# google/speedy

Measured on AMD Instinct MI355X. Metric: Msamples/s processed (16 kHz mono, 3.5x nonlinear), higher is better.
Workload: dtype int16 samples; f64 DFT, f32 features, int32 AMDF/OLA

## Files before the change

### include/speedy_hip.h

```cpp
#ifndef SPEEDY_HIP_H_
#define SPEEDY_HIP_H_
#include <stddef.h>
#include <stdint.h>
#ifdef __cplusplus
extern "C" {
#endif

#ifndef SPX_FEATURE_COUNT
#define SPX_FEATURE_COUNT 15
#endif

typedef struct spx_plan* spx_plan_t;

typedef struct {
  int64_t in_off;
  int64_t n_in;
  int64_t out_off;
  int64_t out_cap;
  int32_t channels;
  float speed;
  float nonlinear;
  float feedback;
} spx_stream_job;

// ... 16 lines not shown
int spx_plan_future(spx_plan_t plan);
int spx_plan_max_required(spx_plan_t plan);
int64_t spx_plan_frames(spx_plan_t plan, int64_t n_in);
int64_t spx_plan_out_capacity(spx_plan_t plan, int64_t n_in, float speed);
int64_t spx_plan_out_capacity_for(spx_plan_t plan, int64_t n_in, float speed, float nonlinear);

size_t spx_batch_workspace_bytes(spx_plan_t plan, const spx_stream_job* jobs, int n_streams);

int spx_batch_run(spx_plan_t plan, const spx_stream_job* jobs, int n_streams, const int16_t* in,
                  int16_t* out, int64_t* n_out, void* workspace, size_t workspace_bytes,
                  const spx_taps* taps, void* hip_stream);

int spx_batch_run_rate(spx_plan_t plan, const spx_stream_job* jobs, const float* rates, int n_streams, const int16_t* in,
                       int16_t* out, int64_t* n_out, void* workspace, size_t workspace_bytes,
                       const spx_taps* taps, void* hip_stream);
size_t spx_batch_workspace_bytes_rate(spx_plan_t plan, const spx_stream_job* jobs, const float* rates, int n_streams);
int64_t spx_plan_out_capacity_rate(spx_plan_t plan, int64_t n_in, float speed, float nonlinear, float rate);

size_t spx_batch_workspace_bytes_float(spx_plan_t plan, const spx_stream_job* jobs, const float* rates, int n_streams);
int spx_batch_run_float(spx_plan_t plan, const spx_stream_job* jobs, const float* rates, int n_streams, const float* in,
                        float* out, int64_t* n_out, void* workspace, size_t workspace_bytes,
                        const spx_taps* taps, void* hip_stream);
int spx_float_to_short(const float* in, int16_t* out, size_t n, int nonlinear_scale, void* hip_stream);
int spx_short_to_float(const int16_t* in, float* out, size_t n, void* hip_stream);

int spx_batch_run_ahead(spx_plan_t plan, const spx_stream_job* jobs, int n_streams, const int16_t* in,
                        int16_t* out, int64_t* n_out, void* workspace, size_t workspace_bytes,
                        const spx_taps* taps, void* hip_stream);

int spx_batch_run_overlapped(spx_plan_t plan, const spx_stream_job* jobs, int n_streams, const int16_t* in,
                             int16_t* out, int64_t* n_out, void* workspace, size_t workspace_bytes,
                             const spx_taps* taps, void* hip_stream);

int spx_batch_run_ahead_when(spx_plan_t plan, const spx_stream_job* jobs, int n_streams, const int16_t* in,
                             int16_t* out, int64_t* n_out, void* workspace, size_t workspace_bytes,
                             const spx_taps* taps, void* hip_stream, void* in_ready_event);

typedef struct spx_pipeline* spx_pipeline_t;
#define SPX_PIPELINE_DEVICE_OUT 1u
spx_pipeline_t spx_pipeline_create(spx_plan_t plan, const spx_stream_job* jobs, int n_streams, int depth, unsigned flags);
spx_pipeline_t spx_pipeline_create_mixed(const spx_plan_t* plans, int n_plans, const spx_stream_job* jobs, const int* plan_index,
                                         int n_streams, int depth, unsigned flags);
void spx_pipeline_destroy(spx_pipeline_t p);
int spx_pipeline_depth(spx_pipeline_t p);
size_t spx_pipeline_input_values(spx_pipeline_t p);
int16_t* spx_pipeline_host_input(spx_pipeline_t p);
int64_t spx_pipeline_submit(spx_pipeline_t p, const int16_t* in, int in_is_device);
int64_t spx_pipeline_submit_jobs(spx_pipeline_t p, const spx_stream_job* jobs, const int16_t* in, int in_is_device);
int spx_pipeline_jobs_fit(spx_pipeline_t p, const spx_stream_job* jobs);
int spx_pipeline_input_consumed(spx_pipeline_t p, int64_t ticket);
int spx_pipeline_wait(spx_pipeline_t p, int64_t ticket, const int16_t** out, const int64_t** offsets, const int64_t** counts);
void* spx_host_alloc(size_t bytes);
void spx_host_free(void* p);

int spx_batch_analyze(spx_plan_t plan, const spx_stream_job* jobs, int n_streams, const int16_t* in,
                      void* workspace, size_t workspace_bytes, const spx_taps* taps, void* hip_stream);
int spx_batch_walk(spx_plan_t plan, const spx_stream_job* jobs, int n_streams, const int16_t* in,
                   int16_t* out, int64_t* n_out, void* workspace, size_t workspace_bytes,
                   const spx_taps* taps, void* hip_stream);

size_t spx_batch_workspace_bytes_mixed(const spx_plan_t* plans, int n_plans, const spx_stream_job* jobs,
                                       const int* plan_index, int n_streams);
int spx_batch_run_mixed(const spx_plan_t* plans, int n_plans, const spx_stream_job* jobs, const int* plan_index,
                        int n_streams, const int16_t* in, int16_t* out, int64_t* n_out, void* workspace,
                        size_t workspace_bytes, void* hip_stream);

int spx_batch_run_mixed_taps(const spx_plan_t* plans, int n_plans, const spx_stream_job* jobs, const int* plan_index,
                             int n_streams, const int16_t* in, int16_t* out, int64_t* n_out, void* workspace,
                             size_t workspace_bytes, const spx_taps* taps, void* hip_stream);
int spx_batch_run_mixed_ahead(const spx_plan_t* plans, int n_plans, const spx_stream_job* jobs, const int* plan_index,
                              int n_streams, const int16_t* in, int16_t* out, int64_t* n_out, void* workspace,
                              size_t workspace_bytes, void* hip_stream);

void spx_set_timing(int enabled);
void spx_set_pipeline_chunks(int chunks);
void spx_set_concurrent(int on);
int spx_timing_collect(double* sum_ms_analyze, double* sum_ms_walk, int* n_calls);
const char* spx_batch_kernel_names(spx_plan_t plan, int n_streams, int max_channels, int speedup_only);
const char* spx_batch_kernel_names_lean(spx_plan_t plan, int n_streams, int max_channels, int speedup_only);
int spx_debug_last_walk_form(void);
int spx_debug_kernel_vgprs(int which);
int spx_debug_walk_info(int sample_rate, int channels, int n_streams, int speedup_only, int short_jobs, int lean, int* out5);
int spx_debug_analysis_info(int sample_rate, int* out4);
int spx_debug_mode_resources(int sample_rate, int channels, int n_streams, int speedup_only, long long* out22);
long long spx_debug_fdiv_check(unsigned seed, unsigned denominators, int exp_lo, int exp_hi);
long long spx_debug_xfade_check(int n_lo, int n_hi);
long long spx_debug_arith_check(unsigned seed, unsigned threads, unsigned per_thread);
int spx_debug_log_check(unsigned first_block, unsigned end_block, unsigned long long* sums);
int spx_debug_last_call_concurrent(void);
double spx_timing_last_tension_ms(void);
double spx_timing_last_rate_ms(void);

int spx_batch_read_steps(spx_plan_t plan, const spx_stream_job* jobs, int n_streams, const void* workspace,
                         int32_t* steps, void* hip_stream);
int spx_batch_read_steps_mixed(const spx_plan_t* plans, int n_plans, const spx_stream_job* jobs, const int* plan_index,
                               int n_streams, const void* workspace, int32_t* steps, void* hip_stream);

void* spx_device_alloc(size_t bytes);
void spx_device_free(void* p);
int spx_batch_pack_outputs(const spx_stream_job* jobs, int n_streams, const int16_t* out, const int64_t* n_out,
                           int16_t* packed, int64_t* offsets, void* hip_stream);
int spx_copy_to_device(void* dst, const void* src, size_t bytes, void* hip_stream);
int spx_copy_to_host(void* dst, const void* src, size_t bytes, void* hip_stream);
int spx_stream_synchronize(void* hip_stream);

#ifdef __cplusplus
}
#endif
#endif
```

### speedy_amd/_lib.py

```python
import ctypes as C
import os
import subprocess

_HERE = os.path.dirname(os.path.abspath(__file__))
LIB_PATH = os.environ.get("SPEEDY_HIP_LIB") or os.path.join(_HERE, "lib", "libspeedy_hip.so")
_LIB = None

c_short_p = C.POINTER(C.c_short)
c_float_p = C.POINTER(C.c_float)
c_int64_p = C.POINTER(C.c_int64)


class StreamJob(C.Structure):
    _fields_ = [("in_off", C.c_int64), ("n_in", C.c_int64), ("out_off", C.c_int64), ("out_cap", C.c_int64),
                ("channels", C.c_int32), ("speed", C.c_float), ("nonlinear", C.c_float), ("feedback", C.c_float)]


class Taps(C.Structure):
    _fields_ = [("tension", C.c_void_p), ("speed", C.c_void_p), ("features", C.c_void_p),
                ("spectrogram", C.c_void_p), ("normalized", C.c_void_p)]


TENSION_FN = C.CFUNCTYPE(None, C.c_void_p, C.c_int, C.c_float)
FEATURES_FN = C.CFUNCTYPE(None, C.c_void_p, C.c_int, c_float_p)

SYMBOLS = {
    "spx_last_error": (C.c_char_p, []),
    "spx_abi_version": (C.c_int, []),
    "spx_plan_create": (C.c_void_p, [C.c_int, C.c_int]),
    "spx_plan_destroy": (None, [C.c_void_p]),
    "spx_plan_frame_step": (C.c_int, [C.c_void_p]),
    "spx_plan_window_size": (C.c_int, [C.c_void_p]),
    "spx_plan_fft_size": (C.c_int, [C.c_void_p]),
    "spx_plan_future": (C.c_int, [C.c_void_p]),
    "spx_plan_max_required": (C.c_int, [C.c_void_p]),
    "spx_plan_frames": (C.c_int64, [C.c_void_p, C.c_int64]),
    "spx_plan_out_capacity": (C.c_int64, [C.c_void_p, C.c_int64, C.c_float]),
    "spx_plan_out_capacity_for": (C.c_int64, [C.c_void_p, C.c_int64, C.c_float, C.c_float]),
    "spx_batch_workspace_bytes": (C.c_size_t, [C.c_void_p, C.POINTER(StreamJob), C.c_int]),
    "spx_batch_run": (C.c_int, [C.c_void_p, C.POINTER(StreamJob), C.c_int, C.c_void_p, C.c_void_p, C.c_void_p,
                                C.c_void_p, C.c_size_t, C.POINTER(Taps), C.c_void_p]),
    "spx_batch_run_rate": (C.c_int, [C.c_void_p, C.POINTER(StreamJob), c_float_p, C.c_int, C.c_void_p, C.c_void_p, C.c_void_p,
                                     C.c_void_p, C.c_size_t, C.POINTER(Taps), C.c_void_p]),
    "spx_batch_workspace_bytes_rate": (C.c_size_t, [C.c_void_p, C.POINTER(StreamJob), c_float_p, C.c_int]),
    "spx_plan_out_capacity_rate": (C.c_int64, [C.c_void_p, C.c_int64, C.c_float, C.c_float, C.c_float]),
    "spx_batch_workspace_bytes_float": (C.c_size_t, [C.c_void_p, C.POINTER(StreamJob), c_float_p, C.c_int]),
    "spx_batch_run_float": (C.c_int, [C.c_void_p, C.POINTER(StreamJob), c_float_p, C.c_int, C.c_void_p, C.c_void_p, C.c_void_p,
                                      C.c_void_p, C.c_size_t, C.POINTER(Taps), C.c_void_p]),
    "spx_float_to_short": (C.c_int, [C.c_void_p, C.c_void_p, C.c_size_t, C.c_int, C.c_void_p]),
    "spx_short_to_float": (C.c_int, [C.c_void_p, C.c_void_p, C.c_size_t, C.c_void_p]),
    "spx_batch_run_ahead": (C.c_int, [C.c_void_p, C.POINTER(StreamJob), C.c_int, C.c_void_p, C.c_void_p, C.c_void_p,
                                      C.c_void_p, C.c_size_t, C.POINTER(Taps), C.c_void_p]),
    "spx_batch_run_overlapped": (C.c_int, [C.c_void_p, C.POINTER(StreamJob), C.c_int, C.c_void_p, C.c_void_p, C.c_void_p,
                                           C.c_void_p, C.c_size_t, C.POINTER(Taps), C.c_void_p]),
    "spx_batch_run_ahead_when": (C.c_int, [C.c_void_p, C.POINTER(StreamJob), C.c_int, C.c_void_p, C.c_void_p, C.c_void_p,
                                           C.c_void_p, C.c_size_t, C.POINTER(Taps), C.c_void_p, C.c_void_p]),
    "spx_batch_workspace_bytes_mixed": (C.c_size_t, [C.POINTER(C.c_void_p), C.c_int, C.POINTER(StreamJob), C.POINTER(C.c_int), C.c_int]),
    "spx_batch_run_mixed": (C.c_int, [C.POINTER(C.c_void_p), C.c_int, C.POINTER(StreamJob), C.POINTER(C.c_int), C.c_int,
                                      C.c_void_p, C.c_void_p, C.c_void_p, C.c_void_p, C.c_size_t, C.c_void_p]),
    "spx_batch_run_mixed_ahead": (C.c_int, [C.POINTER(C.c_void_p), C.c_int, C.POINTER(StreamJob), C.POINTER(C.c_int), C.c_int,
                                      C.c_void_p, C.c_void_p, C.c_void_p, C.c_void_p, C.c_size_t, C.c_void_p]),
    "spx_batch_run_mixed_taps": (C.c_int, [C.POINTER(C.c_void_p), C.c_int, C.POINTER(StreamJob), C.POINTER(C.c_int), C.c_int,
                                           C.c_void_p, C.c_void_p, C.c_void_p, C.c_void_p, C.c_size_t, C.POINTER(Taps), C.c_void_p]),
    "spx_batch_read_steps": (C.c_int, [C.c_void_p, C.POINTER(StreamJob), C.c_int, C.c_void_p, C.POINTER(C.c_int32), C.c_void_p]),
    "spx_batch_read_steps_mixed": (C.c_int, [C.POINTER(C.c_void_p), C.c_int, C.POINTER(StreamJob), C.POINTER(C.c_int), C.c_int,
                                             C.c_void_p, C.POINTER(C.c_int32), C.c_void_p]),
    "spx_batch_analyze": (C.c_int, [C.c_void_p, C.POINTER(StreamJob), C.c_int, C.c_void_p, C.c_void_p,
                                    C.c_size_t, C.POINTER(Taps), C.c_void_p]),
    "spx_batch_walk": (C.c_int, [C.c_void_p, C.POINTER(StreamJob), C.c_int, C.c_void_p, C.c_void_p, C.c_void_p,
                                 C.c_void_p, C.c_size_t, C.POINTER(Taps), C.c_void_p]),
    "spx_set_timing": (None, [C.c_int]),
    "spx_set_pipeline_chunks": (None, [C.c_int]),
    "spx_set_concurrent": (None, [C.c_int]),
    "spx_timing_collect": (C.c_int, [C.POINTER(C.c_double), C.POINTER(C.c_double), C.POINTER(C.c_int)]),
    "spx_timing_last_tension_ms": (C.c_double, []),
    "spx_timing_last_rate_ms": (C.c_double, []),
    "spx_batch_kernel_names": (C.c_char_p, [C.c_void_p, C.c_int, C.c_int, C.c_int]),
    "spx_batch_kernel_names_lean": (C.c_char_p, [C.c_void_p, C.c_int, C.c_int, C.c_int]),
    "spx_debug_last_walk_form": (C.c_int, []),
    "spx_debug_kernel_vgprs": (C.c_int, [C.c_int]),
    "spx_debug_last_call_concurrent": (C.c_int, []),
    "spx_debug_fdiv_check": (C.c_longlong, [C.c_uint, C.c_uint, C.c_int, C.c_int]),
    "spx_debug_xfade_check": (C.c_longlong, [C.c_int, C.c_int]),
    "spx_debug_arith_check": (C.c_longlong, [C.c_uint, C.c_uint, C.c_uint]),
    "spx_debug_log_check": (C.c_int, [C.c_uint, C.c_uint, C.POINTER(C.c_ulonglong)]),
    "spx_debug_walk_info": (C.c_int, [C.c_int, C.c_int, C.c_int, C.c_int, C.c_int, C.c_int, C.POINTER(C.c_int)]),
    "spx_debug_analysis_info": (C.c_int, [C.c_int, C.POINTER(C.c_int)]),
    "spx_debug_mode_resources": (C.c_int, [C.c_int, C.c_int, C.c_int, C.c_int, C.POINTER(C.c_longlong)]),
    "spx_pipeline_create": (C.c_void_p, [C.c_void_p, C.POINTER(StreamJob), C.c_int, C.c_int, C.c_uint]),
    "spx_pipeline_create_mixed": (C.c_void_p, [C.POINTER(C.c_void_p), C.c_int, C.POINTER(StreamJob), C.POINTER(C.c_int), C.c_int, C.c_int, C.c_uint]),
    "spx_pipeline_destroy": (None, [C.c_void_p]),
    "spx_pipeline_depth": (C.c_int, [C.c_void_p]),
    "spx_pipeline_input_values": (C.c_size_t, [C.c_void_p]),
    "spx_pipeline_host_input": (C.c_void_p, [C.c_void_p]),
    "spx_pipeline_submit": (C.c_int64, [C.c_void_p, C.c_void_p, C.c_int]),
    "spx_pipeline_submit_jobs": (C.c_int64, [C.c_void_p, C.POINTER(StreamJob), C.c_void_p, C.c_int]),
    "spx_pipeline_jobs_fit": (C.c_int, [C.c_void_p, C.POINTER(StreamJob)]),
    "spx_pipeline_input_consumed": (C.c_int, [C.c_void_p, C.c_int64]),
    "spx_pipeline_wait": (C.c_int, [C.c_void_p, C.c_int64, C.POINTER(C.c_void_p), C.POINTER(C.c_void_p), C.POINTER(C.c_void_p)]),
    "spx_host_alloc": (C.c_void_p, [C.c_size_t]),
    "spx_host_free": (None, [C.c_void_p]),
    "spx_device_alloc": (C.c_void_p, [C.c_size_t]),
    "spx_device_free": (None, [C.c_void_p]),
    "spx_copy_to_device": (C.c_int, [C.c_void_p, C.c_void_p, C.c_size_t, C.c_void_p]),
    "spx_copy_to_host": (C.c_int, [C.c_void_p, C.c_void_p, C.c_size_t, C.c_void_p]),
    "spx_batch_pack_outputs": (C.c_int, [C.c_void_p, C.c_int, C.c_void_p, C.c_void_p, C.c_void_p, C.c_void_p, C.c_void_p]),
    "spx_stream_synchronize": (C.c_int, [C.c_void_p]),
    "sonicCreateStream": (C.c_void_p, [C.c_int, C.c_int]),
    "sonicDestroyStream": (None, [C.c_void_p]),
    "sonicWriteShortToStream": (C.c_int, [C.c_void_p, c_short_p, C.c_int]),
    "sonicReadShortFromStream": (C.c_int, [C.c_void_p, c_short_p, C.c_int]),
    "sonicWriteFloatToStream": (C.c_int, [C.c_void_p, c_float_p, C.c_int]),
    "sonicReadFloatFromStream": (C.c_int, [C.c_void_p, c_float_p, C.c_int]),
    "sonicSetRate": (None, [C.c_void_p, C.c_float]),
    "sonicSetSpeed": (None, [C.c_void_p, C.c_float]),
    "sonicFlushStream": (C.c_int, [C.c_void_p]),
    "sonicEnableNonlinearSpeedup": (None, [C.c_void_p, C.c_float]),
    "sonicSetDurationFeedbackStrength": (None, [C.c_void_p, C.c_float]),
    "getSonicBufferSize": (C.c_int, [C.c_void_p]),
    "sonicSpectrogramSize": (C.c_int, [C.c_void_p]),
    "sonicTensionCallback": (None, [C.c_void_p, TENSION_FN]),
    "getSonicTensionCallback": (C.c_void_p, [C.c_void_p]),
    "sonicSpeedCallback": (None, [C.c_void_p, TENSION_FN]),
    "getSonicSpeedCallback": (C.c_void_p, [C.c_void_p]),
    "sonicFeaturesCallback": (None, [C.c_void_p, FEATURES_FN]),
    "getSonicFeaturesCallback": (C.c_void_p, [C.c_void_p]),
    "sonicSpectrogramCallback": (None, [C.c_void_p, FEATURES_FN]),
    "getSonicSpectrogramCallback": (C.c_void_p, [C.c_void_p]),
    "sonicNormalizedSpectrogramCallback": (None, [C.c_void_p, FEATURES_FN]),
    "getSonicNormalizedSpectrogramCallback": (C.c_void_p, [C.c_void_p]),
    "sonicIntGetNumChannels": (C.c_int, [C.c_void_p]),
    "sonicIntGetSampleRate": (C.c_int, [C.c_void_p]),
    "sonicIntGetSpeed": (C.c_float, [C.c_void_p]),
    "sonicIntCreateStream": (C.c_void_p, [C.c_int, C.c_int]),
    "sonicIntDestroyStream": (None, [C.c_void_p]),
    "sonicIntSetSpeed": (None, [C.c_void_p, C.c_float]),
    "sonicIntSetRate": (None, [C.c_void_p, C.c_float]),
    "sonicIntWriteShortToStream": (C.c_int, [C.c_void_p, c_short_p, C.c_int]),
    "sonicIntWriteFloatToStream": (C.c_int, [C.c_void_p, c_float_p, C.c_int]),
    "sonicIntReadShortFromStream": (C.c_int, [C.c_void_p, c_short_p, C.c_int]),
    "sonicIntReadFloatFromStream": (C.c_int, [C.c_void_p, c_float_p, C.c_int]),
    "sonicIntFlushStream": (C.c_int, [C.c_void_p]),
    "sonicIntSamplesAvailable": (C.c_int, [C.c_void_p]),
    "sonicIntSetUserData": (None, [C.c_void_p, C.c_void_p]),
    "sonicIntGetUserData": (C.c_void_p, [C.c_void_p]),
    "speedyCreateStream": (C.c_void_p, [C.c_int]),
    "speedyDestroyStream": (None, [C.c_void_p]),
    "speedyInputFrameSize": (C.c_int, [C.c_void_p]),
    "speedyInputFrameStep": (C.c_int, [C.c_void_p]),
    "speedyFFTSize": (C.c_int, [C.c_void_p]),
    "speedyBinToFreq": (C.c_float, [C.c_void_p, C.c_int]),
    "speedyFreqToBin": (C.c_int, [C.c_void_p, C.c_float]),
    "speedyAddData": (None, [C.c_void_p, c_float_p, C.c_int64]),
    "speedyAddDataShort": (None, [C.c_void_p, c_short_p, C.c_int64]),
    "speedyComputeTension": (C.c_int, [C.c_void_p, C.c_int64, c_float_p]),
    "speedyComputeSpeedFromTension": (C.c_float, [C.c_float, C.c_float, C.c_float, C.c_void_p]),
    "speedyGetCurrentTime": (C.c_int64, [C.c_void_p]),
    "speedySpectrogram": (c_float_p, [C.c_void_p, c_float_p]),
    "speedyGetSpectrogram": (c_float_p, [C.c_void_p]),
    "speedyGetSpectrogramAtTime": (c_float_p, [C.c_void_p, C.c_int64]),
    "speedyGetNormalizedSpectrogram": (c_float_p, [C.c_void_p]),
    "speedyGetInternalState": (c_float_p, [C.c_void_p]),
    "speedyGetEnergyCompressed": (C.c_float, [C.c_void_p]),
    "speedyGetSpeechChanges": (C.c_float, [C.c_void_p]),
    "speedyHipHysteresisFuture": (C.c_int, [C.c_void_p]),
    "speedyHipHysteresisPast": (C.c_int, [C.c_void_p]),
    "speedyComputeSpectralDifference": (None, [C.c_void_p, c_float_p, c_float_p, C.c_int64]),
    "speedyComputeLocalEnergy": (None, [C.c_void_p, c_float_p, C.c_int64]),
    "speedySaveSpectrogramData": (None, [C.c_void_p, c_float_p, C.c_int64]),
    "speedyPreemphasisFilter": (None, [C.c_void_p, c_float_p, C.c_int]),
# ... 43 lines not shown
```

### speedy_amd/csrc/sonic2_api.hip

```cpp
#include <stdio.h>
#include <stdlib.h>
#include <string.h>

#include <algorithm>
#include <string>
#include <cmath>
#include <vector>

#include "../../include/sonic2.h"
#include "spx_internal.h"

#include <atomic>
static thread_local std::string g_api_err;
static std::atomic<int> g_match_matlab{0};

#include "sonic2_stream.h"

void spx_internal_set_api_error(const std::string& msg) { g_api_err = msg; }
void spx_api_error(const std::string& msg) { g_api_err = msg; }
int spx_internal_match_matlab() { return g_match_matlab.load(); }

static bool any_callback(sonicStream s) {
  return s->cbTension || s->cbSpeed || s->cbFeatures || s->cbSpectrogram || s->cbNormalized;
}
// ... 277 lines not shown
        }
    }
  }
  SlideBuf<int16_t>& tsmIn = s->mixed ? s->dTsm : s->dIn;
  J.tsmIn = &tsmIn;
  if (!s->dIn.p && !s->dIn.ensure(0, 64 * C, hs, 1 << 16, defer)) return 0;
  if (!tsmIn.p && !tsmIn.ensure(0, 64 * C, hs, 1 << 16, defer)) return 0;
  auto off16 = [&](const SlideBuf<int16_t>& b) -> int64_t {
    return (pool ? (int64_t)(reinterpret_cast<uintptr_t>(b.p) / sizeof(int16_t)) : 0) - b.origin;
  };
  SpxStreamDev& JA = J.JA;
  SpxStreamDev& JW = J.JW;
  memset(&JA, 0, sizeof(JA));
  JA.in_off = off16(s->dIn); JA.n_in = s->nIn;
  JA.out_off = off16(s->dOut); JA.out_cap = (s->dOut.origin + s->dOut.cap) / C;
  JA.frame_off = -s->dRec.origin;
  if (pool && s->dRec.p) JA.frame_off += s->dRec.p - spx_pool_arena_rec(pool);
  JA.n_frames = (int32_t)T; JA.frame_begin = (int32_t)fa;
  JA.channels = (int32_t)C;
  const int common = (flush ? SPX_F_FLUSH : 0) | (s->rateMode ? SPX_F_NO_TRUNC : 0) | (s->speedSet ? SPX_F_SPEED_SET : 0);
  s->speedSet = false;
  JA.flags = common | (s->tensionStarted ? 0 : SPX_F_INIT);
  JA.speed = s->globalSpeed; JA.nonlinear = nonlinear ? s->nonlinearFactor : 0.0f; JA.feedback = s->feedbackStrength;
  JA.tsm_shift = s->tsmShift;
  JA.tension_skip = (int32_t)s->tensionSkip;
  JA.first_tile = 0;
  JW = JA;
  JW.speed = s->tsmSpeed;
  JW.flags = common | (s->started ? 0 : SPX_F_INIT);
  if (s->mixed) {
    JW.in_off = off16(s->dTsm); JW.n_in = s->tPhys;
    JW.flags |= SPX_F_HANDED_IN | (nonlinear ? 0 : SPX_F_KEEP_SPEED);
    JW.handed_in = (int32_t)handedBefore;
    JW.ring_bufs = (int32_t)(s->nIn / B);
    if (flush && !direct) JW.nonlinear = (s->nonlinearFactor != 0.0f) ? s->nonlinearFactor : 1.0f;
  }
  if (!(JA.speed > 1.0f && JW.speed > 1.0f && JA.speed < SPX_FAST_MAX_SPEED && JW.speed < SPX_FAST_MAX_SPEED && JA.nonlinear >= 0.0f &&
        JA.nonlinear <= 1.0f))
    s->speedupOnly = false;
  J.speedupKernel = s->speedupOnly && !s->rateMode && !s->mixed;
  J.tiles = (nonlinear && T > fa) ? (int)((T - fa + P.tile_frames - 1) / P.tile_frames) : 0;
  return 1;
}

void spx_finish_job(sonicStream s, const SpxJobPlan& J) {
  const SpxPlanDev& P = *s->plan;
  const int F = P.F;
  s->started = true;
  s->dirty = true;
  s->outBound = J.need;
  s->handedHost = J.handedAfter;
  if (J.nonlinear) s->tensionStarted = true;
  const int64_t k_first = std::max(s->tensionDone, s->tensionSkip);
  if (J.hasRing) s->framesDone = std::max(s->framesDone, J.nonlinear ? J.T : J.fa);
  if (J.nonlinear) s->tensionDone = std::max<int64_t>(k_first, (J.T >= F) ? J.T - F + 1 : 0);
  if (J.flush) {
    if (J.hasRing && !J.direct) {
      s->tensionSkip = std::max(s->tensionSkip, J.nIn / P.B);
      s->tensionDone = std::max(s->tensionDone, s->tensionSkip);
    }
    s->tsmShift += 2 * (int64_t)P.maxRequired;
  }
}

static int launch_job(sonicStream s, bool flush, bool direct = false) {
  const SpxPlanDev& P = *s->plan;
  const int64_t C = s->channels;
  SpxJobPlan J;
  if (!spx_prepare_job(s, flush, direct, s->hs, nullptr, J)) return 0;
  static_assert(2 * 128 <= SPX_STAGE_JOB && sizeof(SpxStreamDev) <= 128, "job table slot");
  memset(s->hPinned, 0, 256);
  memcpy(s->hPinned, &J.JA, sizeof(SpxStreamDev));
  memcpy(s->hPinned + 128, &J.JW, sizeof(SpxStreamDev));
  SpxStreamDev* dJobW = reinterpret_cast<SpxStreamDev*>(reinterpret_cast<unsigned char*>(s->dJob) + 128);
  if (hipMemcpyAsync(s->dJob, s->hPinned, 256, hipMemcpyHostToDevice, s->hs) != hipSuccess) return 0;
  (void)hipEventRecord(s->evStaged, s->hs);
  SpxTapsDev td = {nullptr, nullptr, nullptr, nullptr, nullptr};
  const int64_t fo = J.JA.frame_off;
  if (J.taps) {
    td.tension = s->tTension.base() - fo; td.speed = s->tSpeed.base() - fo;
    td.features = s->tFeatures.base() - fo * SPX_FEATURE_COUNT;
    td.spectrogram = s->tSpec.base() - fo * P.N; td.normalized = s->tNorm.base() - fo * P.W;
  }
  if (J.tiles > 0) spx_launch_analysis(P, s->dJob, 1, J.tiles, s->dIn.p, s->dRec.p, td, nullptr, nullptr, s->hs);
  if (J.nonlinear) spx_launch_tension(P, s->dJob, 1, s->dState, s->dRec.p, s->dScr.p, td, nullptr, nullptr, s->hs);
  spx_launch_walk(P, {.n_streams = 1, .max_channels = (int)C, .speedup_only = J.speedupKernel, .short_jobs = true}, dJobW, J.tsmIn->p,
                  s->dOut.p, s->dNOut, s->dState, s->dScr.p, nullptr, 0, s->hs);
  if (s->rateMode)
    spx_launch_rate(s->dRate, s->dState, s->dNOut, s->dOut.base(), s->dFinal.base(),
                    (s->dFinal.origin + s->dFinal.cap) / C, (int)C, J.oldR, J.newR, s->rate, s->rate == 1.0f ? 1 : 0,
                    flush ? 1 : 0, s->hs);
  if (hipGetLastError() != hipSuccess) { spx_stream_fail(s, "kernel launch failed"); return 0; }
  const int64_t k_first = std::max(s->tensionDone, s->tensionSkip);
  spx_finish_job(s, J);
  if (J.taps && J.T > J.fa) run_callbacks(s, J.fa, J.T, k_first);
  return 1;
}

static bool enter_rate_mode(sonicStream s) {
  if (s->channels > SPX_RATE_MAX_CHANNELS) {
    g_api_err = "sonicSetRate != 1 supports at most 16 channels";
    return false;
  }
  if (!sync_stream(s)) return false;
  const int64_t C = s->channels;
  const int64_t n = s->outKnown - s->outRead;
  if (!s->dFinal.ensure(s->outRead * C, (s->outKnown + 4096) * C, s->hs, 1 << 16)) return false;
  if (n > 0 && hipMemcpyAsync(s->dFinal.base() + s->outRead * C, s->dOut.base() + s->outRead * C,
                              sizeof(int16_t) * (size_t)(n * C), hipMemcpyDeviceToDevice, s->hs) != hipSuccess)
    return false;
  SpxRateState* h = reinterpret_cast<SpxRateState*>(staging(s, sizeof(SpxRateState)));
  if (!h) return false;
  memset(h, 0, sizeof(*h));
  h->tsm_seen = s->outKnown;
  h->final_n = s->outKnown;
  if (hipMemcpyAsync(s->dRate, h, sizeof(*h), hipMemcpyHostToDevice, s->hs) != hipSuccess) return false;
  (void)hipEventRecord(s->evStaged, s->hs);
  s->finKnown = s->finBound = s->tsmSeenKnown = s->outKnown;
  s->rateMode = true;
  return true;
}

static bool enter_mixed(sonicStream s) {
  if (!sync_stream(s)) return false;
  const int64_t C = s->channels;
  if (s->mode == 0) {
    std::swap(s->dTsm, s->dIn);
    s->tPhys = s->nIn;
    s->nIn = 0;
  } else {
    const int64_t hi = s->handedHost * (int64_t)s->plan->B;
    int64_t lo = std::max<int64_t>(0, s->tsmBase - s->tsmShift - 16);
    lo = std::min(std::max(lo, s->dIn.origin / C), hi);
    s->dTsm.filled = 0;
    if (!s->dTsm.ensure(lo * C, hi * C + 64, s->hs, 1 << 16)) return false;
    if (hi > lo && hipMemcpyAsync(s->dTsm.base() + lo * C, s->dIn.base() + lo * C, sizeof(int16_t) * (size_t)((hi - lo) * C),
                                  hipMemcpyDeviceToDevice, s->hs) != hipSuccess)
      return false;
    s->tPhys = hi;
  }
  s->mixed = true;
  return true;
}

bool spx_settings_ok(sonicStream s) {
  if (!(s->globalSpeed > 0.0f) || !std::isfinite(s->globalSpeed) || !(s->tsmSpeed > 0.0f) || !std::isfinite(s->tsmSpeed)) {
    g_api_err = "sonicSetSpeed: speed must be finite and > 0";
    return false;
  }
  if (!(s->nonlinearFactor >= 0.0f && s->nonlinearFactor <= 1.0f)) {
    g_api_err = "sonicEnableNonlinearSpeedup: factor outside [0, 1] (sonic2.h:73-76; the blended speed could reach 0)";
    return false;
  }
  if (!(s->rate > 0.0f) || !std::isfinite(s->rate)) { g_api_err = "sonicSetRate: rate must be finite and > 0"; return false; }
  if (!std::isfinite(s->feedbackStrength)) { g_api_err = "sonicSetDurationFeedbackStrength: not finite"; return false; }
  return true;
}

static int write_shorts(sonicStream s, const short* in, int sampleCount, bool direct = false) {
  if (spx_stream_failed(s) || !spx_settings_ok(s)) return 0;
  const int want = (s->nonlinearFactor != 0.0f && !direct) ? 1 : 0;
  if (s->pooled && (direct || s->rate != 1.0f || any_callback(s) || (s->mode >= 0 && s->mode != want)) && !spx_pool_leave(s))
    return 0;
  if (!s->pooled) (void)hipSetDevice(s->device);
  if (s->rate != 1.0f && !s->rateMode && !enter_rate_mode(s)) return 0;
  if (want == 1 && !spx_internal_analysis_fits(*s->plan)) {
    g_api_err = "sample rate too high for the nonlinear path (the analysis tile does not fit one CU's LDS); linear mode only";
// ... 143 lines not shown
```

### speedy_amd/csrc/sonic2_pool.hip

```cpp
#include <sched.h>
#include <stdio.h>
#include <stdlib.h>
#include <string.h>

#include <atomic>
#include <chrono>
#include <condition_variable>
#include <mutex>
#include <thread>

#include "sonic2_stream.h"

static std::atomic<int> g_coalesce{-1};

struct PinBuf {
  unsigned char* p = nullptr;
  size_t cap = 0;
  bool reserve(size_t need, size_t keep) {
    if (need <= cap) return true;
    size_t n = cap ? cap : (1u << 20);
    while (n < need) n *= 2;
    unsigned char* np = nullptr;
    if (hipHostMalloc(reinterpret_cast<void**>(&np), n, hipHostMallocDefault) != hipSuccess) return false;
    if (p && keep) memcpy(np, p, keep);
// ... 387 lines not shown
    }
    g.i1 = j;
    groups.push_back(g);
    i = j;
  }
  const size_t b_jobs = sizeof(SpxStreamDev) * n;
  const size_t o_desc = 2 * b_jobs, o_copies = o_desc + sizeof(PoolDesc) * n;
  const size_t o_moves = (o_copies + sizeof(PoolCopy) * copies.size() + 15) & ~(size_t)15;
  const size_t b_tab = o_moves + sizeof(SpxMove) * moves.size();
  auto give_up = [&](const char* why) {
    for (auto& it : items) spx_stream_fail(it.s, why);
    end_run(P, run);
    return RUN_FAILED;
  };
  if (!P->hTab.reserve(b_tab + 64, 0)) return give_up("pinned table allocation failed");
  size_t res_elems = 0;
  int64_t max_slice = 0;
  std::vector<int64_t>& res_off = P->res_off;
  std::vector<int64_t>& res_cap = P->res_cap;
  res_off.resize(n);
  res_cap.resize(n);
  for (size_t i = 0; i < n; i++) {
    sonicStream s = items[i].s;
    res_cap[i] = std::max<int64_t>(0, items[i].J.need - s->outKnown);
    res_off[i] = (int64_t)res_elems;
    const int64_t e = res_cap[i] * s->channels;
    max_slice = std::max(max_slice, e);
    res_elems += (size_t)((e + 7) & ~(int64_t)7);
  }
  const size_t o_out = (sizeof(PoolResult) * n + 63) & ~(size_t)63;
  if (!P->hRes.reserve(o_out + res_elems * sizeof(int16_t) + 64, 0)) return give_up("pinned result allocation failed");
  const size_t w_states = (2 * b_jobs + 63) & ~(size_t)63, w_nout = w_states + ((sizeof(SpxStreamState) * n + 63) & ~(size_t)63);
  const size_t w_total = w_nout + sizeof(int64_t) * n;
  if (w_total > P->dWsCap) {
    if (P->dWs) (void)hipFree(P->dWs);
    P->dWs = nullptr;
    size_t cap = P->dWsCap ? P->dWsCap : 65536;
    while (cap < w_total) cap *= 2;
    if (hipMalloc(reinterpret_cast<void**>(&P->dWs), cap) != hipSuccess) { P->dWs = nullptr; P->dWsCap = 0; (void)hipGetLastError(); return give_up("pool workspace allocation failed"); }
    P->dWsCap = cap;
  }
  SpxStreamDev* hA = reinterpret_cast<SpxStreamDev*>(P->hTab.p);
  SpxStreamDev* hW = hA + n;
  PoolDesc* hD = reinterpret_cast<PoolDesc*>(P->hTab.p + o_desc);
  PoolCopy* hC = reinterpret_cast<PoolCopy*>(P->hTab.p + o_copies);
  for (size_t i = 0; i < n; i++) {
    sonicStream s = items[i].s;
    hA[i] = items[i].J.JA;
    hW[i] = items[i].J.JW;
    hW[i].first_tile = hA[i].first_tile;
    PoolDesc& D = hD[i];
    D.home = s->dState;
    D.out_base = s->dOut.base();
    D.out_from = s->outKnown;
    D.out_cap = items[i].J.JA.out_cap;
    D.res_off = res_off[i];
    D.res_cap = res_cap[i];
    D.channels = s->channels;
    D.pad = 0;
  }
  if (!copies.empty()) memcpy(hC, copies.data(), sizeof(PoolCopy) * copies.size());
  SpxMove* hM = reinterpret_cast<SpxMove*>(P->hTab.p + o_moves);
  if (!moves.empty()) memcpy(hM, moves.data(), sizeof(SpxMove) * moves.size());
  SpxStreamDev* dA = reinterpret_cast<SpxStreamDev*>(P->dWs);
  SpxStreamDev* dW = dA + n;
  SpxStreamState* dStates = reinterpret_cast<SpxStreamState*>(P->dWs + w_states);
  int64_t* dNout = reinterpret_cast<int64_t*>(P->dWs + w_nout);
  PoolResult* hR = reinterpret_cast<PoolResult*>(P->hRes.p);
  int16_t* hOut = reinterpret_cast<int16_t*>(P->hRes.p + o_out);

  const unsigned n_words = (unsigned)(2 * b_jobs / 4);
  const unsigned grid = std::max<unsigned>(std::max<unsigned>((unsigned)(copies.size() + moves.size()), (n_words + 255) / 256), 1u);
  const auto tp2 = std::chrono::steady_clock::now();
  hipLaunchKernelGGL(spx_pool_stage_kernel, dim3(grid), dim3(256), 0, P->hs, reinterpret_cast<const unsigned*>(hA),
                     reinterpret_cast<unsigned*>(dA), n_words, hD, dStates, (unsigned)n, hC, (unsigned)copies.size(), run_in,
                     hM, (unsigned)moves.size());
  auto tl = std::chrono::steady_clock::now();
  auto lap = [&](int k) { const auto t = std::chrono::steady_clock::now(); P->t_l[k] += std::chrono::duration<double>(t - tl).count(); tl = t; };
  lap(0);
  const SpxTapsDev no_taps = {nullptr, nullptr, nullptr, nullptr, nullptr};
  for (const Group& g : groups) {
    const SpxPlanDev& PL = *items[g.i0].s->plan;
    const int ng = (int)(g.i1 - g.i0);
    if (g.tiles > 0) spx_launch_analysis(PL, dA + g.i0, ng, g.tiles, nullptr, P->aRec, no_taps, nullptr, nullptr, P->hs);
    lap(1);
    bool any_nl = false;
    for (size_t i = g.i0; i < g.i1; i++) any_nl = any_nl || items[i].J.nonlinear;
    if (any_nl) spx_launch_tension(PL, dA + g.i0, ng, dStates + g.i0, P->aRec, P->aScr, no_taps, nullptr, nullptr, P->hs);
    lap(2);
    spx_launch_walk(PL, {.n_streams = ng, .max_channels = g.maxC, .speedup_only = items[g.i0].J.speedupKernel, .short_jobs = true}, dW + g.i0,
                    nullptr, nullptr, dNout + g.i0, dStates + g.i0, P->aScr, nullptr, 0, P->hs);
    lap(3);
  }
  const unsigned gy = (unsigned)std::min<int64_t>(64, std::max<int64_t>(1, (max_slice + 8191) / 8192));
  hipLaunchKernelGGL(spx_pool_gather_kernel, dim3((unsigned)n, gy), dim3(256), 0, P->hs, hD, dStates, dNout, hR, hOut);
  lap(4);
  P->launchErr = hipGetLastError();
  P->resOut = o_out;
  P->tLaunched = std::chrono::steady_clock::now();
  P->t_prep += sec(tp0, tp1); P->t_tab += sec(tp1, tp2); P->t_launch += sec(tp2, P->tLaunched);
  return RUN_LAUNCHED;
}

static bool complete_run(SpxPool* P, hipError_t se) {
  const auto tp4 = std::chrono::steady_clock::now();
  std::vector<SpxPool::Item>& items = P->items;
  std::vector<sonicStream>& run = P->run;
  const hipError_t le = P->launchErr;
  if (le != hipSuccess || se != hipSuccess) {
    const std::string why = std::string("coalesced launch failed: ") + hipGetErrorString(le != hipSuccess ? le : se);
    for (auto& it : items) spx_stream_fail(it.s, why);
    end_run(P, run);
    return false;
  }
  const size_t n = items.size();
  const std::vector<int64_t>& res_off = P->res_off;
  const std::vector<int64_t>& res_cap = P->res_cap;
  const PoolResult* hR = reinterpret_cast<const PoolResult*>(P->hRes.p);
  const int16_t* hOut = reinterpret_cast<const int16_t*>(P->hRes.p + P->resOut);
  for (size_t i = 0; i < n; i++) {
    sonicStream s = items[i].s;
    spx_finish_job(s, items[i].J);
    int64_t k = hR[i].n;
    if (k == SPX_NOUT_LOST_PRODUCER) {
      spx_stream_fail(s, "a producer kernel never delivered its frames (device-side poll limit reached)");
      k = s->outKnown;
    } else if (k < 0) {
      spx_stream_fail(s, "output capacity exceeded on the device");
      k = -k;
    }
    const int64_t avail = std::min(k, items[i].J.JA.out_cap) - s->outKnown;
    const int64_t fresh = std::max<int64_t>(0, std::min(avail, res_cap[i]));
    if (avail > res_cap[i] && !s->failed)
      spx_stream_fail(s, "the device produced more frames than the host-side bound of the job (coalesced result slice)");
    if (fresh > 0) {
      const int16_t* src = hOut + res_off[i];
      s->hostOut.insert(s->hostOut.end(), src, src + fresh * s->channels);
    }
    s->outKnown += fresh;
    s->outBound = s->outKnown;
    s->tsmBase = hR[i].st.w.base;
    s->curSpeedKnown = hR[i].st.curSpeed;
    s->dirty = false;
    s->writesSinceSync = 0;
    s->devIn = items[i].J.nIn;
  }
  P->runs++;
  P->jobs += n;
  end_run(P, run);
  const auto tp5 = std::chrono::steady_clock::now();
  P->t_wait += sec(P->tLaunched, tp4); P->t_post += sec(tp4, tp5);
  return true;
}

static bool await_run(SpxPool* P, std::unique_lock<std::mutex>& lk) {
  P->detached.store(false, std::memory_order_release);
  static const long spin_us = [] { const char* e = getenv("SPX_POOL_SPIN_US"); return e ? atol(e) : 2000L; }();
  lk.unlock();
  hipError_t se = hipErrorNotReady;
  if (spin_us > 0) {
    const auto t_spin = std::chrono::steady_clock::now();
    while ((se = hipStreamQuery(P->hs)) == hipErrorNotReady) {
      if (std::chrono::duration<double, std::micro>(std::chrono::steady_clock::now() - t_spin).count() > (double)spin_us) break;
    }
    if (se == hipErrorNotReady) (void)hipGetLastError();
  }
  if (se == hipErrorNotReady) se = hipStreamSynchronize(P->hs);
// ... 227 lines not shown
```

### speedy_amd/csrc/spx_analysis.hip

```cpp
#include <stdlib.h>

#include "spx_internal.h"
#include "spx_walk_common.h"

#ifndef SPX_TF
#define SPX_TF 16
#endif

#ifdef SPX_STAMPS
__device__ unsigned long long g_spx_astamps[16];
#define ASTAMP_DECL unsigned long long as_last = __builtin_readcyclecounter(), as_acc[10] = {0,0,0,0,0,0,0,0,0,0};
#define ASTAMP(i) do { const unsigned long long t_ = __builtin_readcyclecounter(); as_acc[i] += t_ - as_last; as_last = t_; } while (0)
#define ASTAMP_FLUSH if (threadIdx.x == 0 && blockIdx.x == 7) for (int i_ = 0; i_ < 10; i_++) g_spx_astamps[i_] += as_acc[i_];
extern "C" void spx_debug_astamps(unsigned long long* out, int reset) {
  (void)hipMemcpyFromSymbol(out, HIP_SYMBOL(g_spx_astamps), sizeof(unsigned long long) * 16);
  if (reset) { unsigned long long z[16] = {0}; (void)hipMemcpyToSymbol(HIP_SYMBOL(g_spx_astamps), z, sizeof(z)); }
}
#else
#define ASTAMP_DECL
#define ASTAMP(i)
#define ASTAMP_FLUSH
#endif

#ifndef SPX_TF_SMALL
#define SPX_TF_SMALL 8
#endif
#define SPX_TF_TINY 4
int spx_analysis_tile_frames() { return SPX_TF; }
int spx_analysis_small_tile_frames() { return SPX_TF_SMALL; }
int spx_analysis_tiny_tile_frames() { return SPX_TF_TINY; }

#define SPX_CB 24
static __host__ __device__ constexpr int spx_mag_stride(int W) { return (W + 4) & ~3; }
static __host__ __device__ constexpr int spx_cb(int tf) { return tf <= 8 ? 2 * SPX_CB : SPX_CB; }
#ifdef SPX_LOG_V1
#define SPX_LOG_LDS_BYTES 0
#else
#define SPX_LOG_LDS_BYTES 2048
#endif
static __host__ __device__ inline size_t terms_bytes(int W, int tf, bool ct) {
  const size_t b = ct ? (size_t)2 * tf * (spx_cb(tf) + 1) * sizeof(double)
                      : (size_t)tf * (W + 1) * sizeof(double);
  return (b + 15) & ~(size_t)15;
}
static __host__ __device__ inline size_t work_bytes(int W, int tf, bool ct = false, int dft_waves = 4) {
  if (dft_waves < 1 || dft_waves > 4) dft_waves = 4;
  const size_t a = ct ? (size_t)4 * 2 * W * sizeof(double)
                      : (size_t)dft_waves * 2 * 2 * W * sizeof(double);
  const size_t b = terms_bytes(W, tf, ct) + SPX_LOG_LDS_BYTES;
  return (a > b ? a : b);
}
static inline int plan_ct_window(const SpxPlanDev& P) {
  auto is = [](const int* r, int n, std::initializer_list<int> want) {
    if (n != (int)want.size()) return false;
    int k = 0;
    for (int w : want) if (r[k++] != w) return false;
    return true;
  };
  if (!P.rader && P.W == 240 && is(P.radix, P.nstages, {4, 4, 3, 5})) return 240;
  if (!P.rader && P.W == 330 && is(P.radix, P.nstages, {2, 3, 5, 11})) return 330;
  if (P.tile_frames == SPX_TF_SMALL && P.dft_waves == 4) {
    if (!P.rader && P.W == 720 && is(P.radix, P.nstages, {4, 4, 3, 3, 5})) return 720;
    if (P.rader && P.W == 661 && is(P.radixM, P.nstagesM, {4, 3, 5, 11})) return 661;
  }
  if (!P.rader && P.dft_waves == 4) {
    if (P.W == 120 && is(P.radix, P.nstages, {4, 2, 3, 5}) && (P.tile_frames == SPX_TF || P.tile_frames == SPX_TF_SMALL)) return 120;
    if (P.W == 180 && is(P.radix, P.nstages, {4, 3, 3, 5}) && P.tile_frames == SPX_TF) return 180;
    if (P.W == 360 && is(P.radix, P.nstages, {4, 2, 3, 3, 5}) && P.tile_frames == SPX_TF) return 360;
    if (P.W == 480 && is(P.radix, P.nstages, {4, 4, 2, 3, 5}) && P.tile_frames == SPX_TF) return 480;
  }
  return 0;
}
int spx_analysis_prefers_small_tile(const SpxPlanDev& P) {
  SpxPlanDev Q = P;
  Q.tile_frames = SPX_TF_SMALL;
  Q.dft_waves = 4;
  const int w = plan_ct_window(Q);
  return w == 720 || w == 661;
}
static __host__ __device__ inline size_t stage_samples(const SpxPlanDev& P, int tf) {
  return (size_t)(tf + 1) * P.B + (P.W - P.B) + 8;
}
static size_t analysis_lds_bytes(const SpxPlanDev& P, bool ct) {
  const int tf = P.tile_frames > 0 ? P.tile_frames : SPX_TF;
  size_t mags = (size_t)(tf + 1) * spx_mag_stride(P.W) * sizeof(float);
  size_t small = (size_t)3 * (tf + 1) * sizeof(float);
  size_t stage = (stage_samples(P, tf) * sizeof(short) + 15) & ~(size_t)15;
  return work_bytes(P.W, tf, ct, P.dft_waves) + ((mags + 15) & ~(size_t)15) + ((small + 15) & ~(size_t)15) + stage;
}
size_t spx_analysis_lds_bytes(const SpxPlanDev& P) { return analysis_lds_bytes(P, plan_ct_window(P) != 0); }
int spx_analysis_ct_window(const SpxPlanDev& P) { return plan_ct_window(P); }

__device__ __forceinline__ void wave_sync() {
  __builtin_amdgcn_fence(__ATOMIC_RELEASE, "wavefront");
  __builtin_amdgcn_wave_barrier();
  __builtin_amdgcn_fence(__ATOMIC_ACQUIRE, "wavefront");
}

#include "spx_log.h"

__device__ __forceinline__ float spx_untangle_mag(double ar, double ai, double b_r, double b_i, double2 w) {
  const double dr = ar - b_r, di = ai - b_i;
#ifdef SPX_DFT_V1
  const double er = 0.5 * (ar + b_r), ei = 0.5 * (ai + b_i);
  const double o_r = 0.5 * di, o_i = -0.5 * dr;
  const double xr = er + (w.x * o_r - w.y * o_i);
  const double xi = ei + (w.x * o_i + w.y * o_r);
  return spx_sqrt64_to_f32(xr * xr + xi * xi);
#else
  const double xr2 = __builtin_fma(w.x, di, __builtin_fma(w.y, dr, ar + b_r));
  const double xi2 = __builtin_fma(w.y, di, __builtin_fma(-w.x, dr, ai + b_i));
  return spx_sqrt64_to_f32(0.25 * __builtin_fma(xr2, xr2, xi2 * xi2));
#endif
}

#define C5_1 0.30901699437494742
#define C5_2 (-0.80901699437494742)
#define S5_1 0.95105651629515357
#define S5_2 0.58778525229247313
#define S3_1 0.86602540378443865

struct cplx {
  double r, i;
};

#ifdef SPX_DFT_V1
#define SPX_FMA_OR(a, b, c, unfused) (unfused)
#else
#define SPX_FMA_OR(a, b, c, unfused) __builtin_fma((a), (b), (c))
#endif
__host__ __device__ __forceinline__ cplx spx_cmul(cplx b, double wx, double wy) {
  return {SPX_FMA_OR(b.r, wx, -(b.i * wy), b.r * wx - b.i * wy), SPX_FMA_OR(b.r, wy, b.i * wx, b.r * wy + b.i * wx)};
}
__host__ __device__ __forceinline__ double spx_bf3h(double a0, double t1) { return SPX_FMA_OR(-0.5, t1, a0, a0 - 0.5 * t1); }
__host__ __device__ __forceinline__ double spx_bf5m(double a0, double c1, double t1, double c2, double t2) {
  return SPX_FMA_OR(c2, t2, __builtin_fma(c1, t1, a0), (a0 + c1 * t1) + c2 * t2);
}
__host__ __device__ __forceinline__ double spx_bf5n(double s1, double t3, double s2, double t4) { return SPX_FMA_OR(s1, t3, s2 * t4, s1 * t3 + s2 * t4); }
__host__ __device__ __forceinline__ double spx_bf5d(double s2, double t3, double s1, double t4) { return SPX_FMA_OR(s2, t3, -(s1 * t4), s2 * t3 - s1 * t4); }
__host__ __device__ __forceinline__ double spx_acc(double p, double w, double u) { return SPX_FMA_OR(w, u, p, p + w * u); }

__host__ __device__ __forceinline__ cplx ld(const double* buf, int idx) {
  const double2 v = *reinterpret_cast<const double2*>(buf + 2 * idx);
  return {v.x, v.y};
}
__host__ __device__ __forceinline__ void st_tw(double* buf, int idx, cplx b, const double* tw, int t) {
  const double2 w = *reinterpret_cast<const double2*>(tw + 2 * t);
  const cplx v = spx_cmul(b, w.x, w.y);
  *reinterpret_cast<double2*>(buf + 2 * idx) = make_double2(v.r, v.i);
}

__host__ __device__ void dft_stage(const int W, const double* tw, int r, int s, int cur, const double* x, double* y,
                                   int lane, const int nl) {
  const int m = cur / r;
  const int span = W / r;
  const unsigned inv_s = ((1u << 20) + (unsigned)s - 1u) / (unsigned)s;
  if (r == 4) {
    for (int b = lane; b < span; b += nl) {
      const int p = (int)(((unsigned)b * inv_s) >> 20), q = b - p * s;
      cplx a0 = ld(x, b), a1 = ld(x, b + span), a2 = ld(x, b + 2 * span), a3 = ld(x, b + 3 * span);
      cplx t0 = {a0.r + a2.r, a0.i + a2.i}, t1 = {a0.r - a2.r, a0.i - a2.i};
      cplx t2 = {a1.r + a3.r, a1.i + a3.i}, t3 = {a1.r - a3.r, a1.i - a3.i};
      cplx b0 = {t0.r + t2.r, t0.i + t2.i}, b2 = {t0.r - t2.r, t0.i - t2.i};
      cplx b1 = {t1.r + t3.i, t1.i - t3.r}, b3 = {t1.r - t3.i, t1.i + t3.r};
      const int o = q + s * 4 * p;
      const int tp = s * p;
      st_tw(y, o, b0, tw, 0);
      st_tw(y, o + s, b1, tw, tp);
      st_tw(y, o + 2 * s, b2, tw, 2 * tp);
      st_tw(y, o + 3 * s, b3, tw, 3 * tp);
    }
  } else if (r == 2) {
    for (int b = lane; b < span; b += nl) {
// ... 153 lines not shown
    for (int i = 0; i < R; i++) a[u][i] = load(u, i);
  }
  wave_sync();
#pragma unroll
  for (int u = 0; u < NP; u++) {
    const int b = lane + 64 * u;
    if (b < SPAN) {
      cplx o[R];
      ct_bfly<R>(a[u], o);
      const int p = b / S, q = b - p * S;
      const int base = q + S * R * p, tp = S * p;
      st(buf, base, o[0]);
#pragma unroll
      for (int j = 1; j < R; j++) st(buf, base + j * S, LAST ? o[j] : cmul_tw(o[j], twp[j * tp]));
    }
  }
  wave_sync();
}
template <int NPTS, int R>
struct ct_from_buf {
  const double* buf;
  int lane;
  __device__ __forceinline__ cplx operator()(int u, int i) const {
    constexpr int SPAN = NPTS / R;
    const int b = (lane + 64 * u < SPAN) ? lane + 64 * u : 0;
    return ld(buf, b + i * SPAN);
  }
};

template <int W, int ST, int S>
__device__ __forceinline__ void ct_stages_from(double* buf, const double2* __restrict__ twp, const int lane) {
  if constexpr (ST < ct_plan<W>::n) {
    constexpr int R = ct_plan<W>::r[ST];
    ct_stage<W, R, S>(buf, twp, lane, ct_from_buf<W, R>{buf, lane});
    ct_stages_from<W, ST + 1, S * R>(buf, twp, lane);
  }
}

template <int NPTS, int R>
__device__ __forceinline__ void ct_stage_prime_last(double* buf, const int lane, const double (&wc)[R - 1], const double (&ws)[R - 1]) {
  constexpr int SPAN = NPTS / R, H = (R - 1) / 2;
  static_assert(SPAN <= 64, "one pass");
  if (lane < SPAN) {
    cplx a[R];
#pragma unroll
    for (int i = 0; i < R; i++) a[i] = ld(buf, lane + SPAN * i);
    cplx uu[H], vv[H];
    cplx B0 = a[0];
#pragma unroll
    for (int i = 1; i <= H; i++) {
      uu[i - 1] = {a[i].r + a[R - i].r, a[i].i + a[R - i].i};
      vv[i - 1] = {a[i].r - a[R - i].r, a[i].i - a[R - i].i};
      B0.r = B0.r + uu[i - 1].r; B0.i = B0.i + uu[i - 1].i;
    }
    st(buf, lane, B0);
#pragma unroll
    for (int jj = 1; jj <= H; jj++) {
      cplx Pj = a[0], Qj = {0.0, 0.0};
#pragma unroll
      for (int i = 1; i <= H; i++) {
        const double wx = wc[(i * jj) % R - 1], wy = ws[(i * jj) % R - 1];
        Pj.r = spx_acc(Pj.r, wx, uu[i - 1].r); Pj.i = spx_acc(Pj.i, wx, uu[i - 1].i);
        if (i == 1) { Qj.r = wy * vv[0].r; Qj.i = wy * vv[0].i; }
        else { Qj.r = spx_acc(Qj.r, wy, vv[i - 1].r); Qj.i = spx_acc(Qj.i, wy, vv[i - 1].i); }
      }
      st(buf, lane + SPAN * jj, cplx{Pj.r - Qj.i, Pj.i + Qj.r});
      st(buf, lane + SPAN * (R - jj), cplx{Pj.r + Qj.i, Pj.i - Qj.r});
    }
  }
  wave_sync();
}

template <class T>
__device__ __forceinline__ const T* per_frame(const T* p) {
  asm volatile("" : "+s"(p));
  return p;
}
__device__ __forceinline__ double uniform_f64(double v) {
  return __longlong_as_double(((long long)__builtin_amdgcn_readfirstlane((int)(__double_as_longlong(v) >> 32)) << 32) |
                              (unsigned)__builtin_amdgcn_readfirstlane((int)__double_as_longlong(v)));
}

#ifdef SPX_PREEMPH_V1
#define SPX_WIN_SCALE 1.0f
__device__ __forceinline__ float spx_preemph_win_f32(double md, double mpd, float w) {
  const float x = (float)(md / 32768.0), xp = (float)(mpd / 32768.0);
  const float y = (float)(1.0 * (double)x - 0.97 * (double)xp);
  return y * w;
}
#else
#define SPX_WIN_SCALE 0x1p-15f
__device__ __forceinline__ float spx_preemph_win_f32(double md, double mpd, float w15) {
  const float yy = (float)(md - 0.97 * mpd);
  return yy * w15;
}
#endif
__device__ __forceinline__ double spx_preemph_win(double md, double mpd, float w) { return (double)spx_preemph_win_f32(md, mpd, w); }
__device__ __forceinline__ cplx packed_point(const short* fr, int n, int j, int prev0, float w0, float w1) {
  const int i0 = 2 * n;
  const int m0 = fr[i0], m1 = fr[i0 + 1];
  const int mp0 = (i0 > 0) ? (int)fr[i0 - 1] : ((j > 0) ? (int)fr[prev0] : 0);
  const double d0 = (double)m0;
  return {spx_preemph_win(d0, (double)mp0, w0 * SPX_WIN_SCALE), spx_preemph_win((double)m1, d0, w1 * SPX_WIN_SCALE)};
}

#ifndef SPX_AN_W_330
#define SPX_AN_W_330 3
#endif
#ifndef SPX_AN_W_BIG
#define SPX_AN_W_BIG 2
#endif
template <int TF, int WCT>
__global__ void __launch_bounds__(SPX_BLOCK, (WCT == 240 || WCT == 120 || WCT == 180) ? 4 : WCT == 330 ? SPX_AN_W_330 : (WCT == 661 || WCT == 720) ? SPX_AN_W_BIG : (WCT == 480 || WCT == 360) ? 2 : 1)
spx_analysis_kernel(SpxPlanDev P, const SpxStreamDev* __restrict__ streams, int n_streams,
                    const int16_t* __restrict__ in_base, SpxFrameRec* __restrict__ rec, SpxTapsDev taps,
                    const int* __restrict__ tile_order, int* tile_flags, const float* __restrict__ frames,
                    int frame_mode) {
  extern __shared__ __attribute__((aligned(16))) unsigned char lds[];
  const int W = WCT ? WCT : P.W, B = P.B, N = 2 * W;
  const int tid = threadIdx.x, lane = tid & 63, wave = tid >> 6;

  const int tile = tile_order ? tile_order[blockIdx.x] : (int)blockIdx.x;
  int lo = 0, hi = n_streams - 1;
  while (lo < hi) {
    int mid = (lo + hi + 1) >> 1;
    if (streams[mid].first_tile <= tile) lo = mid; else hi = mid - 1;
  }
  const SpxStreamDev S = streams[lo];
  const int T = S.n_frames;
  const int j0 = S.frame_begin + (tile - S.first_tile) * TF;
  const int j1 = min(j0 + TF, T);
  const int C = S.channels;
  const int16_t* __restrict__ in = in_base + S.in_off;

  double* work = reinterpret_cast<double*>(lds);
  const size_t wb = work_bytes(W, TF, WCT != 0, (WCT != 0) ? 4 : P.dft_waves);
  float* mags = reinterpret_cast<float*>(lds + wb);
  const size_t mags_b = (((size_t)(TF + 1) * spx_mag_stride(W) * sizeof(float)) + 15) & ~(size_t)15;
  float* fE = reinterpret_cast<float*>(lds + wb + mags_b);
  float* fThr = fE + (TF + 1);
  float* fInv = fThr + (TF + 1);
  const int MS = spx_mag_stride(W);

  const size_t small_b = (((size_t)3 * (TF + 1) * sizeof(float)) + 15) & ~(size_t)15;
  const double* ltw = P.tw;
  const double* ltw2 = P.tw2;
  short* smono = reinterpret_cast<short*>(lds + wb + mags_b + small_b);

  double* bufA = work + (size_t)wave * (WCT != 0 ? 2 : 4) * W;
  double* bufB = (WCT != 0) ? bufA : bufA + 2 * W;

  const int jfirst = (j0 > 0) ? j0 - 1 : 0;
  const int64_t sbase = (int64_t)jfirst * B;
  const int nstage = (j1 - jfirst) * B + (W - B);
  if (frames != nullptr) {
  } else if (C == 1) {
    const int16_t* __restrict__ src = in + sbase;
    for (int k0 = tid; k0 < nstage; k0 += 8 * SPX_BLOCK) {
      short v[8];
#pragma unroll
      for (int u = 0; u < 8; u++) { const int k = k0 + u * SPX_BLOCK; v[u] = (k < nstage) ? src[k] : (short)0; }
#pragma unroll
      for (int u = 0; u < 8; u++) { const int k = k0 + u * SPX_BLOCK; if (k < nstage) smono[k] = v[u]; }
    }
  } else {
    for (int k = tid; k < nstage; k += SPX_BLOCK) smono[k] = (short)mono_sample(in, sbase + k, C);
  }
  __syncthreads();

  ASTAMP_DECL
  if constexpr (WCT == 240) {
    const double2* twp = reinterpret_cast<const double2*>(P.tw);
    const double2* tw2p = reinterpret_cast<const double2*>(P.tw2);
    const int b = lane;
    const bool on60 = b < 60, on48 = b < 48;
    const int bb = on60 ? b : 0;
    double2 w1[3], w2[3], w3[2][2], wu[4];
    float wn[4];
#pragma unroll
    for (int j = 1; j < 4; j++) { w1[j - 1] = twp[bb * j]; w2[j - 1] = twp[4 * (bb >> 2) * j]; }
#pragma unroll
    for (int u = 0; u < 2; u++) {
      const int b3 = lane + 64 * u, p3 = (b3 < 80) ? (b3 >> 4) : 0;
      w3[u][0] = twp[16 * p3];
      w3[u][1] = twp[32 * p3];
    }
#pragma unroll
    for (int u = 0; u < 4; u++) { const int k = lane + 64 * u; wu[u] = tw2p[k < 240 ? k : 0]; }
    wn[0] = P.window[2 * bb]; wn[1] = P.window[2 * bb + 1]; wn[2] = P.window[2 * bb + 120]; wn[3] = P.window[2 * bb + 121];
#pragma unroll
    for (int k = 0; k < 4; k++) wn[k] *= SPX_WIN_SCALE;
    for (int s = wave; s <= TF; s += 4) {
      const int j = j0 - 1 + s;
      float* mrow = mags + (size_t)s * MS;
      if (j < 0 || j >= j1) {
        for (int k = lane; k < 240; k += SPX_WAVE) mrow[k] = 0.0f;
        continue;
      }
      const short* fr = smono + (size_t)(j - jfirst) * B;
      if (on60) {
        const int i0 = 2 * b, i1 = 2 * b + 120;
        const int m0 = fr[i0], m1 = fr[i0 + 1], m2 = fr[i1], m3 = fr[i1 + 1];
        const int mp0 = (i0 > 0) ? (int)fr[i0 - 1] : ((j > 0) ? (int)fr[(240 - B) - 1] : 0);
        const int mp2 = fr[i1 - 1];
        const double d0 = (double)m0, d2 = (double)m2;
        const cplx a0 = {spx_preemph_win(d0, (double)mp0, wn[0]), spx_preemph_win((double)m1, d0, wn[1])},
                   a1 = {spx_preemph_win(d2, (double)mp2, wn[2]), spx_preemph_win((double)m3, d2, wn[3])};
        const cplx b0 = {a0.r + a1.r, a0.i + a1.i}, b2 = {a0.r - a1.r, a0.i - a1.i};
        const cplx b1 = {a0.r + a1.i, a0.i - a1.r}, b3 = {a0.r - a1.i, a0.i + a1.r};
        st(bufA, 4 * b, b0);
        st(bufA, 4 * b + 1, cmul_tw(b1, w1[0]));
        st(bufA, 4 * b + 2, cmul_tw(b2, w1[1]));
        st(bufA, 4 * b + 3, cmul_tw(b3, w1[2]));
      }
      wave_sync();
      ASTAMP(0);
      if (on60) {
        const cplx a0 = ld(bufA, b), a1 = ld(bufA, b + 60), a2 = ld(bufA, b + 120), a3 = ld(bufA, b + 180);
        wave_sync();
        const cplx t0 = {a0.r + a2.r, a0.i + a2.i}, t1 = {a0.r - a2.r, a0.i - a2.i};
        const cplx t2 = {a1.r + a3.r, a1.i + a3.i}, t3 = {a1.r - a3.r, a1.i - a3.i};
        const cplx b0 = {t0.r + t2.r, t0.i + t2.i}, b2 = {t0.r - t2.r, t0.i - t2.i};
        const cplx b1 = {t1.r + t3.i, t1.i - t3.r}, b3 = {t1.r - t3.i, t1.i + t3.r};
        const int o = (b & 3) + 16 * (b >> 2);
        st(bufB, o, b0);
        st(bufB, o + 4, cmul_tw(b1, w2[0]));
        st(bufB, o + 8, cmul_tw(b2, w2[1]));
        st(bufB, o + 12, cmul_tw(b3, w2[2]));
      }
      wave_sync();
      {
        cplx q0[2], q1[2], q2[2];
#pragma unroll
        for (int u = 0; u < 2; u++) {
          const int b3i = (lane + 64 * u < 80) ? lane + 64 * u : 0;
          q0[u] = ld(bufB, b3i); q1[u] = ld(bufB, b3i + 80); q2[u] = ld(bufB, b3i + 160);
        }
        wave_sync();
#pragma unroll
        for (int u = 0; u < 2; u++) {
          const int b3i = lane + 64 * u;
          if (b3i < 80) {
            const cplx a0 = q0[u], a1 = q1[u], a2 = q2[u];
            const cplx t1 = {a1.r + a2.r, a1.i + a2.i};
            const cplx t2 = {spx_bf3h(a0.r, t1.r), spx_bf3h(a0.i, t1.i)};
            const cplx t3 = {S3_1 * (a1.r - a2.r), S3_1 * (a1.i - a2.i)};
            const cplx b0 = {a0.r + t1.r, a0.i + t1.i};
            const cplx b1 = {t2.r + t3.i, t2.i - t3.r}, b2 = {t2.r - t3.i, t2.i + t3.r};
            const int o = (b3i & 15) + 48 * (b3i >> 4);
            st(bufA, o, b0);
            st(bufA, o + 16, cmul_tw(b1, w3[u][0]));
            st(bufA, o + 32, cmul_tw(b2, w3[u][1]));
          }
        }
// ... 413 lines not shown
            const cplx a = ld(x, k);
            const double2 b = *reinterpret_cast<const double2*>(P.bfft + 2 * k);
            const cplx cc = spx_cmul(a, b.x, b.y);
            *reinterpret_cast<double2*>(x + 2 * k) = make_double2(cc.r, -cc.i);
          }
          wave_sync();
        }
      }
      const double inv = 1.0 / (double)M;
      const double* abuf = (P.nstagesM & 1) ? y : x;
      const cplx A0 = ld(abuf, M);
      wave_sync();
      for (int q = lane; q < M; q += SPX_WAVE) {
        const cplx c = ld(x, q);
        const double cr = c.r * inv, ci = -c.i * inv;
        *reinterpret_cast<double2*>(y + 2 * P.iperm[q]) = make_double2(x0.r + cr, x0.i + ci);
      }
      if (lane == 0) *reinterpret_cast<double2*>(y) = make_double2(x0.r + A0.r, x0.i + A0.i);
      wave_sync();
      { double* t = x; x = y; y = t; }
    } else {
      int sprod = 1, cur = W;
      for (int stg = 0; stg < P.nstages; stg++) {
        const int r = P.radix[stg];
        dft_stage(W, ltw, r, sprod, cur, x, y, lane, SPX_WAVE);
        wave_sync();
        double* t = x; x = y; y = t;
        sprod *= r;
        cur /= r;
      }
    }
    ASTAMP(1);
    float* spec_out = taps.spectrogram ? taps.spectrogram + (size_t)(S.frame_off + j) * N : nullptr;
    for (int k = lane; k < W; k += SPX_WAVE) {
      const int k2 = (k == 0) ? 0 : W - k;
      cplx a = ld(x, k), bb = ld(x, k2);
      const double b_r = bb.r, b_i = -bb.i;
      const float mag = spx_untangle_mag(a.r, a.i, b_r, b_i, *reinterpret_cast<const double2*>(ltw2 + 2 * k));
      mrow[k] = mag;
      if (spec_out) {
        spec_out[k] = mag;
        if (k > 0) spec_out[N - k] = mag;
        else spec_out[W] = (float)__builtin_fabs(a.r - a.i);
      }
    }
    wave_sync();
    ASTAMP(2);
  }
  ASTAMP(3);
  __syncthreads();
  ASTAMP(4);

  if (wave > 0) {
#ifdef SPX_ROWMAX_V1
    for (int s = wave - 1; s <= TF; s += 3) {
      const float* mrow = mags + (size_t)s * MS;
      float mx = 0.0f;
      for (int i = 1 + lane; i < W; i += SPX_WAVE) mx = fmaxf(mx, mrow[i]);
#pragma unroll
      for (int d = 32; d >= 1; d >>= 1) mx = fmaxf(mx, __shfl_xor(mx, d));
      if (lane == 0) fThr[s] = (float)((double)mx / 100.0);
    }
#else
    unsigned keep = 0u;
    int nrows = 0;
    for (int s = wave - 1; s <= TF; s += 3, nrows++) {
      const unsigned* mrow = reinterpret_cast<const unsigned*>(mags + (size_t)s * MS);
      unsigned m = 0u;
      for (int q = lane; 4 * q < W; q += SPX_WAVE) {
        const uint4 v = *reinterpret_cast<const uint4*>(mrow + 4 * q);
        const unsigned a = (q == 0) ? 0u : v.x;
        const unsigned b = (4 * q + 1 < W) ? v.y : 0u, c = (4 * q + 2 < W) ? v.z : 0u, d = (4 * q + 3 < W) ? v.w : 0u;
        const unsigned ab = a > b ? a : b, cd = c > d ? c : d;
        const unsigned abcd = ab > cd ? ab : cd;
        m = m > abcd ? m : abcd;
      }
      const float mx = wave_max_f(__builtin_bit_cast(float, m));
      if (lane == nrows) keep = __builtin_bit_cast(unsigned, mx);
    }
    if (lane < nrows) fThr[wave - 1 + 3 * lane] = (float)((double)__builtin_bit_cast(float, keep) / 100.0);
#endif
#ifndef SPX_LOG_V1
    if (tid < SPX_WAVE + 128)
      reinterpret_cast<uint4*>(reinterpret_cast<unsigned char*>(work) + terms_bytes(W, TF, WCT != 0))[tid - SPX_WAVE] =
          reinterpret_cast<const uint4*>(spx_log_table_dev)[tid - SPX_WAVE];
#endif
  } else if (tid <= TF) {
    const float4* r4 = reinterpret_cast<const float4*>(mags + (size_t)tid * MS);
    float e = 0.0f;
    __builtin_amdgcn_s_setprio(3);
    auto acc8 = [&](const float4& p, const float4& q) {
      const float4 pp = {p.x * p.x, p.y * p.y, p.z * p.z, p.w * p.w}, qq = {q.x * q.x, q.y * q.y, q.z * q.z, q.w * q.w};
      e += pp.x; e += pp.y; e += pp.z; e += pp.w;
      e += qq.x; e += qq.y; e += qq.z; e += qq.w;
    };
    {
      const float4 h = r4[0];
      if (1 < W) e += h.y * h.y;
      if (2 < W) e += h.z * h.z;
      if (3 < W) e += h.w * h.w;
    }
    int i = 4;
    float4 c0 = r4[1], c1 = r4[2], c2 = r4[3], c3 = r4[4];
#pragma unroll 1
    for (; i + 16 <= W; i += 16) {
      const float4 n0 = r4[(i >> 2) + 4], n1 = r4[(i >> 2) + 5], n2 = r4[(i >> 2) + 6], n3 = r4[(i >> 2) + 7];
      __builtin_amdgcn_sched_barrier(0);
      acc8(c0, c1);
      acc8(c2, c3);
      c0 = n0; c1 = n1; c2 = n2; c3 = n3;
    }
    {
      const float t[16] = {c0.x, c0.y, c0.z, c0.w, c1.x, c1.y, c1.z, c1.w, c2.x, c2.y, c2.z, c2.w, c3.x, c3.y, c3.z, c3.w};
#pragma unroll
      for (int u = 0; u < 16; u++)
        if (i + u < W) e += t[u] * t[u];
    }
    __builtin_amdgcn_s_setprio(0);
    const float eps = 2.2204e-16f;
    fE[tid] = e;
    fInv[tid] = (float)(1.0 / (__builtin_sqrt((double)e) + (double)eps));
  }
  __syncthreads();
  ASTAMP(5);

  const int nfr = j1 - j0;
#ifndef SPX_LOG_V1
  const SpxLogEntry* ltab = reinterpret_cast<const SpxLogEntry*>(reinterpret_cast<const unsigned char*>(work) + terms_bytes(W, TF, WCT != 0));
  auto log_of_ratio = [&](float ratio) -> double {
    double v = spx_log_v2_f32(ratio, ltab);
    if (__builtin_expect(!spx_log_v2_domain(ratio), 0)) v = spx_log_v1((double)ratio);
    return v;
  };
#else
  auto log_of_ratio = [&](float ratio) -> double { return spx_log_v1((double)ratio); };
#endif
  auto log_term = [&](int f, int i) -> double {
    const int sl = f + 1;
    const float cur = mags[(size_t)sl * MS + i], last = mags[(size_t)(sl - 1) * MS + i];
    const float thr = fThr[sl];
    double term = 0.0;
    if (cur > thr && last > thr) {
      const float eps = 2.2204e-16f;
      const float nc = cur * fInv[sl], nl = last * fInv[sl - 1];
      const float ratio = spx_fdiv32(nc + eps, nl + eps);
      term = __builtin_fabs(log_of_ratio(ratio));
    }
    return term;
  };
  auto write_rec = [&](int f, float lsd) {
    const float lowthr = (float)(0.04 * (double)1.41421f);
    const float e = fE[f + 1];
    SpxFrameRec r;
    r.energy = e;
    r.lsd = (e <= lowthr) ? 0.0f : lsd;
    rec[S.frame_off + j0 + f] = r;
  };
  if (taps.normalized) {
    for (int idx = tid; idx < nfr * W; idx += SPX_BLOCK) {
      const int f = idx / W, i = idx - f * W;
      const int j = j0 + f;
      const int row = j + (S.unit_time0 ? 0 : 1);
      if (row < T + (S.unit_time0 ? 1 : 0))
        taps.normalized[(size_t)(S.frame_off + row) * W + i] = mags[(size_t)(f + 1) * MS + i] * fInv[f + 1];
    }
    if (S.unit_time0) {
    } else if (j0 == 0) {
      for (int i = tid; i < W; i += SPX_BLOCK) taps.normalized[(size_t)S.frame_off * W + i] = 0.0f;
    } else if (j0 == S.frame_begin) {
      for (int i = tid; i < W; i += SPX_BLOCK)
        taps.normalized[(size_t)(S.frame_off + j0) * W + i] = mags[i] * fInv[0];
    }
  }
  if constexpr (WCT != 0) {
    constexpr int CB = spx_cb(TF);
    constexpr int CBS = CB + 1;
    static_assert(TF * CB == 2 * (SPX_BLOCK - SPX_WAVE), "two terms per lane of waves 1..3 and block");
    double* tblk = work;
    constexpr int NBLK = (WCT - 1 + CB - 1) / CB;
    float lsd = 0.0f;
    int fi[2], ci[2];
    bool ok[2];
#ifndef SPX_TERMS_V1
    const float* rowc[2];
    const float* rowl[2];
    float thrv[2], invc[2], invl[2];
#endif
#pragma unroll
    for (int t = 0; t < 2; t++) {
      const int it = tid - SPX_WAVE + t * (SPX_BLOCK - SPX_WAVE);
      fi[t] = wave > 0 ? it / CB : 0;
      ci[t] = wave > 0 ? it - fi[t] * CB : 0;
      ok[t] = wave > 0 && fi[t] < nfr;
#ifndef SPX_TERMS_V1
      const int fl = ok[t] ? fi[t] : 0;
      rowc[t] = mags + (size_t)(fl + 1) * MS;
      rowl[t] = mags + (size_t)fl * MS;
      thrv[t] = fThr[fl + 1];
      invc[t] = fInv[fl + 1];
      invl[t] = fInv[fl];
#endif
    }
    for (int k = 0; k <= NBLK; k++) {
      if (wave > 0) {
        if (k < NBLK) {
          double* tb = tblk + (size_t)(k & 1) * TF * CBS;
          bool gate[2];
          float xr[2];
#pragma unroll
          for (int t = 0; t < 2; t++) {
            const int i = 1 + k * CB + ci[t];
            const bool in = ok[t] && i < WCT;
#ifdef SPX_TERMS_V1
            const int fl = in ? fi[t] : 0, il = in ? i : 1;
            const float cur = mags[(size_t)(fl + 1) * MS + il], last = mags[(size_t)fl * MS + il];
            const float thr = fThr[fl + 1];
            const float fic = fInv[fl + 1], fil = fInv[fl];
#else
            const int il = (i < WCT) ? i : 1;
            const float cur = rowc[t][il], last = rowl[t][il];
            const float thr = thrv[t], fic = invc[t], fil = invl[t];
#endif
            gate[t] = in && cur > thr && last > thr;
            const float eps = 2.2204e-16f;
            const float nc = cur * fic, nl = last * fil;
            const float ratio = spx_fdiv32(nc + eps, nl + eps);
            xr[t] = gate[t] ? ratio : 2.0f;
          }
#ifdef SPX_LOG_V1
          const spx_log_parts p0 = spx_log_main((double)xr[0]), p1 = spx_log_main((double)xr[1]);
          const double t0 = gate[0] ? __builtin_fabs(spx_log_finish(p0, (double)xr[0])) : 0.0;
          const double t1 = gate[1] ? __builtin_fabs(spx_log_finish(p1, (double)xr[1])) : 0.0;
#else
          const double l0 = log_of_ratio(xr[0]), l1 = log_of_ratio(xr[1]);
          const double t0 = gate[0] ? __builtin_fabs(l0) : 0.0;
          const double t1 = gate[1] ? __builtin_fabs(l1) : 0.0;
#endif
          if (ok[0]) tb[fi[0] * CBS + ci[0]] = t0;
          if (ok[1]) tb[fi[1] * CBS + ci[1]] = t1;
        }
      } else if (k > 0 && tid < nfr) {
        const double* tb = tblk + (size_t)((k - 1) & 1) * TF * CBS + tid * CBS;
        const int i0 = 1 + (k - 1) * CB;
        __builtin_amdgcn_s_setprio(3);
        (void)i0;
        static_assert(CB % 8 == 0, "batches of eight");
        double tv[8];
#pragma unroll
        for (int u = 0; u < 8; u++) tv[u] = tb[u];
#pragma unroll
        for (int c = 0; c < CB; c += 8) {
          double nx[8];
          if (c + 8 < CB) {
#pragma unroll
            for (int u = 0; u < 8; u++) nx[u] = tb[c + 8 + u];
          }
#pragma unroll
          for (int u = 0; u < 8; u++) lsd = (float)((double)lsd + tv[u]);
          if (c + 8 < CB) {
#pragma unroll
            for (int u = 0; u < 8; u++) tv[u] = nx[u];
// ... 47 lines not shown
__global__ void spx_arith_check_kernel(unsigned seed, unsigned per_thread, unsigned long long* bad) {
  unsigned long long st = (unsigned long long)seed * 0x9E3779B97F4A7C15ull + (blockIdx.x * blockDim.x + threadIdx.x) * 0xD1B54A32D192ED03ull + 1;
  auto next = [&]() { st ^= st >> 12; st ^= st << 25; st ^= st >> 27; return st * 0x2545F4914F6CDD1Dull; };
  unsigned long long miss = 0;
  for (unsigned i = 0; i < per_thread; i++) {
    const unsigned long long a = next(), b = next(), c = next();
    const float fn = __uint_as_float((unsigned)((127 - 53 + (a % 57)) << 23) | (unsigned)((a >> 8) & 0x7fffff));
    const float fd = __uint_as_float((unsigned)((127 - 53 + (b % 57)) << 23) | (unsigned)((b >> 8) & 0x7fffff));
    if (__float_as_uint(spx_fdiv32(fn, fd)) != __float_as_uint(fn / fd)) miss++;
    const long long fb = ((long long)(1023 - 21 + (c % 20)) << 52) | (long long)((c >> 8) & 0xfffffffffffffll) | ((c >> 63) ? (1ll << 63) : 0);
    const double f = __longlong_as_double(fb);
    if (__double_as_longlong(spx_fdiv64(f, 2.0 + f)) != __double_as_longlong(f / (2.0 + f))) miss++;
    const long long xb = ((long long)(1023 - 800 + (a >> 33) % 1811) << 52) | (long long)((b >> 10) & 0xfffffffffffffll);
    const double x = ((c & 1023) == 0) ? 0.0 : __longlong_as_double(xb);
    if (__float_as_uint(spx_sqrt64_to_f32(x)) != __float_as_uint((float)__builtin_sqrt(x))) miss++;
  }
  if (miss) atomicAdd(bad, miss);
}
extern "C" long long spx_debug_arith_check(unsigned seed, unsigned threads, unsigned per_thread) {
  unsigned long long* d = nullptr;
  unsigned long long h = 0;
  if (hipMalloc(&d, sizeof(h)) != hipSuccess) return -1;
  if (hipMemcpy(d, &h, sizeof(h), hipMemcpyHostToDevice) != hipSuccess) { (void)hipFree(d); return -1; }
  const unsigned blocks = (threads + 255) / 256;
  hipLaunchKernelGGL(spx_arith_check_kernel, dim3(blocks), dim3(256), 0, nullptr, seed, per_thread, d);
  const bool ok = hipDeviceSynchronize() == hipSuccess && hipMemcpy(&h, d, sizeof(h), hipMemcpyDeviceToHost) == hipSuccess;
  (void)hipFree(d);
  return ok ? (long long)h : -1;
}

__global__ void __launch_bounds__(256) spx_log_check_kernel(unsigned first_block, unsigned long long* __restrict__ sums) {
#ifndef SPX_LOG_V1
  __shared__ SpxLogEntry tab[128];
  __shared__ unsigned long long acc;
  if (threadIdx.x < 128) reinterpret_cast<uint4*>(tab)[threadIdx.x] = reinterpret_cast<const uint4*>(spx_log_table_dev)[threadIdx.x];
  if (threadIdx.x == 0) acc = 0;
  __syncthreads();
  const unsigned b = first_block + blockIdx.x;
  unsigned long long sum = 0;
  for (unsigned i = threadIdx.x; i < (1u << 20); i += 256) {
    const float x = __uint_as_float((b << 20) | i);
    sum += (unsigned long long)__double_as_longlong(spx_log_v2_f32(x, tab));
  }
  atomicAdd(&acc, sum);
  __syncthreads();
  if (threadIdx.x == 0) sums[b] = acc;
#endif
}
extern "C" int spx_debug_log_check(unsigned first_block, unsigned end_block, unsigned long long* sums) {
#ifdef SPX_LOG_V1
  (void)first_block; (void)end_block; (void)sums;
  return -3;
#else
  if (first_block < 8) first_block = 8;
  if (end_block > 2040) end_block = 2040;
  if (!sums || first_block >= end_block) return -1;
  unsigned long long* d = nullptr;
  if (hipMalloc(&d, 2040 * sizeof(unsigned long long)) != hipSuccess) return -1;
  bool ok = hipMemset(d, 0, 2040 * sizeof(unsigned long long)) == hipSuccess;
  if (ok) hipLaunchKernelGGL(spx_log_check_kernel, dim3(end_block - first_block), dim3(256), 0, nullptr, first_block, d);
  ok = ok && hipDeviceSynchronize() == hipSuccess && hipMemcpy(sums, d, 2040 * sizeof(unsigned long long), hipMemcpyDeviceToHost) == hipSuccess;
  (void)hipFree(d);
  return ok ? 0 : -1;
#endif
}

SpxKernelChoice spx_analysis_select(int tile_frames, int ctw) {
#define AN_K(TFV, WV) SpxKernelChoice{"spx_analysis_kernel", reinterpret_cast<const void*>(spx_analysis_kernel<TFV, WV>), SPX_BLOCK, 2, {TFV, WV}}
  static_assert(std::is_same<decltype(spx_analysis_kernel<SPX_TF_TINY, 0>), SpxAnalysisArgs>::value, "SpxAnalysisArgs is the kernel's argument list");
  if (tile_frames == SPX_TF_TINY) return AN_K(SPX_TF_TINY, 0);
  if (tile_frames == SPX_TF_SMALL)
    return ctw == 240 ? AN_K(SPX_TF_SMALL, 240) : ctw == 330 ? AN_K(SPX_TF_SMALL, 330) : ctw == 720 ? AN_K(SPX_TF_SMALL, 720)
         : ctw == 661 ? AN_K(SPX_TF_SMALL, 661) : ctw == 120 ? AN_K(SPX_TF_SMALL, 120) : AN_K(SPX_TF_SMALL, 0);
  return ctw == 240 ? AN_K(SPX_TF, 240) : ctw == 330 ? AN_K(SPX_TF, 330) : ctw == 120 ? AN_K(SPX_TF, 120) : ctw == 360 ? AN_K(SPX_TF, 360)
       : ctw == 180 ? AN_K(SPX_TF, 180) : ctw == 480 ? AN_K(SPX_TF, 480) : AN_K(SPX_TF, 0);
#undef AN_K
}
int spx_analysis_vgprs(const SpxPlanDev& P, int* scratch_bytes) {
  return spx_kernel_vgprs(spx_analysis_select(P.tile_frames, plan_ct_window(P)).fn, scratch_bytes);
}

void spx_launch_analysis(const SpxPlanDev& P, const SpxStreamDev* streams, int n_streams, int n_tiles,
                         const int16_t* in, SpxFrameRec* rec, SpxTapsDev taps, const int* tile_order, int* tile_flags,
                         hipStream_t st) {
  if (n_tiles <= 0) return;
  SpxLaunch<SpxAnalysisArgs>::go(spx_analysis_select(P.tile_frames, plan_ct_window(P)), n_tiles, spx_analysis_lds_bytes(P), st, P, streams,
                                 n_streams, in, rec, taps, tile_order, tile_flags, nullptr, 0);
}

void spx_launch_analysis_frames(const SpxPlanDev& P, const SpxStreamDev* streams, int n_tiles, const float* frames,
                                bool preemph, SpxFrameRec* rec, SpxTapsDev taps, hipStream_t st) {
  if (n_tiles <= 0) return;
  SpxPlanDev Q = P;
  if (Q.tile_frames != SPX_TF_SMALL && Q.tile_frames != SPX_TF_TINY) Q.tile_frames = SPX_TF;
  SpxLaunch<SpxAnalysisArgs>::go(spx_analysis_select(Q.tile_frames, 0), n_tiles, analysis_lds_bytes(Q, false), st, Q, streams, 1, nullptr, rec,
                                 taps, nullptr, nullptr, frames, preemph ? 1 : 2);
}
```

### speedy_amd/csrc/spx_diag.hip

```cpp
#include "spx_engine.h"

extern "C" {
static const char* kernel_names(spx_plan_t plan, int n_streams, int max_channels, int speedup_only, bool lean);
const char* spx_batch_kernel_names(spx_plan_t plan, int n_streams, int max_channels, int speedup_only) {
  return kernel_names(plan, n_streams, max_channels, speedup_only, false);
}
const char* spx_batch_kernel_names_lean(spx_plan_t plan, int n_streams, int max_channels, int speedup_only) {
  return kernel_names(plan, n_streams, max_channels, speedup_only, true);
}
static const char* kernel_names(spx_plan_t plan, int n_streams, int max_channels, int speedup_only, bool lean) {
  static thread_local char buf[256];
  const SpxPlanDev& d = plan->dev;
  const SpxWalkConfig c = spx_walk_config(d, {.n_streams = n_streams, .max_channels = max_channels, .speedup_only = speedup_only != 0,
                                              .any_speed = speedup_only == 0, .lean = lean});
  size_t at = 0;
  auto put = [&](const SpxKernelChoice& k) {
    at += snprintf(buf + at, sizeof(buf) - at, "%s<", k.name);
    for (int i = 0; i < k.n_targs; i++) at += snprintf(buf + at, sizeof(buf) - at, i ? ", %d" : "%d", k.targs[i]);
    at += snprintf(buf + at, sizeof(buf) - at, ">");
  };
  put(spx_analysis_select(d.tile_frames, spx_analysis_ct_window(d)));
  at += snprintf(buf + at, sizeof(buf) - at, ";spx_tension_kernel;");
  put(c.kernel);
  return buf;
}

int spx_debug_last_call_concurrent(void) { return g_last_concurrent.load(std::memory_order_relaxed); }
int spx_debug_kernel_vgprs(int which) {
  if (which == 0) return spx_tension_vgprs();
  const int rate = (which == 2 || which == 4) ? 22050 : 16000;
  const SpxPlanDev* P = spx_internal_shared_plan(rate, 0);
  if (!P) return -1;
  switch (which) {
    case 1: return spx_walk_vgprs(*P, {.n_streams = 256, .max_channels = 1, .speedup_only = true}, nullptr);
    case 2: return spx_walk_vgprs(*P, {.n_streams = 256, .max_channels = 1, .speedup_only = true, .lean = true}, nullptr);
    case 3: case 4: return spx_analysis_vgprs(*P);
    case 5: return spx_walk_vgprs(*P, {.n_streams = 256, .max_channels = 2, .speedup_only = true}, nullptr);
    default: return -1;
  }
}

int spx_debug_walk_info(int sample_rate, int channels, int n_streams, int speedup_only, int short_jobs, int lean, int* out) {
  const SpxPlanDev* P = spx_internal_shared_plan(sample_rate, 0);
  if (!P || !out) return -1;
  const SpxWalkConfig c = spx_walk_config(*P, {.n_streams = n_streams, .max_channels = channels, .speedup_only = speedup_only != 0,
                                               .any_speed = speedup_only == 0, .short_jobs = short_jobs != 0, .lean = lean != 0});
  int scratch = -1;
  out[0] = spx_kernel_vgprs(c.kernel.fn, &scratch);
  out[1] = scratch;
  out[2] = (int)c.lds;
  out[3] = c.fast_kernel ? 16 * c.nwm + c.nwc : 0;
  out[4] = c.waves;
  return 0;
}
int spx_debug_analysis_info(int sample_rate, int* out) {
  const SpxPlanDev* P = spx_internal_shared_plan(sample_rate, 0);
  if (!P || !out) return -1;
  int scratch = -1;
  out[0] = spx_analysis_vgprs(*P, &scratch);
  out[1] = scratch;
  out[2] = (int)spx_analysis_lds_bytes(*P);
  out[3] = P->dft_waves;
  return 0;
}

void spx_set_timing(int enabled) { g_timing = enabled != 0; }
void spx_set_concurrent(int on) { g_concurrent = on != 0; }
void spx_set_pipeline_chunks(int chunks) { g_chunks_set = true; g_chunks = chunks < 1 ? 1 : (chunks > SPX_MAX_CHUNKS ? SPX_MAX_CHUNKS : chunks); }
static double g_last_tension_ms = 0.0, g_last_rate_ms = 0.0;
double spx_timing_last_tension_ms(void) { return g_last_tension_ms; }
double spx_timing_last_rate_ms(void) { return g_last_rate_ms; }
int spx_timing_collect(double* sum_ms_analyze, double* sum_ms_walk, int* n_calls) {
  std::lock_guard<std::mutex> g(g_tmu);
  double a = 0, w = 0, t = 0, r = 0;
  for (auto& ev : g_ev_pending) {
    HIPCHK(hipEventSynchronize(ev.b));
    float ms = 0;
    HIPCHK(hipEventElapsedTime(&ms, ev.a, ev.b));
    if (ev.kind == 0) a += ms; else if (ev.kind == 1) w += ms; else if (ev.kind == 3) r += ms; else t += ms;
    g_ev_free.push_back(ev.a);
    g_ev_free.push_back(ev.b);
  }
  g_ev_pending.clear();
  g_last_tension_ms = t;
  g_last_rate_ms = r;
  if (sum_ms_analyze) *sum_ms_analyze = a;
  if (sum_ms_walk) *sum_ms_walk = w;
  if (n_calls) *n_calls = g_calls_pending;
  g_calls_pending = 0;
  return 0;
}

void* spx_device_alloc(size_t bytes) {
  void* p = nullptr;
  if (hipMalloc(&p, bytes ? bytes : 1) != hipSuccess) { fail(-2, "spx_device_alloc failed"); return nullptr; }
  return p;
}
void spx_device_free(void* p) { if (p) (void)hipFree(p); }
int spx_copy_to_device(void* dst, const void* src, size_t bytes, void* hs) {
  HIPCHK(hipMemcpyAsync(dst, src, bytes, hipMemcpyHostToDevice, static_cast<hipStream_t>(hs)));
  return 0;
}
}

__global__ void __launch_bounds__(256)
spx_pack_offsets_kernel(const int64_t* __restrict__ n_out, const int* __restrict__ channels,
                        const int64_t* __restrict__ caps, int n, int64_t* __restrict__ offsets) {
  __shared__ int64_t sh[256];
  __shared__ int64_t carry;
  const int t = threadIdx.x;
  if (t == 0) carry = 0;
  __syncthreads();
  for (int i0 = 0; i0 < n; i0 += 256) {
    const int i = i0 + t;
    int64_t v = 0;
    if (i < n) {
      const int64_t k = n_out[i];
      int64_t f = (k == INT64_MIN ? 0 : (k > 0 ? k : -k));
      if (f > caps[i]) f = caps[i];
      v = f * channels[i];
    }
    sh[t] = v;
    __syncthreads();
    for (int d = 1; d < 256; d <<= 1) {
      const int64_t add = (t >= d) ? sh[t - d] : 0;
      __syncthreads();
      sh[t] += add;
      __syncthreads();
    }
    const int64_t base = carry;
    if (i < n) offsets[i] = base + sh[t] - v;
    __syncthreads();
    if (t == 255) carry = base + sh[255];
    __syncthreads();
  }
  if (t == 0) offsets[n] = carry;
}
__global__ void __launch_bounds__(256)
spx_pack_copy_kernel(const int16_t* __restrict__ out, const int64_t* __restrict__ out_offs,
                     const int64_t* __restrict__ offsets, int16_t* __restrict__ packed) {
  const int i = blockIdx.x;
  const int16_t* src = out + out_offs[i];
  int16_t* dst = packed + offsets[i];
  const int64_t cnt = offsets[i + 1] - offsets[i];
// ... 54 lines not shown
```

### speedy_amd/csrc/spx_engine.hip

```cpp
#include "spx_engine.h"

__attribute__((constructor(101))) static void spx_default_hw_queues() {
  if (getenv("SPX_KEEP_HW_QUEUES") || getenv("GPU_MAX_HW_QUEUES")) return;
  setenv("GPU_MAX_HW_QUEUES", "8", 0);
  if (getenv("SPX_DEBUG_MODE")) fprintf(stderr, "[spx] GPU_MAX_HW_QUEUES was unset: set to 8 at load time (SPX_KEEP_HW_QUEUES=1 leaves the environment alone)\n");
}

thread_local std::string g_spx_err;

std::atomic<bool> g_timing{false};
std::atomic<int> g_last_concurrent{0};
std::atomic<int> g_concurrent{1};
std::atomic<bool> g_chunks_set{false};
std::atomic<int> g_chunks{1};
std::mutex g_tmu;
std::vector<EvPair> g_ev_pending;
std::vector<hipEvent_t> g_ev_free;
int g_calls_pending = 0;

SpxDevGuard g_guard[64];

int spx_kernel_vgprs(const void* fn, int* scratch_bytes) {
  static std::mutex mu;
  static std::map<const void*, std::pair<int, int>> cache;
// ... 78 lines not shown
    const int64_t Ttot = nonlinear ? frames_for(d, j.n_in) : 0;
    int64_t Tprev = 0;
    for (int c = 0; c < nch; c++) {
      int64_t n_c = j.n_in;
      if (c < nch - 1) n_c = (j.n_in * (c + 1) / nch) / d.B * d.B;
      SpxStreamDev& s = v[(size_t)c * n + i];
      s.in_off = j.in_off; s.n_in = n_c; s.out_off = j.out_off; s.out_cap = j.out_cap;
      s.channels = j.channels; s.speed = j.speed; s.nonlinear = j.nonlinear; s.feedback = j.feedback;
      const int64_t T = nonlinear ? frames_for(d, n_c) : 0;
      s.n_frames = (int32_t)T;
      s.frame_begin = (int32_t)Tprev;
      s.flags = (c == 0 ? SPX_F_INIT : 0) | (c == nch - 1 ? SPX_F_FLUSH : 0);
      if (rc) {
        s.out_off = rc->walk_out_off[i]; s.out_cap = rc->walk_out_cap[i];
        if (rc->no_trunc[i]) s.flags |= SPX_F_NO_TRUNC;
      }
      s.frame_off = fo;
      s.first_tile = tiles_per_chunk[c];
      tiles_per_chunk[c] += (int)((T - Tprev + TF - 1) / TF);
      Tprev = T;
    }
    fo += Ttot;
  }
}

static SpxTapsDev taps_of(const spx_taps* t) {
  SpxTapsDev d = {nullptr, nullptr, nullptr, nullptr, nullptr};
  if (t) { d.tension = t->tension; d.speed = t->speed; d.features = t->features;
           d.spectrogram = t->spectrogram; d.normalized = t->normalized; }
  return d;
}

__global__ void spx_gate_kernel(const int* started, int n_walk, unsigned max_spins) {
  if (threadIdx.x == 0) {
    for (unsigned i = 0; i < max_spins; i++) {
      if (__hip_atomic_load(started, __ATOMIC_RELAXED, __HIP_MEMORY_SCOPE_AGENT) >= n_walk) break;
      __builtin_amdgcn_s_sleep(8);
    }
  }
}
void spx_launch_gate(const int* started, int n_walk, unsigned max_spins, hipStream_t st) {
  hipLaunchKernelGGL(spx_gate_kernel, dim3(1), dim3(64), 0, st, started, n_walk, max_spins);
}
__global__ void __launch_bounds__(256)
spx_stage_kernel(const unsigned* __restrict__ src, unsigned* __restrict__ dst_a, unsigned n_a, unsigned* __restrict__ dst_b,
                 unsigned n_b, unsigned* __restrict__ zero_a, unsigned nz_a, unsigned* __restrict__ zero_b, unsigned nz_b,
                 const int* gate_started, int gate_n, unsigned gate_spins) {
  const unsigned stride = gridDim.x * blockDim.x, t0 = blockIdx.x * blockDim.x + threadIdx.x;
  for (unsigned i = t0; i < n_a; i += stride) dst_a[i] = src[i];
  for (unsigned i = t0; i < n_b; i += stride) dst_b[i] = src[n_a + i];
  for (unsigned i = t0; i < nz_a; i += stride) zero_a[i] = 0u;
  for (unsigned i = t0; i < nz_b; i += stride) zero_b[i] = 0u;
  if (gate_started != nullptr && t0 == 0) {
    for (unsigned i = 0; i < gate_spins; i++) {
      if (__hip_atomic_load(gate_started, __ATOMIC_RELAXED, __HIP_MEMORY_SCOPE_AGENT) >= gate_n) break;
      __builtin_amdgcn_s_sleep(8);
    }
  }
}
extern "C" {

static hipEvent_t take_event() {
  std::lock_guard<std::mutex> g(g_tmu);
  if (!g_ev_free.empty()) { hipEvent_t e = g_ev_free.back(); g_ev_free.pop_back(); return e; }
  hipEvent_t e;
  (void)hipEventCreate(&e);
  return e;
}

}
int dev_side_streams(int dev, hipStream_t* side, hipStream_t* side2) {
  static std::mutex mu;
  static hipStream_t s1[64], s2[64];
  const int d = (dev >= 0 && dev < 64) ? dev : 0;
  std::lock_guard<std::mutex> g(mu);
  if (!s1[d]) {
    if (hipStreamCreateWithFlags(&s1[d], hipStreamNonBlocking) != hipSuccess) { s1[d] = nullptr; return -1; }
    if (hipStreamCreateWithFlags(&s2[d], hipStreamNonBlocking) != hipSuccess) { (void)hipStreamDestroy(s1[d]); s1[d] = nullptr; s2[d] = nullptr; return -1; }
  }
  *side = s1[d]; *side2 = s2[d];
  return 0;
}

int walk_stream_count() { return 2; }
int dev_walk_streams(int dev, hipStream_t* w, int n) {
  static std::mutex mu;
  static hipStream_t s3[64][SPX_MAX_WALK_STREAMS];
  hipStream_t side = nullptr, side2 = nullptr;
  if (dev_side_streams(dev, &side, &side2)) return -1;
  const int d = (dev >= 0 && dev < 64) ? dev : 0;
  std::lock_guard<std::mutex> g(mu);
  w[0] = side2;
  for (int i = 1; i < n && i < SPX_MAX_WALK_STREAMS; i++) {
    if (!s3[d][i] && hipStreamCreateWithFlags(&s3[d][i], hipStreamNonBlocking) != hipSuccess) { s3[d][i] = nullptr; return -1; }
    w[i] = s3[d][i];
  }
  return 0;
}

int ring_note(spx_plan* plan, hipStream_t st) {
  const int cur = plan->ahead_calls & 1;
  if (!plan->ev_call[cur]) HIPCHK(hipEventCreateWithFlags(&plan->ev_call[cur], hipEventDisableTiming));
  HIPCHK(hipEventRecord(plan->ev_call[cur], st));
  plan->ev_call_valid[cur] = true;
  plan->ev_call_st[cur] = st;
  return 0;
}
int ring_wait(spx_plan* plan, hipStream_t sa, const void* ws, hipStream_t st, bool* waited_prev) {
  const int c = plan->ahead_calls % SPX_RING;
  if (waited_prev) *waited_prev = false;
  for (int back = SPX_RING; back >= 1; back--) {
    const int j = (c + SPX_RING - back) % SPX_RING;
    if (!plan->ev_walk_valid[j]) continue;
    if (back > SPX_RING / 2 || plan->ring_ws[j] == ws || plan->ring_st[j] != st) {
      HIPCHK(hipStreamWaitEvent(sa, plan->ev_walk[j], 0));
      if (back == 1 && waited_prev) *waited_prev = true;
    }
  }
  return 0;
}
bool ring_previous_in_flight(spx_plan* plan) {
  const int j = (plan->ahead_calls + SPX_RING - 1) % SPX_RING;
  const bool f = plan->ev_walk_valid[j] && hipEventQuery(plan->ev_walk[j]) == hipErrorNotReady;
  (void)hipGetLastError();
  return f;
}
int ring_record(spx_plan* plan, hipStream_t on, void* ws, hipStream_t st, const void* out, const void* n_out, bool detached) {
  const int c = plan->ahead_calls % SPX_RING;
  if (!plan->ev_walk[c]) HIPCHK(hipEventCreateWithFlags(&plan->ev_walk[c], hipEventDisableTiming));
  HIPCHK(hipEventRecord(plan->ev_walk[c], on));
  if (on != st && !detached) HIPCHK(hipStreamWaitEvent(st, plan->ev_walk[c], 0));
  plan->ev_walk_valid[c] = true;
  plan->ring_ws[c] = ws;
  plan->ring_st[c] = st;
  plan->ahead_last_out = out;
  plan->ahead_last_nout = n_out;
  plan->ahead_calls++;
  return 0;
}

SpxModeEnv mode_env() {
  SpxModeEnv e;
  e.concurrent_enabled = g_concurrent.load() != 0;
  e.chunks_set = g_chunks_set.load();
  e.chunks = g_chunks.load();
  return e;
}
bool device_ours_cb(void* ctx) { return device_is_ours(*static_cast<int*>(ctx)); }
SpxSpeedClass speed_class(const spx_stream_job* jobs, int n) {
  SpxSpeedClass c = {1, true, true};
  for (int i = 0; i < n; i++) {
    if (jobs[i].channels > c.maxC) c.maxC = jobs[i].channels;
    const bool ok = jobs[i].speed > 0.0f && jobs[i].speed < SPX_FAST_MAX_SPEED && jobs[i].nonlinear >= 0.0f && jobs[i].nonlinear <= 1.0f;
    if (!(ok && jobs[i].speed > 1.0f)) c.speedup_only = false;
    if (!ok) c.any_speed = false;
  }
  if (c.speedup_only) c.any_speed = false;
  return c;
}
SpxModeWalk mode_walk(const SpxPlanDev& d, const SpxWalkAsk& ask) {
  const SpxWalkConfig c = spx_walk_config(d, ask);
  SpxModeWalk w;
  w.lds = c.lds; w.waves = c.waves; w.fast_kernel = c.fast_kernel; w.nwc = c.nwc;
  w.vgprs = spx_kernel_vgprs(c.kernel.fn);
  return w;
}
static const SpxModeResources& mode_resources(spx_plan* plan, int n, int maxC, bool speedup_only, bool any_speed = false, bool short_window = false) {
  const long long key = ((long long)n << 16) ^ ((long long)maxC << 3) ^ (short_window ? 4 : 0) ^ (any_speed ? 2 : 0) ^ (speedup_only ? 1 : 0);
  auto it = plan->res_cache.find(key);
  if (it != plan->res_cache.end()) return it->second;
  const SpxPlanDev& d = plan->dev;
  SpxModeResources R;
  memset(&R, 0, sizeof(R));
  R.cu_count = plan->cu_count;
  R.lds_per_cu = plan->lds_per_cu;
  R.walk = mode_walk(d, {.n_streams = n, .max_channels = maxC, .speedup_only = speedup_only, .any_speed = any_speed, .short_window = short_window});
  R.walk_lean = R.walk;
  if (maxC == 1 && n <= plan->cu_count && R.walk.fast_kernel && R.walk.nwc > 0) {
    R.walk_lean = mode_walk(d, {.n_streams = n, .max_channels = maxC, .speedup_only = speedup_only, .any_speed = any_speed, .lean = true});
    R.lean_valid = true;
  }
  R.tension_lds = spx_tension_lds_bytes();
  R.tension_vgprs = spx_tension_vgprs();
  R.tile_default = d.tile_frames;
  R.tile_big = spx_analysis_tile_frames();
  R.tile_small = spx_analysis_small_tile_frames();
  SpxPlanDev d8 = d;
  d8.tile_frames = R.tile_small;
  R.an_lds_default = spx_analysis_lds_bytes(d);
  R.an_vgprs_default = spx_analysis_vgprs(d);
  R.an_lds_small = spx_analysis_lds_bytes(d8);
  R.an_vgprs_small = spx_analysis_vgprs(d8);
  if (plan->res_cache.size() > 64) plan->res_cache.clear();
  return plan->res_cache.emplace(key, R).first->second;
}
extern "C" int spx_debug_mode_resources(int sample_rate, int channels, int n_streams, int speedup_only, long long* out) {
  spx_plan* plan = shared_plan_full(sample_rate, 0);
  if (!plan || !out || n_streams < 1) return -1;
  std::lock_guard<std::mutex> g(plan->mu);
  const SpxModeResources& R = mode_resources(plan, n_streams, channels < 1 ? 1 : channels, speedup_only != 0, speedup_only == 0);
  const long long v[22] = {R.cu_count, (long long)R.lds_per_cu, (long long)R.walk.lds, R.walk.waves, R.walk.vgprs, R.walk.fast_kernel, R.walk.nwc,
                           (long long)R.walk_lean.lds, R.walk_lean.waves, R.walk_lean.vgprs, R.walk_lean.fast_kernel, R.walk_lean.nwc, R.lean_valid,
                           (long long)R.tension_lds, R.tension_vgprs, R.tile_default, R.tile_big, R.tile_small, (long long)R.an_lds_default,
                           (long long)R.an_lds_small, R.an_vgprs_default, R.an_vgprs_small};
  for (int i = 0; i < 22; i++) out[i] = v[i];
  return 0;
}

static int stage_tables(spx_plan* plan, const std::vector<SpxStreamDev>& sv, const std::vector<int>& order, SpxStreamDev* dstreams,
                        int* d_order, int* d_flags, unsigned n_flags, int* d_ready, unsigned n_ready, hipStream_t on, hipEvent_t* done,
                        const int* gate_started = nullptr, int gate_n = 0, unsigned gate_spins = 0) {
  const size_t b_sv = sizeof(SpxStreamDev) * sv.size(), b_or = sizeof(int) * order.size();
  SpxStage& G = plan->stage[plan->stage_next];
  plan->stage_next ^= 1;
  if (G.done) HIPCHK(hipEventSynchronize(G.done));
  else HIPCHK(hipEventCreateWithFlags(&G.done, hipEventDisableTiming));
  if (G.cap < b_sv + b_or) {
    if (G.p) (void)hipHostFree(G.p);
    G.p = nullptr; G.cap = 0;
    const size_t cap = (b_sv + b_or) * 2 + 4096;
    HIPCHK(hipHostMalloc(&G.p, cap, hipHostMallocDefault));
    G.cap = cap;
  }
  unsigned char* hp = static_cast<unsigned char*>(G.p);
  memcpy(hp, sv.data(), b_sv);
  if (b_or) memcpy(hp + b_sv, order.data(), b_or);
  hipLaunchKernelGGL(spx_stage_kernel, dim3(64), dim3(256), 0, on, reinterpret_cast<const unsigned*>(hp),
                     reinterpret_cast<unsigned*>(dstreams), (unsigned)(b_sv / 4), reinterpret_cast<unsigned*>(d_order), (unsigned)(b_or / 4),
                     reinterpret_cast<unsigned*>(d_flags), n_flags, reinterpret_cast<unsigned*>(d_ready), n_ready, gate_started, gate_n, gate_spins);
  HIPCHK(hipEventRecord(G.done, on));
  *done = G.done;
  return 0;
}

struct SpxTimed {
  hipEvent_t a = nullptr, b = nullptr;
  hipStream_t s = nullptr;
  int kind = 0;
  SpxTimed(bool on, int kind_, hipStream_t s_) : s(s_), kind(kind_) {
    if (on) { a = take_event(); b = take_event(); (void)hipEventRecord(a, s); }
  }
  ~SpxTimed() {
    if (!a) return;
    (void)hipEventRecord(b, s);
    std::lock_guard<std::mutex> g(g_tmu);
    g_ev_pending.push_back({a, b, kind});
  }
};

int run_impl(spx_plan_t plan, const spx_stream_job* jobs, int n, const int16_t* in, int16_t* out,
             int64_t* n_out, void* ws, size_t ws_bytes, const spx_taps* taps, void* hs, bool do_a,
             bool do_w, const SpxCallOpts& opt) {
  const SpxForce* force = opt.force;
  if (spx_check_jobs(plan, jobs, n, opt.rate != nullptr, force && force->no_exclusive)) return -1;
  SpxRange range_(do_a && do_w ? "spx_batch_run" : (do_a ? "spx_batch_analyze" : "spx_batch_walk"));
  SpxPlanDev d = plan->dev;
  Layout L = layout_for(d, jobs, n);
  if (ws_bytes < L.total || !ws) return fail(-1, "spx_batch: workspace too small");
  const SpxSpeedClass SC = speed_class(jobs, n);
  const int maxC = SC.maxC;
  const bool speedup_only = SC.speedup_only && !opt.rate, any_speed = SC.any_speed && !opt.rate;
  std::lock_guard<std::mutex> plan_lock(plan->mu);
  if (!opt.split_part) plan->split_of.erase(ws);
  const bool short_window_res = opt.force && opt.force->no_exclusive;
  const SpxModeResources& R = mode_resources(plan, n, maxC, speedup_only, any_speed, short_window_res);
  hipStream_t st = static_cast<hipStream_t>(hs);
  SpxModeShape S;
  S.n = n; S.max_channels = maxC; S.do_a = do_a; S.do_w = do_w; S.has_frames = L.total_frames > 0;
  S.forced = force != nullptr;
  S.force_concurrent = force && force->concurrent != 0;
  S.force_ahead = force && force->ahead_sa != nullptr;
  S.force_total_streams = force ? force->total_streams : n;
  S.ahead_req = opt.ahead_req; S.overlap_req = opt.overlap_req;
  SpxModeEnv E = mode_env();
// ... 43 lines not shown
  SpxStreamDev* dstreams = reinterpret_cast<SpxStreamDev*>(w + L.off_streams);
  SpxStreamState* states = reinterpret_cast<SpxStreamState*>(w + L.off_states);
  SpxFrameRec* rec = reinterpret_cast<SpxFrameRec*>(w + L.off_rec);
  float* scratch = reinterpret_cast<float*>(w + L.off_scratch);
  int* d_order = reinterpret_cast<int*>(w + L.off_order);
  int* d_flags = reinterpret_cast<int*>(w + L.off_flags);
  int* d_ready = reinterpret_cast<int*>(w + L.off_ready);
  SpxTapsDev td = taps_of(taps);
  const bool timed = g_timing.load() && do_a && do_w;
  if (do_a && do_w) g_last_concurrent.store(concurrent ? 1 : (ahead ? 2 : 0), std::memory_order_relaxed);
  static const bool dbg_mode = getenv("SPX_DEBUG_MODE") != nullptr;
  if (dbg_mode)
    fprintf(stderr, "[spx mode] rate %d n %d maxC %d: co_resident %d doubtful %d lean %d want_concurrent %d chunks %d tiles %d -> %s%s\n",
            d.rate, n, maxC, (int)M.co_resident, (int)M.doubtful, (int)M.launch_lean, (int)M.want_concurrent, nch, tiles[0],
            concurrent ? "concurrent" : (ahead ? (M.seq_ahead ? "ahead (kernels in sequence)" : "ahead") : (chunk_ahead ? "sequence, producers ahead" : "sequence")),
            M.walk2 ? ", walk kernels overlapping" : "");
  hipStream_t stw = st;
  const bool detached = opt.detached && M.walk2 && !force;
  if (do_w && !force && !detached && ring_note(plan, st)) return -2;
  if (do_w && !force && detached) { plan->ev_call_valid[plan->ahead_calls & 1] = false; plan->ev_call_st[plan->ahead_calls & 1] = nullptr; }
  if (M.walk2) {
    hipStream_t wst[SPX_MAX_WALK_STREAMS];
    const int nws = walk_stream_count();
    if (dev_walk_streams(plan->device, wst, nws)) return fail(-1, "spx_batch: no walk streams");
    const int cur = plan->ahead_calls & 1;
    stw = wst[plan->ahead_calls % nws];
    const bool same_out = !opt.sub && (out == plan->ahead_last_out || n_out == plan->ahead_last_nout);
    const bool foreign_prev = !plan->ev_call_valid[cur ^ 1] || plan->ev_call_st[cur ^ 1] != st;
    if (detached) { }
    else if (same_out || (foreign_prev && plan->ahead_calls > 0)) HIPCHK(hipStreamWaitEvent(stw, plan->ev_call[cur], 0));
    else if (plan->ev_call_valid[cur ^ 1]) HIPCHK(hipStreamWaitEvent(stw, plan->ev_call[cur ^ 1], 0));
  }
  hipStream_t sa = st;
  if (nch > 1 || concurrent || ahead) {
    if (!plan->side) {
      if (dev_side_streams(plan->device, &plan->side, &plan->side2)) return fail(-1, "spx_batch: no side streams");
      HIPCHK(hipEventCreateWithFlags(&plan->ev_start, hipEventDisableTiming));
      HIPCHK(hipEventCreateWithFlags(&plan->ev_tension, hipEventDisableTiming));
      for (auto& e : plan->ev_chunk) HIPCHK(hipEventCreateWithFlags(&e, hipEventDisableTiming));
    }
    sa = M.ahead_forced ? force->ahead_sa : plan->side;
  }
  std::vector<int> order;
  if (concurrent) {
    order.reserve((size_t)tiles[0]);
    std::vector<int> cnt(n);
    int maxT = 0;
    for (int i = 0; i < n; i++) {
      cnt[i] = (i + 1 < n ? sv[i + 1].first_tile : tiles[0]) - sv[i].first_tile;
      if (cnt[i] > maxT) maxT = cnt[i];
    }
    for (int t = 0; t < maxT; t++)
      for (int i = 0; i < n; i++)
        if (t < cnt[i]) order.push_back(sv[i].first_tile + t);
  }
  bool waited_prev = false;
  if ((ahead || chunk_ahead) && !force) {
    if (ring_wait(plan, sa, ws, st, &waited_prev)) return -2;
    if (opt.in_ready) HIPCHK(hipStreamWaitEvent(sa, static_cast<hipEvent_t>(opt.in_ready), 0));
  }
  if (!ahead && !chunk_ahead && opt.in_ready) HIPCHK(hipStreamWaitEvent(st, static_cast<hipEvent_t>(opt.in_ready), 0));
  hipEvent_t staged_ev = nullptr;
  const bool ahead_gate = ahead && !force && plan->ahead_started != nullptr && plan->ahead_n > 0 && !waited_prev &&
                          ring_previous_in_flight(plan);
  const int rc = stage_tables(plan, sv, opt.rate ? opt.rate->table : order, dstreams, opt.rate ? reinterpret_cast<int*>(opt.rate->d_table) : d_order, d_flags, concurrent ? (unsigned)tiles[0] : 0u, d_ready,
                    (concurrent || ahead) ? (unsigned)n + 1u : 0u, (ahead || chunk_ahead) ? sa : st, &staged_ev,
                    ahead_gate ? plan->ahead_started : nullptr, plan->ahead_n, 8000u);
  if (rc) return rc;
  if (M.trial_slot >= 0) {
    hipEvent_t& e0 = TR.ev[2 * M.trial_slot];
    if (!e0) HIPCHK(hipEventCreate(&e0));
    HIPCHK(hipEventRecord(e0, st));
  }
  if (sa != st && !ahead && !chunk_ahead) {
    HIPCHK(hipStreamWaitEvent(sa, staged_ev, 0));
    if (concurrent) HIPCHK(hipStreamWaitEvent(plan->side2, staged_ev, 0));
  }
  for (int c = 0; c < nch; c++) {
    SpxStreamDev* dj = dstreams + (size_t)c * n;
    if (concurrent && do_w && idle_start)
      hipLaunchKernelGGL(spx_gate_kernel, dim3(1), dim3(64), 0, sa, d_ready + n, n, 1200u);
    if (do_a && tiles[c] > 0) {
      SpxTimed tm(timed, 0, sa);
      spx_launch_analysis(d, dj, n, tiles[c], in, rec, td, concurrent ? d_order : nullptr, concurrent ? d_flags : nullptr, sa);
    }
    if (force && force->after_analysis && c == nch - 1) HIPCHK(hipEventRecord(force->after_analysis, sa));
    if (sa != st) HIPCHK(hipEventRecord(plan->ev_chunk[c], sa));
    if (sa != st && !concurrent && !ahead) HIPCHK(hipStreamWaitEvent(st, plan->ev_chunk[c], 0));
    if (do_w) {
      hipStream_t stn = concurrent ? plan->side2 : (ahead ? sa : st);
      {
        SpxTimed tm(timed, 2, stn);
        spx_launch_tension(d, dj, n, states, rec, scratch, td, concurrent ? d_flags : nullptr, (concurrent || ahead) ? d_ready : nullptr, stn);
      }
      if (concurrent || ahead) HIPCHK(hipEventRecord(plan->ev_tension, stn));
      if (ahead) HIPCHK(hipStreamWaitEvent(stw, plan->ev_tension, 0));
      {
        SpxTimed tm(timed, 1, stw);
        const SpxWalkAsk ask = {.n_streams = n, .max_channels = maxC, .speedup_only = speedup_only, .any_speed = any_speed, .lean = M.launch_lean,
                                .short_window = short_window_res || (!force && M.walk2 && !M.launch_lean && maxC > 1)};
        spx_launch_walk(d, ask, dj, in, out, opt.rate ? opt.rate->d_tsm_n : n_out, states, scratch, (concurrent || ahead) ? d_ready : nullptr,
                        (M.exclusive_cu && !(force && force->no_exclusive)) ? R.lds_per_cu / 2 + 1024 : 0, stw);
      }
      if (opt.rate && c == nch - 1) {
        SpxTimed tm(timed, 3, stw);
        spx_launch_rate_batch(opt.rate->d_table, n, opt.rate->max_blocks, states, opt.rate->d_tsm_n, opt.rate->tsm_base, out, n_out, stw);
      }
      if (M.ahead_forced && force->started_out) *force->started_out = d_ready + n;
      if (c == nch - 1 && !force) {
        if (ring_record(plan, stw, ws, st, out, n_out, detached)) return -2;
        plan->ahead_started = (concurrent || ahead) ? d_ready + n : nullptr;
        plan->ahead_n = n;
        plan->mixed_started.clear();
      }
    }
    if (concurrent) {
      HIPCHK(hipStreamWaitEvent(st, plan->ev_chunk[c], 0));
      HIPCHK(hipStreamWaitEvent(st, plan->ev_tension, 0));
    }
  }
  if (concurrent && !force) {
    if (!guard.last) HIPCHK(hipEventCreateWithFlags(&guard.last, hipEventDisableTiming));
    HIPCHK(hipEventRecord(guard.last, st));
    guard.last_stream = st;
    guard.valid = true;
  }
  if (M.trial_slot >= 0) {
    hipEvent_t& e1 = TR.ev[2 * M.trial_slot + 1];
    if (!e1) HIPCHK(hipEventCreate(&e1));
    HIPCHK(hipEventRecord(e1, st));
  }
  if (opt.done_event && do_w) HIPCHK(hipEventRecord(static_cast<hipEvent_t>(opt.done_event), detached ? stw : st));
  if (timed) { std::lock_guard<std::mutex> g(g_tmu); g_calls_pending++; }
  HIPCHK(hipGetLastError());
  return 0;
}

#define SPX_SPLIT_LIMIT 4
struct SplitPlan { int k; std::vector<int> first; std::vector<size_t> ws_off, ws_bytes; size_t total; };
static SplitPlan split_geometry(const spx_plan* plan, const spx_stream_job* jobs, int n, int max_mult) {
  SplitPlan P;
  P.k = 1; P.total = 0;
  const int cu = plan->cu_count > 0 ? plan->cu_count : 1;
  if (max_mult > SPX_SPLIT_LIMIT) max_mult = SPX_SPLIT_LIMIT;
  if (n <= cu || n > max_mult * cu) return P;
  P.k = (n + cu - 1) / cu;
  size_t o = 0;
  for (int i = 0; i < P.k; i++) {
    const int a = (int)((long long)n * i / P.k), b = (int)((long long)n * (i + 1) / P.k);
    P.first.push_back(a);
    const size_t bytes = layout_for(plan->dev, jobs + a, b - a).total;
    P.ws_off.push_back(o); P.ws_bytes.push_back(bytes);
    o += (bytes + 255) & ~(size_t)255;
  }
  P.first.push_back(n);
  P.total = o;
  return P;
}
static int run_split(spx_plan_t plan, const spx_stream_job* jobs, int n, const int16_t* in, int16_t* out, int64_t* n_out, void* ws,
                     size_t ws_bytes, const spx_taps* taps, void* hs, const SpxCallOpts& opt) {
  if (!plan || !jobs || n <= 0) return fail(-1, "spx_batch: bad arguments");
  SplitPlan P = split_geometry(plan, jobs, n, opt.ahead_req && opt.overlap_req ? 2 : 1);
  if (P.k > 1 && (g_chunks_set.load() || ws_bytes < P.total)) P.k = 1;
  if (P.k > 1) {
    const SpxSpeedClass SC = speed_class(jobs, n);
    const int maxC = SC.maxC;
    std::lock_guard<std::mutex> plan_lock(plan->mu);
// ... 224 lines not shown
```

### speedy_amd/csrc/spx_internal.h

```cpp
#pragma once
#include <hip/hip_runtime.h>
#include <stdint.h>

#include <stdlib.h>
#include <type_traits>


#define SPX_FAST_MAX_SPEED 1.0e18f

#define SPX_MAX_STAGES 16
#define SPX_WAVE 64
#define SPX_BLOCK 256
#define SPX_FEATURE_COUNT 15

struct SpxPlanDev {
  int rate;
  int B;
  int W;
  int N;
  int F;
  int Pp;
  int nstages;
  int radix[SPX_MAX_STAGES];
  int minPeriod, maxPeriod, maxRequired, skip;
  int tile_frames;
  int dft_waves;
  float alpha;
  float one_minus_alpha;
  const double* tw;
  const double* tw2;
  const float* window;
  const float* taperF;
  const float* taperP;
  int rader;
  int nstagesM;
  int radixM[SPX_MAX_STAGES];
  const double* twM;
  const double* bfft;
  const int* perm;
  const int* iperm;
  const int* qlog;
};

#define SPX_F_INIT 1
#define SPX_F_FLUSH 2
#define SPX_F_TENSION_RANGE 4
#define SPX_F_NO_SPEED 8
#define SPX_F_NO_TRUNC 16
#define SPX_F_SPEED_SET 32
#define SPX_F_KEEP_SPEED 64
#define SPX_F_HANDED_IN 128
struct SpxStreamDev {
  int64_t in_off, n_in, out_off, out_cap;
  int64_t frame_off;
  int32_t n_frames;
  int32_t frame_begin;
  int32_t channels;
  int32_t flags;
  float speed, nonlinear, feedback;
  int32_t first_tile;
  int64_t tsm_shift;
  int32_t tension_skip;
  int32_t unit_time0;
  int32_t tension_to;
  int32_t handed_in;
  int32_t ring_bufs;
  int32_t pad4;
};

struct SpxWalkState {
  int64_t base;
  int64_t out_n;
  int64_t avail;
  int remaining;
  int prevPeriod, prevMinDiff;
  int overflow;
  int prevPeriod_toggle;
  int steps;
};
struct SpxStreamState {
  SpxWalkState w;
  float lp;
  float lpf;
  float cur_dur;
  float des_dur;
  float curSpeed;
  int handed;
  int flush_remaining;
  int flush_out_mark;
  int tension_first;
  int pad2_;
};

#define SPX_RATE_MAX_CHANNELS 16
struct SpxRateState {
  int64_t tsm_seen;
  int64_t final_n;
  int32_t old_pos, new_pos;
  int32_t has_left;
  int32_t overflow;
  int16_t left[SPX_RATE_MAX_CHANNELS];
};
void spx_launch_rate(SpxRateState* rs, const SpxStreamState* st, const int64_t* tsm_n, const int16_t* tsm, int16_t* fin,
                     int64_t fin_cap, int channels, int old_rate, int new_rate, float rate, int bypass, int flush,
                     hipStream_t hs);

struct SpxRateJob {
  int64_t tsm_off;
  int64_t tsm_cap;
  int64_t fin_off;
  int64_t fin_cap;
  int32_t channels;
  int32_t old_rate, new_rate;
  int32_t bypass;
  float rate;
  int32_t n_blocks;
  int64_t pad_;
};
int spx_rate_batch_blocks(int64_t frames, int channels);
void spx_launch_rate_batch(const SpxRateJob* jobs, int n_streams, int max_blocks, const SpxStreamState* states, const int64_t* tsm_n,
                           const int16_t* tsm_base, int16_t* fin_base, int64_t* n_out, hipStream_t hs);

struct SpxFrameRec {
  float energy;
  float lsd;
};

struct SpxTapsDev {
  float* tension;
  float* speed;
  float* features;
  float* spectrogram;
  float* normalized;
};

void spx_launch_analysis(const SpxPlanDev& P, const SpxStreamDev* streams, int n_streams, int n_tiles,
                         const int16_t* in, SpxFrameRec* rec, SpxTapsDev taps, const int* tile_order, int* tile_flags,
                         hipStream_t st);
void spx_launch_analysis_frames(const SpxPlanDev& P, const SpxStreamDev* streams, int n_tiles, const float* frames,
                                bool preemph, SpxFrameRec* rec, SpxTapsDev taps, hipStream_t st);
void spx_launch_tension(const SpxPlanDev& P, const SpxStreamDev* streams, int n_streams, SpxStreamState* states,
                        const SpxFrameRec* rec, float* scratch, SpxTapsDev taps, const int* tile_flags, int* speed_ready,
                        hipStream_t st);
struct SpxKernelChoice {
  const char* name;
  const void* fn;
  int block;
  int n_targs;
  int targs[5];
};
using SpxAnalysisArgs = void(SpxPlanDev, const SpxStreamDev*, int, const int16_t*, SpxFrameRec*, SpxTapsDev, const int*, int*, const float*, int);
using SpxWalkArgs = void(SpxPlanDev, const SpxStreamDev*, const int16_t*, int16_t*, int64_t*, SpxStreamState*, const float*, int, const int*);
using SpxWalkFastArgs = void(SpxPlanDev, const SpxStreamDev*, const int16_t*, int16_t*, int64_t*, SpxStreamState*, const float*, const int*, int);
template <typename F> struct SpxLaunch;
template <typename... P> struct SpxLaunch<void(P...)> {
  static void go(const SpxKernelChoice& k, int grid, size_t lds, hipStream_t st, P... p) {
    void* args[] = {&p...};
    (void)hipLaunchKernel(k.fn, dim3(grid), dim3(k.block), args, lds, st);
  }
};
struct SpxWalkAsk {
  int n_streams = 0;
  int max_channels = 1;
  bool speedup_only = false;
  bool any_speed = false;
  bool short_jobs = false;
  bool lean = false;
  bool short_window = false;
};
void spx_launch_walk(const SpxPlanDev& P, const SpxWalkAsk& ask, const SpxStreamDev* streams, const int16_t* in, int16_t* out,
                     int64_t* n_out, SpxStreamState* states, const float* scratch, const int* speed_ready, size_t lds_min,
                     hipStream_t st);
size_t spx_analysis_lds_bytes(const SpxPlanDev& P);
int spx_analysis_ct_window(const SpxPlanDev& P);
void spx_host_dft(int n, const int* radix, int nstages, const double* tw, const double* in, double* out);
size_t spx_walk_lds_bytes(const SpxPlanDev& P, int max_channels, bool speedup_only);
struct SpxWalkConfig {
  int mode;
  bool fast_kernel;
  int nw;
  int nwm, nwc, wcap;
  int waves;
  size_t lds;
  bool slow;
  SpxKernelChoice kernel;
};
SpxWalkConfig spx_walk_config(const SpxPlanDev& P, const SpxWalkAsk& ask);
SpxKernelChoice spx_walk_select(int nw, int mode);
size_t spx_walk_fast_lds_bytes(const SpxPlanDev& P, int wcap);
bool spx_walk_fast_supports(const SpxPlanDev& P, int nwm);
SpxKernelChoice spx_walk_fast_select(const SpxPlanDev& P, int nwm, int nwc, int wcap, int max_channels, bool slow);
SpxKernelChoice spx_analysis_select(int tile_frames, int ct_window);
#define SPX_NOUT_LOST_PRODUCER INT64_MIN
size_t spx_tension_lds_bytes();
int spx_kernel_vgprs(const void* fn, int* scratch_bytes = nullptr);
int spx_tension_vgprs();
int spx_analysis_vgprs(const SpxPlanDev& P, int* scratch_bytes = nullptr);
int spx_walk_vgprs(const SpxPlanDev& P, const SpxWalkAsk& ask, int* scratch_bytes);
void spx_launch_speed_from_tension(SpxStreamState* state, float tension, float Rg, float feedback, float* speed_out,
                                   hipStream_t st);
int spx_analysis_tile_frames();
int spx_analysis_small_tile_frames();
int spx_analysis_tiny_tile_frames();
int spx_analysis_prefers_small_tile(const SpxPlanDev& P);

struct spx_plan;
int64_t spx_internal_out_bound(const SpxPlanDev& P, int64_t n_in, float speed, bool nonlinear);
const SpxPlanDev* spx_internal_shared_plan(int sample_rate, int match_matlab);
bool spx_internal_analysis_fits(const SpxPlanDev& d);
int64_t spx_internal_frames_for(const SpxPlanDev& d, int64_t n_in);
```

### speedy_amd/csrc/spx_mixed.hip

```cpp
#include "spx_engine.h"

extern "C" {
__global__ void spx_scatter_nout_kernel(const int64_t* __restrict__ src, const int* __restrict__ idx, int n, int64_t* __restrict__ dst) {
  const int i = blockIdx.x * blockDim.x + threadIdx.x;
  if (i < n) dst[idx[i]] = src[i];
}
struct MixedLayout { std::vector<size_t> ws_off, ws_bytes; size_t off_nout, off_idx, total; };
static MixedLayout mixed_layout(const spx_plan_t* plans, int n_plans, const std::vector<std::vector<spx_stream_job>>& gj, int n) {
  MixedLayout M;
  size_t o = 0;
  for (int g = 0; g < n_plans; g++) {
    const size_t b = gj[g].empty() ? 0 : layout_for(plans[g]->dev, gj[g].data(), (int)gj[g].size()).total;
    M.ws_off.push_back(o); M.ws_bytes.push_back(b);
    o += (b + 255) & ~(size_t)255;
  }
  M.off_nout = o; o += ((sizeof(int64_t) * (size_t)n + 255) & ~(size_t)255);
  M.off_idx = o;  o += ((sizeof(int) * (size_t)n + 255) & ~(size_t)255);
  M.total = o;
  return M;
}
static int mixed_groups(int n_plans, const spx_stream_job* jobs, const int* plan_index, int n,
                        std::vector<std::vector<spx_stream_job>>& gj, std::vector<std::vector<int>>& gi) {
  gj.assign(n_plans, {}); gi.assign(n_plans, {});
  for (int i = 0; i < n; i++) {
    const int g = plan_index ? plan_index[i] : 0;
    if (g < 0 || g >= n_plans) return fail(-1, "spx_batch_run_mixed: plan_index out of range");
    gj[g].push_back(jobs[i]); gi[g].push_back(i);
  }
  return 0;
}
size_t spx_batch_workspace_bytes_mixed(const spx_plan_t* plans, int n_plans, const spx_stream_job* jobs, const int* plan_index,
                                       int n_streams) {
  std::vector<std::vector<spx_stream_job>> gj;
  std::vector<std::vector<int>> gi;
  if (!plans || n_plans < 1 || !jobs || n_streams < 1 || mixed_groups(n_plans, jobs, plan_index, n_streams, gj, gi)) return 0;
  return mixed_layout(plans, n_plans, gj, n_streams).total;
}
static int mixed_impl(const spx_plan_t* plans, int n_plans, const spx_stream_job* jobs, const int* plan_index, int n,
                      const int16_t* in, int16_t* out, int64_t* n_out, void* ws, size_t ws_bytes, const spx_taps* taps,
                      void* hs, bool ahead_req, void* in_ready = nullptr, void* done_event = nullptr, bool detached = false);
}
int spx_internal_run_mixed(const spx_plan_t* plans, int n_plans, const spx_stream_job* jobs, const int* plan_index, int n, const int16_t* in,
                           int16_t* out, int64_t* n_out, void* ws, size_t ws_bytes, void* hs, bool ahead, void* in_ready,
                           void* done_event, bool detached) {
  return mixed_impl(plans, n_plans, jobs, plan_index, n, in, out, n_out, ws, ws_bytes, nullptr, hs, ahead, in_ready, done_event, detached);
}
extern "C" {
int spx_batch_run_mixed(const spx_plan_t* plans, int n_plans, const spx_stream_job* jobs, const int* plan_index, int n,
                        const int16_t* in, int16_t* out, int64_t* n_out, void* ws, size_t ws_bytes, void* hs) {
  return mixed_impl(plans, n_plans, jobs, plan_index, n, in, out, n_out, ws, ws_bytes, nullptr, hs, false);
}
int spx_batch_run_mixed_taps(const spx_plan_t* plans, int n_plans, const spx_stream_job* jobs, const int* plan_index, int n,
                             const int16_t* in, int16_t* out, int64_t* n_out, void* ws, size_t ws_bytes, const spx_taps* taps,
                             void* hs) {
  return mixed_impl(plans, n_plans, jobs, plan_index, n, in, out, n_out, ws, ws_bytes, taps, hs, false);
}
int spx_batch_run_mixed_ahead(const spx_plan_t* plans, int n_plans, const spx_stream_job* jobs, const int* plan_index, int n,
                              const int16_t* in, int16_t* out, int64_t* n_out, void* ws, size_t ws_bytes, void* hs) {
  return mixed_impl(plans, n_plans, jobs, plan_index, n, in, out, n_out, ws, ws_bytes, nullptr, hs, true);
}
static int mixed_impl(const spx_plan_t* plans, int n_plans, const spx_stream_job* jobs, const int* plan_index, int n,
                      const int16_t* in, int16_t* out, int64_t* n_out, void* ws, size_t ws_bytes, const spx_taps* taps,
                      void* hs, bool ahead_req, void* in_ready, void* done_event, bool detached_req) {
  if (!plans || n_plans < 1 || n_plans > 8 || !jobs || n <= 0) return fail(-1, "spx_batch_run_mixed: bad arguments");
  SpxRange range_("spx_batch_run_mixed");
  std::vector<std::vector<spx_stream_job>> gj;
  std::vector<std::vector<int>> gi;
  int rc = mixed_groups(n_plans, jobs, plan_index, n, gj, gi);
  if (rc) return rc;
  for (int g = 0; g < n_plans; g++)
    if (!gj[g].empty() && spx_check_jobs(plans[g], gj[g].data(), (int)gj[g].size())) return -1;
  const MixedLayout M = mixed_layout(plans, n_plans, gj, n);
  if (!ws || ws_bytes < M.total) return fail(-1, "spx_batch_run_mixed: workspace too small");
  hipStream_t st = static_cast<hipStream_t>(hs);
  spx_plan* lead = plans[0];
  for (int g = 0; g < n_plans; g++) if (plans[g]->device != lead->device) return fail(-1, "spx_batch_run_mixed: plans of different devices");
  std::vector<SpxModeGroup> G;
  for (int g = 0; g < n_plans; g++) {
    if (gj[g].empty()) continue;
    const SpxPlanDev& d = plans[g]->dev;
    const SpxSpeedClass SC = speed_class(gj[g].data(), (int)gj[g].size());
    const int maxC = SC.maxC;
    bool any_nl = false;
    for (const auto& j : gj[g]) any_nl = any_nl || j.nonlinear != 0.0f;
    SpxModeGroup mg;
    mg.n = (int)gj[g].size();
    mg.walk = mode_walk(d, {.n_streams = mg.n, .max_channels = maxC, .speedup_only = SC.speedup_only, .any_speed = SC.any_speed});
    mg.any_nonlinear = any_nl;
    mg.an_lds = spx_analysis_lds_bytes(d);
    mg.an_vgprs = spx_analysis_vgprs(d);
    G.push_back(mg);
  }
  const int groups = (int)G.size();
  SpxModeRuntime T;
  memset(&T, 0, sizeof(T));
  T.device_ours = device_ours_cb;
  T.device_ctx = &lead->device;
  const SpxModeEnv E = mode_env();
  SpxMixedMode MM = spx_choose_mixed_mode(G.data(), groups, n, lead->cu_count, lead->lds_per_cu, spx_tension_lds_bytes(), spx_tension_vgprs(),
                                          E, ahead_req, T);
  SpxDevGuard& guard = g_guard[(lead->device >= 0 && lead->device < 64) ? lead->device : 0];
  std::unique_lock<std::mutex> guard_lock(guard.mu, std::defer_lock);
  SpxForce force = {0, false, n, nullptr, nullptr, nullptr, false};
  if (MM.concurrent) {
    guard_lock.lock();
    const hipError_t q = guard.valid ? hipEventQuery(guard.last) : hipSuccess;
    (void)hipGetLastError();
    force.idle_start = (q == hipSuccess);
    if (guard.valid && guard.last_stream != st && q == hipErrorNotReady) {
      T.guard_busy = true;
      MM = spx_choose_mixed_mode(G.data(), groups, n, lead->cu_count, lead->lds_per_cu, spx_tension_lds_bytes(), spx_tension_vgprs(), E,
                                 ahead_req, T);
      guard_lock.unlock();
    }
  }
  const bool concurrent = MM.concurrent;
  const bool ahead = MM.ahead;
  force.concurrent = concurrent ? 1 : 0;
  const bool walk2 = spx_mixed_walk2(MM, detached_req, taps != nullptr);
  static_assert(SPX_MAX_WALK_STREAMS >= 4, "two pairs of walk streams taking turns");
  hipStream_t wst[SPX_MAX_WALK_STREAMS] = {nullptr};
  if (walk2 && dev_walk_streams(lead->device, wst, 4)) return fail(-1, "spx_batch_run_mixed: no walk streams");
  force.no_exclusive = walk2;
  std::lock_guard<std::mutex> lead_lock(lead->mix_mu);
  {
    std::lock_guard<std::mutex> ring_lock(lead->mu);
    if (ring_note(lead, st)) return -2;
  }
  if (!lead->ev_fork) HIPCHK(hipEventCreateWithFlags(&lead->ev_fork, hipEventDisableTiming));
  if (in_ready && !ahead) HIPCHK(hipStreamWaitEvent(st, static_cast<hipEvent_t>(in_ready), 0));
  HIPCHK(hipEventRecord(lead->ev_fork, st));
  unsigned char* w = static_cast<unsigned char*>(ws);
  int64_t* d_nout = reinterpret_cast<int64_t*>(w + M.off_nout);
  int* d_idx = reinterpret_cast<int*>(w + M.off_idx);
  std::vector<int> order;
  order.reserve((size_t)n);
  for (int g = 0; g < n_plans; g++) order.insert(order.end(), gi[g].begin(), gi[g].end());
  auto upload_idx = [&](hipStream_t on) -> int {
    SpxStage& G = lead->mix_stage[lead->mix_next];
    lead->mix_next ^= 1;
    if (G.done) HIPCHK(hipEventSynchronize(G.done));
    else HIPCHK(hipEventCreateWithFlags(&G.done, hipEventDisableTiming));
    if (G.cap < sizeof(int) * (size_t)n) {
      if (G.p) (void)hipHostFree(G.p);
      G.p = nullptr; G.cap = 0;
      HIPCHK(hipHostMalloc(&G.p, sizeof(int) * (size_t)n * 2 + 1024, hipHostMallocDefault));
      G.cap = sizeof(int) * (size_t)n * 2 + 1024;
    }
    memcpy(G.p, order.data(), sizeof(int) * (size_t)n);
    HIPCHK(hipMemcpyAsync(d_idx, G.p, sizeof(int) * (size_t)n, hipMemcpyHostToDevice, on));
    HIPCHK(hipEventRecord(G.done, on));
    return 0;
  };
  if (!ahead && upload_idx(st)) return -2;
  std::vector<size_t> gpos(n_plans, 0);
  { size_t pos = 0; for (int g = 0; g < n_plans; g++) { gpos[g] = pos; pos += gj[g].size(); } }
  std::vector<spx_taps> gtaps(n_plans);
  if (taps) {
    size_t rows = 0, o_spec = 0, o_norm = 0;
    for (int g = 0; g < n_plans; g++) {
      spx_taps& t = gtaps[g];
      t.tension = taps->tension ? taps->tension + rows : nullptr;
      t.speed = taps->speed ? taps->speed + rows : nullptr;
      t.features = taps->features ? taps->features + rows * SPX_FEATURE_COUNT : nullptr;
      t.spectrogram = taps->spectrogram ? taps->spectrogram + o_spec : nullptr;
      t.normalized = taps->normalized ? taps->normalized + o_norm : nullptr;
      const size_t fr = gj[g].empty() ? 0 : (size_t)layout_for(plans[g]->dev, gj[g].data(), (int)gj[g].size()).total_frames;
      rows += fr; o_spec += fr * (size_t)plans[g]->dev.N; o_norm += fr * (size_t)plans[g]->dev.W;
    }
  }
  std::vector<int> ord;
  for (int g = 0; g < n_plans; g++) if (!gj[g].empty()) ord.push_back(g);
// ... 101 lines not shown
```

### speedy_amd/csrc/spx_mode.h

```cpp
#ifndef SPX_MODE_H_
#define SPX_MODE_H_
#include <stddef.h>

#define SPX_MODE_MAX_CHUNKS 16

struct SpxModeWalk {
  size_t lds;
  int waves;
  int vgprs;
  bool fast_kernel;
  int nwc;
};
struct SpxModeResources {
  int cu_count;
  size_t lds_per_cu;
  SpxModeWalk walk;
  SpxModeWalk walk_lean;
  bool lean_valid;
  size_t tension_lds;
  int tension_vgprs;
  int tile_default, tile_big, tile_small;
  size_t an_lds_default, an_lds_small;
  int an_vgprs_default, an_vgprs_small;
};
struct SpxModeShape {
  int n, max_channels;
  bool do_a, do_w;
  bool has_frames;
  bool forced;
  bool force_concurrent, force_ahead;
  int force_total_streams;
  bool ahead_req;
  bool overlap_req;
};
struct SpxModeEnv {
  bool concurrent_enabled;
  bool chunks_set;
  int chunks;
};
struct SpxModeTrial {
  long long key;
  int calls;
  int choice;
};
struct SpxModeRuntime {
  bool two_workspaces;
  bool guard_busy;
  bool trial_times_ready;
  float ms_seq, ms_con;
  long long trial_key;
  bool (*device_ours)(void*);
  void* device_ctx;
};
struct SpxMode {
  bool lean_walk;
  bool launch_lean;
  int tile_frames;
  bool co_resident, doubtful;
  int trial_slot;
  bool want_concurrent;
  bool concurrent;
  bool ahead, seq_ahead, ahead_forced;
  bool walk2;
  bool chunk_ahead;
  int nch;
  bool exclusive_cu;
  bool asked_device;
  SpxModeTrial trial_next;
};

static inline bool spx_mode_fits2(const SpxModeResources& R, const SpxModeWalk& w, size_t lds_usable) {
  return w.lds + R.tension_lds + 2 * R.an_lds_default <= lds_usable &&
         ((w.waves + 3) / 4) * w.vgprs + R.tension_vgprs + 2 * R.an_vgprs_default <= 512;
}

static inline SpxMode spx_mode_pass(const SpxModeShape& S, const SpxModeResources& R, const SpxModeEnv& E, const SpxModeRuntime& T,
                                    const SpxModeTrial& trial_in, bool lean_walk) {
  SpxMode M;
  M.lean_walk = lean_walk;
  M.asked_device = false;
  M.trial_next = trial_in;
  const SpxModeWalk& W = lean_walk ? R.walk_lean : R.walk;
  const bool both = S.do_a && S.do_w;
  const size_t lds_usable = R.lds_per_cu > 6144 ? R.lds_per_cu - 6144 : R.lds_per_cu;
  const size_t per_stream_lds = W.lds + R.tension_lds;
  const size_t per_stream_waves = (size_t)W.waves + 4;
  auto ours = [&]() { M.asked_device = true; return T.device_ours ? T.device_ours(T.device_ctx) : true; };
  int tile = R.tile_default;
  if (per_stream_lds + 2 * R.an_lds_default > lds_usable && both && R.tile_default == R.tile_big &&
      per_stream_lds + 2 * R.an_lds_small <= lds_usable)
    tile = R.tile_small;
  const size_t an_lds = tile == R.tile_default ? R.an_lds_default : R.an_lds_small;
  const int an_vgprs = tile == R.tile_default ? R.an_vgprs_default : R.an_vgprs_small;
  bool co_resident = false, doubtful = false;
  if (an_lds < R.lds_per_cu) {
    const size_t lds_closing = R.lds_per_cu - an_lds + 1;
    const size_t closed = ((size_t)S.n * per_stream_lds) / lds_closing + ((size_t)S.n * per_stream_waves) / 29;
    co_resident = closed < (size_t)R.cu_count && S.n <= R.cu_count;
    if (per_stream_lds + 2 * an_lds > lds_usable) co_resident = false;
    if (co_resident) {
      const int walk_regs = ((W.waves + 3) / 4) * W.vgprs;
      if (walk_regs + R.tension_vgprs + 2 * an_vgprs > 512) {
        if (walk_regs + R.tension_vgprs + an_vgprs > 512) co_resident = false;
        else doubtful = true;
      }
    }
  }
  M.doubtful = doubtful;
  int trial_slot = -1;
  if (co_resident && doubtful && both && E.concurrent_enabled && !S.forced) {
    SpxModeTrial& N = M.trial_next;
    if (N.key != T.trial_key) { N.key = T.trial_key; N.calls = 0; N.choice = -1; }
    if (N.choice < 0 && N.calls >= 3 && T.trial_times_ready) N.choice = T.ms_con < T.ms_seq ? 1 : 0;
    if (N.choice >= 0) co_resident = N.choice == 1;
    else if (N.calls == 0) { }
    else if (N.calls == 1) trial_slot = 1;
    else if (N.calls == 2) { trial_slot = 0; co_resident = false; }
    else co_resident = false;
    N.calls++;
  }
  M.co_resident = co_resident;
  M.trial_slot = trial_slot;
  bool want_concurrent = E.concurrent_enabled && co_resident && both;
  if (want_concurrent && !S.forced && !ours()) want_concurrent = false;
  if (S.forced) want_concurrent = S.force_concurrent && both;
  M.ahead_forced = S.forced && S.force_ahead && both;
  const bool chunks_free = !E.chunks_set || E.chunks == 1;
  bool seq_ahead = false;
  if (S.ahead_req && !want_concurrent && !S.forced && both && S.n <= R.cu_count && E.concurrent_enabled &&
      trial_slot < 0 && chunks_free && !lean_walk) {
    const size_t walk_lds = W.lds > R.lds_per_cu / 2 + 1024 ? W.lds : R.lds_per_cu / 2 + 1024;
    const int walk_regs = ((W.waves + 3) / 4) * W.vgprs;
    seq_ahead = walk_lds + R.tension_lds + R.an_lds_default <= lds_usable &&
                walk_regs + R.tension_vgprs + R.an_vgprs_default <= 512 && ours();
  }
  M.seq_ahead = seq_ahead;
  M.ahead = M.ahead_forced || seq_ahead ||
            (S.ahead_req && want_concurrent && !doubtful && !S.forced && trial_slot < 0 && chunks_free);
  if (!S.has_frames && !M.ahead_forced) { M.ahead = false; seq_ahead = false; M.seq_ahead = false; }
  if (M.ahead) want_concurrent = false;
  if (want_concurrent && !S.forced && T.guard_busy) want_concurrent = false;
  M.want_concurrent = want_concurrent;
  if (!want_concurrent && (!M.ahead || seq_ahead)) tile = R.tile_default;
  M.tile_frames = tile;
  int nch = both ? E.chunks : 1;
  if (both && !E.chunks_set && !want_concurrent && S.n > 2 * R.cu_count) nch = 2;
  if (M.ahead) nch = 1;
  if (nch < 1) nch = 1;
  if (nch > SPX_MODE_MAX_CHUNKS) nch = SPX_MODE_MAX_CHUNKS;
  M.nch = nch;
  M.concurrent = want_concurrent && nch == 1 && S.has_frames;
  M.walk2 = S.overlap_req && M.ahead && !S.forced && !seq_ahead;
  const int total = S.forced ? S.force_total_streams : S.n;
  M.exclusive_cu = !M.concurrent && (!M.ahead || M.ahead_forced || seq_ahead) && nch == 1 && total <= R.cu_count;
  M.launch_lean = lean_walk && (M.concurrent || M.ahead);
  M.chunk_ahead = S.ahead_req && !S.forced && both && !M.ahead && !want_concurrent && nch >= 2 && S.n > 2 * R.cu_count &&
                  E.concurrent_enabled && trial_slot < 0 && ours();
  return M;
}

static inline SpxMode spx_choose_mode(const SpxModeShape& S, const SpxModeResources& R, const SpxModeEnv& E, const SpxModeRuntime& T,
                                      const SpxModeTrial& trial_in) {
  const size_t lds_usable = R.lds_per_cu > 6144 ? R.lds_per_cu - 6144 : R.lds_per_cu;
  const bool lean_possible = S.do_a && S.do_w && S.max_channels == 1 && S.n <= R.cu_count && R.walk.fast_kernel && R.walk.nwc > 0 &&
                             !S.forced && R.lean_valid && R.walk_lean.fast_kernel && R.walk_lean.nwc == 0;
  const bool lean_fits = lean_possible && spx_mode_fits2(R, R.walk_lean, lds_usable);
  const bool need_lean = lean_fits && !spx_mode_fits2(R, R.walk, lds_usable);
  SpxMode M = spx_mode_pass(S, R, E, T, trial_in, need_lean);
  if (!need_lean && lean_fits && M.walk2 && S.overlap_req && !T.two_workspaces) {
    SpxMode L = spx_mode_pass(S, R, E, T, trial_in, true);
    L.asked_device = L.asked_device || M.asked_device;
    if (L.ahead && L.walk2) return L;
  }
  return M;
}

struct SpxModeGroup {
  int n;
  SpxModeWalk walk;
  bool any_nonlinear;
  size_t an_lds;
  int an_vgprs;
};
struct SpxMixedMode {
  bool concurrent;
  bool ahead;
  bool chain_analyses;
  bool asked_device;
};
static inline SpxMixedMode spx_choose_mixed_mode(const SpxModeGroup* G, int groups, int n_total, int cu_count, size_t lds_per_cu,
                                                 size_t tension_lds, int tension_vgprs, const SpxModeEnv& E, bool ahead_req,
                                                 const SpxModeRuntime& T) {
  SpxMixedMode M = {false, false, false, false};
  size_t cons_lds = 0, cons_waves = 0, max_ps_lds = 0, max_an_lds = 0;
  int max_walk_regs = 0, max_an_regs = 0;
  for (int g = 0; g < groups; g++) {
    const size_t ps = G[g].walk.lds + tension_lds;
    cons_lds += (size_t)G[g].n * ps;
    cons_waves += (size_t)G[g].n * (G[g].walk.waves + 4);
    if (ps > max_ps_lds) max_ps_lds = ps;
    if (G[g].any_nonlinear) {
      if (G[g].an_lds > max_an_lds) max_an_lds = G[g].an_lds;
      if (G[g].an_vgprs > max_an_regs) max_an_regs = G[g].an_vgprs;
    }
    const int wr = ((G[g].walk.waves + 3) / 4) * G[g].walk.vgprs;
    if (wr > max_walk_regs) max_walk_regs = wr;
  }
  auto ours = [&]() { M.asked_device = true; return T.device_ours ? T.device_ours(T.device_ctx) : true; };
  bool concurrent = false;
  if (max_an_lds > 0 && max_an_lds < lds_per_cu && n_total <= cu_count) {
    const size_t closed = cons_lds / (lds_per_cu - max_an_lds + 1) + cons_waves / 29;
    concurrent = closed < (size_t)cu_count;
    const size_t lds_usable = lds_per_cu > 6144 ? lds_per_cu - 6144 : lds_per_cu;
    if (max_ps_lds + 2 * max_an_lds > lds_usable) concurrent = false;
    if (max_walk_regs + tension_vgprs + 2 * max_an_regs > 512) concurrent = false;
  }
  if (!E.concurrent_enabled || groups == 0) concurrent = false;
  if (concurrent && !ours()) concurrent = false;
  if (concurrent && T.guard_busy) concurrent = false;
  M.ahead = ahead_req && !concurrent && E.concurrent_enabled && groups > 0 && n_total <= cu_count && ours();
  M.concurrent = concurrent;
  M.chain_analyses = !concurrent && groups > 1;
  return M;
}

static inline bool spx_mixed_walk2(const SpxMixedMode& M, bool detached, bool taps) {
  return M.ahead && !M.concurrent && detached && !taps;
}

#endif
```

### speedy_amd/csrc/spx_plan.hip

```cpp
#include "spx_engine.h"
#include "spx_twiddle.h"
#include "spx_twiddle_hashes.h"

int64_t spx_internal_out_bound(const SpxPlanDev& P, int64_t n_in, float speed, bool nonlinear) {
  const int64_t slack = 4 * (int64_t)P.maxRequired + 1024;
  if (speed >= 1.0f) return n_in + slack;
  double s = nonlinear ? 0.01 : (double)speed;
  if (s < 1e-4) s = 1e-4;
  return (int64_t)((double)(n_in + 2 * (int64_t)P.maxRequired) * (2.0 / s)) + slack;
}

void spx_internal_set_error(const char* msg) { g_spx_err = msg ? msg : ""; }
extern "C" {

const char* spx_last_error(void) { return g_spx_err.c_str(); }
void spx_debug_twiddle_entry(long k, long n, double* c, double* s) { spx_tw::sincos_2pi(k, n, c, s); }
unsigned long long spx_debug_twiddle_hash(long den, long count) {
  uint64_t h = 0xcbf29ce484222325ull;
  for (long t = 0; t < count; t++) {
    double e[2];
    spx_tw::entry(t, den, e);
    const unsigned char* b = reinterpret_cast<const unsigned char*>(e);
    for (int i = 0; i < 16; i++) { h ^= b[i]; h *= 0x100000001b3ull; }
  }
  return h;
}
int spx_abi_version(void) { return 1; }

static int factor_radices(int n, int* radix) {
  int ns = 0;
  while (n % 4 == 0) { radix[ns++] = 4; n /= 4; }
  while (n % 2 == 0) { radix[ns++] = 2; n /= 2; }
  while (n % 3 == 0) { radix[ns++] = 3; n /= 3; }
  while (n % 5 == 0) { radix[ns++] = 5; n /= 5; }
  for (int p = 7; n > 1; p += 2)
    while (n % p == 0) { radix[ns++] = p; n /= p; }
  return ns;
}

spx_plan_t spx_plan_create(int sample_rate, int match_matlab) {
  if (sample_rate < 1000 || sample_rate > 127999) {
    fail(-1, "spx_plan_create: unsupported sample rate");
    return nullptr;
  }
  spx_plan* p = new spx_plan();
  SpxPlanDev& d = p->dev;
  memset(&d, 0, sizeof(d));
  {
    hipDeviceProp_t prop;
    if (hipGetDevice(&p->device) == hipSuccess && hipGetDeviceProperties(&prop, p->device) == hipSuccess) {
      p->cu_count = prop.multiProcessorCount > 0 ? prop.multiProcessorCount : 1;
      p->lds_per_cu = prop.maxSharedMemoryPerMultiProcessor ? (size_t)prop.maxSharedMemoryPerMultiProcessor : 65536;
    }
  }
  d.rate = sample_rate;
  d.B = (int)(sample_rate / 100.0);
  d.W = (int)(1.5 * sample_rate / (float)100.0);
  d.N = 2 * d.W;
  d.F = match_matlab ? 8 : 12;
  d.Pp = match_matlab ? 12 : 8;
  d.nstages = (d.W > 1) ? factor_radices(d.W, d.radix) : 0;
  if (d.nstages > SPX_MAX_STAGES) {
    delete p;
    fail(-1, "spx_plan_create: too many DFT stages");
    return nullptr;
  }
  d.minPeriod = sample_rate / 400;
  d.maxPeriod = sample_rate / 65;
  d.maxRequired = 2 * d.maxPeriod;
  d.skip = sample_rate > 4000 ? sample_rate / 4000 : 1;
  d.alpha = (float)exp(-1.0 / (float)100.0);
  d.one_minus_alpha = 1 - d.alpha;

  const int W = d.W;
  const int M = W - 1;
  bool rader = W > 64;
  for (int q = 2; rader && (long)q * q <= W; q++) if (W % q == 0) rader = false;
  if (rader) {
    int m = M;
    for (int q = 2; q <= 13; q++) while (m % q == 0) m /= q;
    rader = (m == 1);
  }
  if (rader) {
    d.rader = 1;
    d.nstagesM = factor_radices(M, d.radixM);
  }
  d.dft_waves = 4;
  d.tile_frames = spx_analysis_tile_frames();
  const int cand[5][2] = {{spx_analysis_tile_frames(), 4}, {spx_analysis_small_tile_frames(), 4}, {spx_analysis_small_tile_frames(), 2},
                          {spx_analysis_tiny_tile_frames(), 2}, {spx_analysis_tiny_tile_frames(), 1}};
  for (int c = 0; c < 5; c++) {
    d.tile_frames = cand[c][0];
    d.dft_waves = cand[c][1];
    if (spx_analysis_lds_bytes(d) <= 160 * 1024) break;
  }
  if (spx_analysis_prefers_small_tile(d)) {
    d.tile_frames = spx_analysis_small_tile_frames();
    d.dft_waves = 4;
  }
  const size_t n_tw = 2 * (size_t)W, n_win = (size_t)W, n_tf = d.F + 1, n_tp = d.Pp + 1;
  const size_t n_rd = rader ? 2 * (size_t)M : 0;
  const size_t n_ri = rader ? (size_t)M : 0;
  const size_t n_ql = rader ? (size_t)W : 0;
  const size_t bytes = sizeof(double) * (2 * n_tw + 2 * n_rd) + sizeof(float) * (n_win + n_tf + n_tp + 8) +
                       sizeof(int) * (2 * n_ri + n_ql);
  std::vector<unsigned char> host(bytes, 0);
  double* tw = reinterpret_cast<double*>(host.data());
  double* tw2 = tw + n_tw;
  double* twM = tw2 + n_tw;
  double* bfft = twM + n_rd;
  float* win = reinterpret_cast<float*>(bfft + n_rd);
  float* tf = win + n_win;
  float* tp = tf + n_tf;
  int* perm = reinterpret_cast<int*>(tp + n_tp + 8);
  int* iperm = perm + n_ri;
  int* qlog = iperm + n_ri;
  for (int t = 0; t < W; t++) {
    spx_tw::entry(t, W, &tw[2 * t]);
    spx_tw::entry(t, 2L * W, &tw2[2 * t]);
    double c = 1.0, sn = 0.0;
    if (W > 1) spx_tw::sincos_2pi(t, W - 1, &c, &sn);
    win[t] = 0.54 - 0.46 * c;
  }
  if (rader) {
    for (int t = 0; t < M; t++) spx_tw::entry(t, M, &twM[2 * t]);
    int g = 2;
    for (; g < W; g++) {
      long v = 1;
      int k = 0;
      do { v = (v * g) % W; k++; } while (v != 1);
      if (k == M) break;
    }
    long v = 1;
    for (int k = 0; k < M; k++) { perm[k] = (int)v; v = (v * g) % W; }
    for (int q = 0; q < M; q++) iperm[q] = perm[(M - q) % M];
    for (int q = 0; q < M; q++) qlog[iperm[q]] = q;
    std::vector<double> b(2 * (size_t)M);
    for (int q = 0; q < M; q++) { b[2 * q] = tw[2 * iperm[q]]; b[2 * q + 1] = tw[2 * iperm[q] + 1]; }
    spx_host_dft(M, d.radixM, d.nstagesM, twM, b.data(), bfft);
  }
  {
    const struct { long den, count; const double* t; } built[3] = {{W, W, tw}, {2L * W, W, tw2}, {rader ? M : 0, rader ? M : 0, twM}};
    for (const auto& b : built)
      for (const auto& pin : spx_twiddle_pins)
        if (b.count > 0 && pin.den == b.den && pin.count == b.count && spx_tw::fnv1a(b.t, 16 * (size_t)b.count) != pin.hash) {
          delete p;
          fail(-1, "spx_plan_create: a twiddle table does not hash to its pinned value (spx_twiddle_hashes.h) -- host code built with fast-math or fp contraction?");
          return nullptr;
        }
  }
  for (int i = 0; i <= d.F; i++) tf[i] = (d.F - i) / (float)d.F;
  for (int i = 0; i <= d.Pp; i++) tp[i] = (d.Pp - i) / (float)d.Pp;
  {
    hipStream_t w[SPX_MAX_WALK_STREAMS];
    (void)dev_walk_streams(p->device, w, walk_stream_count());
    (void)hipGetLastError();
  }
  if (hipMalloc(&p->tables, bytes) != hipSuccess ||
      hipMemcpy(p->tables, host.data(), bytes, hipMemcpyHostToDevice) != hipSuccess) {
    fail(-2, "spx_plan_create: device allocation/copy failed (is a GPU visible?)");
    if (p->tables) (void)hipFree(p->tables);
    delete p;
    return nullptr;
  }
  unsigned char* base = static_cast<unsigned char*>(p->tables);
  d.tw = reinterpret_cast<const double*>(base);
  d.tw2 = d.tw + n_tw;
  d.twM = d.tw2 + n_tw;
  d.bfft = d.twM + n_rd;
  d.window = reinterpret_cast<const float*>(d.bfft + n_rd);
  d.taperF = d.window + n_win;
  d.taperP = d.taperF + n_tf;
  d.perm = reinterpret_cast<const int*>(d.taperP + n_tp + 8);
  d.iperm = d.perm + n_ri;
  d.qlog = d.iperm + n_ri;
  return p;
}

void spx_plan_destroy(spx_plan_t plan) {
  if (!plan) return;
  if (plan->side) (void)hipStreamSynchronize(plan->side);
  if (plan->side2) (void)hipStreamSynchronize(plan->side2);
  if (plan->mix) { (void)hipStreamSynchronize(plan->mix); (void)hipStreamDestroy(plan->mix); }
  if (plan->ev_join) (void)hipEventDestroy(plan->ev_join);
  if (plan->ev_an) (void)hipEventDestroy(plan->ev_an);
  if (plan->ev_fork) (void)hipEventDestroy(plan->ev_fork);
  for (auto& g : plan->mix_stage) {
    if (g.done) { (void)hipEventSynchronize(g.done); (void)hipEventDestroy(g.done); }
    if (g.p) (void)hipHostFree(g.p);
  }
  if (plan->ev_tension) (void)hipEventDestroy(plan->ev_tension);
  if (plan->ev_start) (void)hipEventDestroy(plan->ev_start);
  for (auto& e : plan->ev_chunk) if (e) (void)hipEventDestroy(e);
  for (auto& e : plan->trial.ev) if (e) (void)hipEventDestroy(e);
  for (auto& e : plan->ev_walk) if (e) { (void)hipEventSynchronize(e); (void)hipEventDestroy(e); }
  for (auto& e : plan->ev_call) if (e) (void)hipEventDestroy(e);
  for (auto& g : plan->stage) {
    if (g.done) { (void)hipEventSynchronize(g.done); (void)hipEventDestroy(g.done); }
    if (g.p) (void)hipHostFree(g.p);
  }
  if (plan->tables) (void)hipFree(plan->tables);
  delete plan;
}
int spx_plan_frame_step(spx_plan_t p) { return p->dev.B; }
int spx_plan_window_size(spx_plan_t p) { return p->dev.W; }
int spx_plan_fft_size(spx_plan_t p) { return p->dev.N; }
int spx_plan_future(spx_plan_t p) { return p->dev.F; }
int spx_plan_max_required(spx_plan_t p) { return p->dev.maxRequired; }

int64_t spx_plan_frames(spx_plan_t p, int64_t n_in) { return frames_for(p->dev, n_in); }

int64_t spx_plan_out_capacity_for(spx_plan_t p, int64_t n_in, float speed, float nonlinear) {
  return spx_internal_out_bound(p->dev, n_in, speed, nonlinear != 0.0f);
}
int64_t spx_plan_out_capacity(spx_plan_t p, int64_t n_in, float speed) {
  return spx_internal_out_bound(p->dev, n_in, speed, true);
}

}
bool spx_internal_analysis_fits(const SpxPlanDev& d) { return spx_analysis_lds_bytes(d) <= 160 * 1024; }

spx_plan* shared_plan_full(int sample_rate, int match_matlab) {
  static std::mutex mu;
  static std::map<std::pair<int, std::pair<int, int>>, spx_plan*> cache;
  std::lock_guard<std::mutex> g(mu);
  int dev = 0;
  (void)hipGetDevice(&dev);
  auto key = std::make_pair(dev, std::make_pair(sample_rate, match_matlab ? 1 : 0));
  auto it = cache.find(key);
  if (it != cache.end()) return it->second;
  spx_plan* p = spx_plan_create(sample_rate, match_matlab);
  if (!p) return nullptr;
  cache[key] = p;
  return p;
}
const SpxPlanDev* spx_internal_shared_plan(int sample_rate, int match_matlab) {
  spx_plan* p = shared_plan_full(sample_rate, match_matlab);
  return p ? &p->dev : nullptr;
}
int64_t spx_internal_frames_for(const SpxPlanDev& d, int64_t n_in) { return frames_for(d, n_in); }
```

Before: 45420.

## Add lean LDS layout and per-lane constant table for 240-point analysis kernel

For the W=240 analysis tile, adds a lean path that overlaps the magnitude rows with the DFT work area, keeps the last rows in registers, and reads mono samples straight from global memory, skipping the LDS staging buffer. Per-lane twiddle and window constants are precomputed on the host into a lane-major table, so each lane loads them as vector reads. Launch bounds rise to five blocks, and the mode selector can now pick the lean walk when that leaves room for more analysis waves. The aim is higher occupancy and fewer index and LDS costs, at the cost of more code complexity and possible register pressure.

```diff
diff --git a/include/speedy_hip.h b/include/speedy_hip.h
--- a/include/speedy_hip.h
+++ b/include/speedy_hip.h
@@ -122,6 +122,7 @@
 int spx_debug_kernel_vgprs(int which);
 int spx_debug_walk_info(int sample_rate, int channels, int n_streams, int speedup_only, int short_jobs, int lean, int* out5);
 int spx_debug_analysis_info(int sample_rate, int* out4);
+int spx_debug_lane_consts(int sample_rate, void* out, double* tw, double* tw2, float* win);
 int spx_debug_mode_resources(int sample_rate, int channels, int n_streams, int speedup_only, long long* out22);
 long long spx_debug_fdiv_check(unsigned seed, unsigned denominators, int exp_lo, int exp_hi);
 long long spx_debug_xfade_check(int n_lo, int n_hi);
diff --git a/speedy_amd/_lib.py b/speedy_amd/_lib.py
--- a/speedy_amd/_lib.py
+++ b/speedy_amd/_lib.py
@@ -86,6 +86,7 @@
     "spx_debug_log_check": (C.c_int, [C.c_uint, C.c_uint, C.POINTER(C.c_ulonglong)]),
     "spx_debug_walk_info": (C.c_int, [C.c_int, C.c_int, C.c_int, C.c_int, C.c_int, C.c_int, C.POINTER(C.c_int)]),
     "spx_debug_analysis_info": (C.c_int, [C.c_int, C.POINTER(C.c_int)]),
+    "spx_debug_lane_consts": (C.c_int, [C.c_int, C.c_void_p, C.POINTER(C.c_double), C.POINTER(C.c_double), c_float_p]),
     "spx_debug_mode_resources": (C.c_int, [C.c_int, C.c_int, C.c_int, C.c_int, C.POINTER(C.c_longlong)]),
     "spx_pipeline_create": (C.c_void_p, [C.c_void_p, C.POINTER(StreamJob), C.c_int, C.c_int, C.c_uint]),
     "spx_pipeline_create_mixed": (C.c_void_p, [C.POINTER(C.c_void_p), C.c_int, C.POINTER(StreamJob), C.POINTER(C.c_int), C.c_int, C.c_int, C.c_uint]),
diff --git a/speedy_amd/csrc/sonic2_api.hip b/speedy_amd/csrc/sonic2_api.hip
--- a/speedy_amd/csrc/sonic2_api.hip
+++ b/speedy_amd/csrc/sonic2_api.hip
@@ -383,7 +383,7 @@
     td.features = s->tFeatures.base() - fo * SPX_FEATURE_COUNT;
     td.spectrogram = s->tSpec.base() - fo * P.N; td.normalized = s->tNorm.base() - fo * P.W;
   }
-  if (J.tiles > 0) spx_launch_analysis(P, s->dJob, 1, J.tiles, s->dIn.p, s->dRec.p, td, nullptr, nullptr, s->hs);
+  if (J.tiles > 0) spx_launch_analysis(P, s->dJob, 1, J.tiles, s->dIn.p, s->dRec.p, td, nullptr, nullptr, C == 1, s->hs);
   if (J.nonlinear) spx_launch_tension(P, s->dJob, 1, s->dState, s->dRec.p, s->dScr.p, td, nullptr, nullptr, s->hs);
   spx_launch_walk(P, {.n_streams = 1, .max_channels = (int)C, .speedup_only = J.speedupKernel, .short_jobs = true}, dJobW, J.tsmIn->p,
                   s->dOut.p, s->dNOut, s->dState, s->dScr.p, nullptr, 0, s->hs);
diff --git a/speedy_amd/csrc/sonic2_pool.hip b/speedy_amd/csrc/sonic2_pool.hip
--- a/speedy_amd/csrc/sonic2_pool.hip
+++ b/speedy_amd/csrc/sonic2_pool.hip
@@ -493,7 +493,7 @@
   for (const Group& g : groups) {
     const SpxPlanDev& PL = *items[g.i0].s->plan;
     const int ng = (int)(g.i1 - g.i0);
-    if (g.tiles > 0) spx_launch_analysis(PL, dA + g.i0, ng, g.tiles, nullptr, P->aRec, no_taps, nullptr, nullptr, P->hs);
+    if (g.tiles > 0) spx_launch_analysis(PL, dA + g.i0, ng, g.tiles, nullptr, P->aRec, no_taps, nullptr, nullptr, false, P->hs);
     lap(1);
     bool any_nl = false;
     for (size_t i = g.i0; i < g.i1; i++) any_nl = any_nl || items[i].J.nonlinear;
diff --git a/speedy_amd/csrc/spx_analysis.hip b/speedy_amd/csrc/spx_analysis.hip
--- a/speedy_amd/csrc/spx_analysis.hip
+++ b/speedy_amd/csrc/spx_analysis.hip
@@ -81,14 +81,23 @@
 static __host__ __device__ inline size_t stage_samples(const SpxPlanDev& P, int tf) {
   return (size_t)(tf + 1) * P.B + (P.W - P.B) + 8;
 }
-static size_t analysis_lds_bytes(const SpxPlanDev& P, bool ct) {
+static __host__ __device__ constexpr bool an_lean_layout(int tf, int wct) { return tf == SPX_TF && wct == 240; }
+#define SPX_LT_FRONT_ROWS 13
+static __host__ __device__ constexpr size_t an_lt_front_bytes() { return (size_t)SPX_LT_FRONT_ROWS * spx_mag_stride(240) * sizeof(float); }
+static __host__ __device__ constexpr size_t an_lt_small_off() { return (size_t)(SPX_TF + 1 - SPX_LT_FRONT_ROWS) * spx_mag_stride(240) * sizeof(float); }
+static __host__ __device__ constexpr size_t an_lt_terms_off() { return (an_lt_small_off() + 3 * (SPX_TF + 1) * sizeof(float) + 15) & ~(size_t)15; }
+static_assert(SPX_TF + 1 - SPX_LT_FRONT_ROWS == 4, "one held row per wave");
+static_assert(an_lt_front_bytes() % 16 == 0 && an_lt_small_off() % 16 == 0, "16-byte rows, 16-byte work area");
+static size_t analysis_lds_bytes(const SpxPlanDev& P, int ctw, bool mono) {
   const int tf = P.tile_frames > 0 ? P.tile_frames : SPX_TF;
+  const bool ct = ctw != 0;
   size_t mags = (size_t)(tf + 1) * spx_mag_stride(P.W) * sizeof(float);
   size_t small = (size_t)3 * (tf + 1) * sizeof(float);
   size_t stage = (stage_samples(P, tf) * sizeof(short) + 15) & ~(size_t)15;
+  if (an_lean_layout(tf, ctw)) return an_lt_front_bytes() + work_bytes(P.W, tf, ct, P.dft_waves) + (mono ? 0 : stage);
   return work_bytes(P.W, tf, ct, P.dft_waves) + ((mags + 15) & ~(size_t)15) + ((small + 15) & ~(size_t)15) + stage;
 }
-size_t spx_analysis_lds_bytes(const SpxPlanDev& P) { return analysis_lds_bytes(P, plan_ct_window(P) != 0); }
+size_t spx_analysis_lds_bytes(const SpxPlanDev& P, bool mono) { return analysis_lds_bytes(P, plan_ct_window(P), mono); }
 int spx_analysis_ct_window(const SpxPlanDev& P) { return plan_ct_window(P); }
 
 __device__ __forceinline__ void wave_sync() {
@@ -408,14 +417,12 @@
 }
 
 #ifdef SPX_PREEMPH_V1
-#define SPX_WIN_SCALE 1.0f
 __device__ __forceinline__ float spx_preemph_win_f32(double md, double mpd, float w) {
   const float x = (float)(md / 32768.0), xp = (float)(mpd / 32768.0);
   const float y = (float)(1.0 * (double)x - 0.97 * (double)xp);
   return y * w;
 }
 #else
-#define SPX_WIN_SCALE 0x1p-15f
 __device__ __forceinline__ float spx_preemph_win_f32(double md, double mpd, float w15) {
   const float yy = (float)(md - 0.97 * mpd);
   return yy * w15;
@@ -437,7 +444,7 @@
 #define SPX_AN_W_BIG 2
 #endif
 template <int TF, int WCT>
-__global__ void __launch_bounds__(SPX_BLOCK, (WCT == 240 || WCT == 120 || WCT == 180) ? 4 : WCT == 330 ? SPX_AN_W_330 : (WCT == 661 || WCT == 720) ? SPX_AN_W_BIG : (WCT == 480 || WCT == 360) ? 2 : 1)
+__global__ void __launch_bounds__(SPX_BLOCK, an_lean_layout(TF, WCT) ? 5 : (WCT == 240 || WCT == 120 || WCT == 180) ? 4 : WCT == 330 ? SPX_AN_W_330 : (WCT == 661 || WCT == 720) ? SPX_AN_W_BIG : (WCT == 480 || WCT == 360) ? 2 : 1)
 spx_analysis_kernel(SpxPlanDev P, const SpxStreamDev* __restrict__ streams, int n_streams,
                     const int16_t* __restrict__ in_base, SpxFrameRec* __restrict__ rec, SpxTapsDev taps,
                     const int* __restrict__ tile_order, int* tile_flags, const float* __restrict__ frames,
@@ -459,19 +466,24 @@
   const int C = S.channels;
   const int16_t* __restrict__ in = in_base + S.in_off;
 
-  double* work = reinterpret_cast<double*>(lds);
+  constexpr bool LT = an_lean_layout(TF, WCT);
   const size_t wb = work_bytes(W, TF, WCT != 0, (WCT != 0) ? 4 : P.dft_waves);
-  float* mags = reinterpret_cast<float*>(lds + wb);
   const size_t mags_b = (((size_t)(TF + 1) * spx_mag_stride(W) * sizeof(float)) + 15) & ~(size_t)15;
-  float* fE = reinterpret_cast<float*>(lds + wb + mags_b);
+  const size_t small_b = (((size_t)3 * (TF + 1) * sizeof(float)) + 15) & ~(size_t)15;
+  double* work = reinterpret_cast<double*>(LT ? lds + an_lt_front_bytes() : lds);
+  float* mags = reinterpret_cast<float*>(LT ? lds : lds + wb);
+  float* fE = reinterpret_cast<float*>(LT ? lds + an_lt_front_bytes() + an_lt_small_off() : lds + wb + mags_b);
   float* fThr = fE + (TF + 1);
   float* fInv = fThr + (TF + 1);
   const int MS = spx_mag_stride(W);
-
-  const size_t small_b = (((size_t)3 * (TF + 1) * sizeof(float)) + 15) & ~(size_t)15;
+  unsigned char* const terms_base = reinterpret_cast<unsigned char*>(work) + (LT ? an_lt_terms_off() : 0);
+  static_assert(!LT || an_lt_terms_off() + (size_t)2 * SPX_TF * (spx_cb(SPX_TF) + 1) * sizeof(double) + SPX_LOG_LDS_BYTES <= (size_t)4 * 2 * 240 * sizeof(double),
+                "two blocks of log terms and the log table inside the work area (terms_bytes, work_bytes)");
+
   const double* ltw = P.tw;
   const double* ltw2 = P.tw2;
-  short* smono = reinterpret_cast<short*>(lds + wb + mags_b + small_b);
+  short* smono = reinterpret_cast<short*>(LT ? lds + an_lt_front_bytes() + wb : lds + wb + mags_b + small_b);
+  const bool direct = LT && frame_mode == 3;
 
   double* bufA = work + (size_t)wave * (WCT != 0 ? 2 : 4) * W;
   double* bufB = (WCT != 0) ? bufA : bufA + 2 * W;
@@ -479,7 +491,7 @@
   const int jfirst = (j0 > 0) ? j0 - 1 : 0;
   const int64_t sbase = (int64_t)jfirst * B;
   const int nstage = (j1 - jfirst) * B + (W - B);
-  if (frames != nullptr) {
+  if (frames != nullptr || direct) {
   } else if (C == 1) {
     const int16_t* __restrict__ src = in + sbase;
     for (int k0 = tid; k0 < nstage; k0 += 8 * SPX_BLOCK) {
@@ -495,7 +507,175 @@
   __syncthreads();
 
   ASTAMP_DECL
-  if constexpr (WCT == 240) {
+  if constexpr (LT) {
+    const int b = lane;
+    const bool on60 = b < 60, on48 = b < 48;
+    const int bb = on60 ? b : 0;
+    typedef double lc_v2d __attribute__((ext_vector_type(2)));
+    typedef float lc_v4f __attribute__((ext_vector_type(4)));
+    typedef const __attribute__((address_space(1))) lc_v2d* lc_ptr;
+    typedef const __attribute__((address_space(1))) lc_v4f* lc_ptr4;
+    const double2* const lc0 = reinterpret_cast<const double2*>(P.lane_consts);
+    auto take6 = [&](auto fr, int j, int (&m)[6]) {
+      m[0] = fr[0]; m[1] = fr[1]; m[2] = fr[120]; m[3] = fr[121]; m[5] = fr[119];
+      m[4] = fr[bb > 0 ? -1 : (240 - B) - 1];
+      if (bb == 0 && j == 0) m[4] = 0;
+    };
+    auto fetch6 = [&](int s, int (&m)[6]) {
+      const int j = j0 - 1 + s;
+      if (s <= TF && j >= 0 && j < j1) take6(in + (int64_t)j * B + 2 * bb, j, m);
+    };
+    int nx[6] = {0, 0, 0, 0, 0, 0};
+    float hold[4] = {0.0f, 0.0f, 0.0f, 0.0f};
+    if (direct) fetch6(wave, nx);
+    for (int s = wave; s <= TF; s += 4) {
+      const int j = j0 - 1 + s;
+      const bool keep = s + 4 > TF;
+      float* mrow = mags + (size_t)s * MS;
+      if (j < 0 || j >= j1) {
+        if (!keep) for (int k = lane; k < 240; k += SPX_WAVE) mrow[k] = 0.0f;
+#pragma unroll
+        for (int u = 0; u < 4; u++) hold[u] = 0.0f;
+        if (direct) fetch6(s + 4, nx);
+        continue;
+      }
+      int ln = lane;
+      asm volatile("" : "+v"(ln));
+      __builtin_assume(ln >= 0 && ln < SPX_WAVE);
+      const lc_ptr lcb[4] = {(lc_ptr)per_frame(lc0), (lc_ptr)per_frame(lc0 + 256), (lc_ptr)per_frame(lc0 + 512), (lc_ptr)per_frame(lc0 + 768)};
+      typedef const __attribute__((address_space(1))) unsigned char* lc_bytes;
+      unsigned lane_off = 16u * (unsigned)lane;
+      asm volatile("" : "+v"(lane_off));
+      auto lc = [&](int c) -> double2 {
+        const lc_v2d v = *(lc_ptr)((lc_bytes)lcb[c >> 2] + lane_off + 1024u * (unsigned)(c & 3));
+        return make_double2(v.x, v.y);
+      };
+      int m[6];
+      if (direct) {
+#pragma unroll
+        for (int u = 0; u < 6; u++) m[u] = nx[u];
+      } else {
+        take6(smono + (size_t)(j - jfirst) * B + 2 * bb, j, m);
+      }
+      {
+        const lc_v4f wn = *(lc_ptr4)((lc_bytes)lcb[SPX_LC_WN >> 2] + lane_off + 1024u * (SPX_LC_WN & 3));
+        const double2 w1a = lc(SPX_LC_W1 + 0), w1b = lc(SPX_LC_W1 + 1), w1c = lc(SPX_LC_W1 + 2);
+        if (on60) {
+          const double d0 = (double)m[0], d2 = (double)m[2];
+          const cplx a0 = {spx_preemph_win(d0, (double)m[4], wn.x), spx_preemph_win((double)m[1], d0, wn.y)},
+                     a1 = {spx_preemph_win(d2, (double)m[5], wn.z), spx_preemph_win((double)m[3], d2, wn.w)};
+          const cplx b0 = {a0.r + a1.r, a0.i + a1.i}, b2 = {a0.r - a1.r, a0.i - a1.i};
+          const cplx b1 = {a0.r + a1.i, a0.i - a1.r}, b3 = {a0.r - a1.i, a0.i + a1.r};
+          st(bufA, 4 * ln, b0);
+          st(bufA, 4 * ln + 1, cmul_tw(b1, w1a));
+          st(bufA, 4 * ln + 2, cmul_tw(b2, w1b));
+          st(bufA, 4 * ln + 3, cmul_tw(b3, w1c));
+        }
+      }
+      {
+        const double2 w2a = lc(SPX_LC_W2 + 0), w2b = lc(SPX_LC_W2 + 1), w2c = lc(SPX_LC_W2 + 2);
+        wave_sync();
+        ASTAMP(0);
+        if (on60) {
+          const cplx a0 = ld(bufA, ln), a1 = ld(bufA, ln + 60), a2 = ld(bufA, ln + 120), a3 = ld(bufA, ln + 180);
+          wave_sync();
+          const cplx t0 = {a0.r + a2.r, a0.i + a2.i}, t1 = {a0.r - a2.r, a0.i - a2.i};
+          const cplx t2 = {a1.r + a3.r, a1.i + a3.i}, t3 = {a1.r - a3.r, a1.i - a3.i};
+          const cplx b0 = {t0.r + t2.r, t0.i + t2.i}, b2 = {t0.r - t2.r, t0.i - t2.i};
+          const cplx b1 = {t1.r + t3.i, t1.i - t3.r}, b3 = {t1.r - t3.i, t1.i + t3.r};
+          const int o = (ln & 3) + 16 * (ln >> 2);
+          st(bufB, o, b0);
+          st(bufB, o + 4, cmul_tw(b1, w2a));
+          st(bufB, o + 8, cmul_tw(b2, w2b));
+          st(bufB, o + 12, cmul_tw(b3, w2c));
+        }
+      }
+      {
+        double2 w3[2][2];
+#pragma unroll
+        for (int u = 0; u < 2; u++) { w3[u][0] = lc(SPX_LC_W3 + 2 * u); w3[u][1] = lc(SPX_LC_W3 + 2 * u + 1); }
+        wave_sync();
+        cplx q0[2], q1[2], q2[2];
+#pragma unroll
+        for (int u = 0; u < 2; u++) {
+          const int b3i = (ln + 64 * u < 80) ? ln + 64 * u : 0;
+          q0[u] = ld(bufB, b3i); q1[u] = ld(bufB, b3i + 80); q2[u] = ld(bufB, b3i + 160);
+        }
+        wave_sync();
+#pragma unroll
+        for (int u = 0; u < 2; u++) {
+          const int b3i = ln + 64 * u;
+          if (b3i < 80) {
+            const cplx a0 = q0[u], a1 = q1[u], a2 = q2[u];
+            const cplx t1 = {a1.r + a2.r, a1.i + a2.i};
+            const cplx t2 = {spx_bf3h(a0.r, t1.r), spx_bf3h(a0.i, t1.i)};
+            const cplx t3 = {S3_1 * (a1.r - a2.r), S3_1 * (a1.i - a2.i)};
+            const cplx b0 = {a0.r + t1.r, a0.i + t1.i};
+            const cplx b1 = {t2.r + t3.i, t2.i - t3.r}, b2 = {t2.r - t3.i, t2.i + t3.r};
+            const int o = (b3i & 15) + 48 * (b3i >> 4);
+            st(bufA, o, b0);
+            st(bufA, o + 16, cmul_tw(b1, w3[u][0]));
+            st(bufA, o + 32, cmul_tw(b2, w3[u][1]));
+          }
+        }
+      }
+      wave_sync();
+      if (on48) {
+        const cplx a0 = ld(bufA, ln), a1 = ld(bufA, ln + 48), a2 = ld(bufA, ln + 96), a3 = ld(bufA, ln + 144),
+                   a4 = ld(bufA, ln + 192);
+        wave_sync();
+        const cplx t1 = {a1.r + a4.r, a1.i + a4.i}, t2 = {a2.r + a3.r, a2.i + a3.i};
+        const cplx t3 = {a1.r - a4.r, a1.i - a4.i}, t4 = {a2.r - a3.r, a2.i - a3.i};
+        const cplx b0 = {(a0.r + t1.r) + t2.r, (a0.i + t1.i) + t2.i};
+        const cplx m1 = {spx_bf5m(a0.r, C5_1, t1.r, C5_2, t2.r), spx_bf5m(a0.i, C5_1, t1.i, C5_2, t2.i)};
+        const cplx m2 = {spx_bf5m(a0.r, C5_2, t1.r, C5_1, t2.r), spx_bf5m(a0.i, C5_2, t1.i, C5_1, t2.i)};
+        const cplx n1 = {spx_bf5n(S5_1, t3.r, S5_2, t4.r), spx_bf5n(S5_1, t3.i, S5_2, t4.i)};
+        const cplx n2 = {spx_bf5d(S5_2, t3.r, S5_1, t4.r), spx_bf5d(S5_2, t3.i, S5_1, t4.i)};
+        const cplx b1 = {m1.r + n1.i, m1.i - n1.r}, b4 = {m1.r - n1.i, m1.i + n1.r};
+        const cplx b2 = {m2.r + n2.i, m2.i - n2.r}, b3 = {m2.r - n2.i, m2.i + n2.r};
+        st(bufB, ln, b0);
+        st(bufB, ln + 48, b1);
+        st(bufB, ln + 96, b2);
+        st(bufB, ln + 144, b3);
+        st(bufB, ln + 192, b4);
+      }
+      if (direct) fetch6(s + 4, nx);
+      double2 wu[4];
+#pragma unroll
+      for (int u = 0; u < 4; u++) wu[u] = lc(SPX_LC_WU + u);
+      wave_sync();
+      ASTAMP(1);
+      float* spec_out = taps.spectrogram ? taps.spectrogram + (size_t)(S.frame_off + j) * 480 : nullptr;
+#pragma unroll
+      for (int u = 0; u < 4; u++) {
+        const int k = ln + 64 * u;
+        if (k < 240) {
+          const int k2 = (k == 0) ? 0 : 240 - k;
+          const cplx a = ld(bufB, k), c = ld(bufB, k2);
+          const double b_r = c.r, b_i = -c.i;
+          const float mag = spx_untangle_mag(a.r, a.i, b_r, b_i, wu[u]);
+          hold[u] = mag;
+          if (!keep) mrow[k] = mag;
+          if (spec_out) {
+            spec_out[k] = mag;
+            if (k > 0) spec_out[480 - k] = mag;
+            else spec_out[240] = (float)__builtin_fabs(a.r - a.i);
+          }
+        }
+      }
+      wave_sync();
+      ASTAMP(2);
+    }
+    __syncthreads();
+    {
+      float* mrow = mags + (size_t)(wave == 0 ? TF : TF - 4 + wave) * MS;
+#pragma unroll
+      for (int u = 0; u < 4; u++) {
+        const int k = lane + 64 * u;
+        if (k < 240) mrow[k] = hold[u];
+      }
+    }
+  } else if constexpr (WCT == 240) {
     const double2* twp = reinterpret_cast<const double2*>(P.tw);
     const double2* tw2p = reinterpret_cast<const double2*>(P.tw2);
     const int b = lane;
@@ -1075,7 +1255,7 @@
 #endif
 #ifndef SPX_LOG_V1
     if (tid < SPX_WAVE + 128)
-      reinterpret_cast<uint4*>(reinterpret_cast<unsigned char*>(work) + terms_bytes(W, TF, WCT != 0))[tid - SPX_WAVE] =
+      reinterpret_cast<uint4*>(terms_base + terms_bytes(W, TF, WCT != 0))[tid - SPX_WAVE] =
           reinterpret_cast<const uint4*>(spx_log_table_dev)[tid - SPX_WAVE];
 #endif
   } else if (tid <= TF) {
@@ -1119,7 +1299,7 @@
 
   const int nfr = j1 - j0;
 #ifndef SPX_LOG_V1
-  const SpxLogEntry* ltab = reinterpret_cast<const SpxLogEntry*>(reinterpret_cast<const unsigned char*>(work) + terms_bytes(W, TF, WCT != 0));
+  const SpxLogEntry* ltab = reinterpret_cast<const SpxLogEntry*>(terms_base + terms_bytes(W, TF, WCT != 0));
   auto log_of_ratio = [&](float ratio) -> double {
     double v = spx_log_v2_f32(ratio, ltab);
     if (__builtin_expect(!spx_log_v2_domain(ratio), 0)) v = spx_log_v1((double)ratio);
@@ -1169,7 +1349,7 @@
     constexpr int CB = spx_cb(TF);
     constexpr int CBS = CB + 1;
     static_assert(TF * CB == 2 * (SPX_BLOCK - SPX_WAVE), "two terms per lane of waves 1..3 and block");
-    double* tblk = work;
+    double* tblk = reinterpret_cast<double*>(terms_base);
     constexpr int NBLK = (WCT - 1 + CB - 1) / CB;
     float lsd = 0.0f;
     int fi[2], ci[2];
@@ -1383,10 +1563,12 @@
 
 void spx_launch_analysis(const SpxPlanDev& P, const SpxStreamDev* streams, int n_streams, int n_tiles,
                          const int16_t* in, SpxFrameRec* rec, SpxTapsDev taps, const int* tile_order, int* tile_flags,
-                         hipStream_t st) {
+                         bool mono, hipStream_t st) {
   if (n_tiles <= 0) return;
-  SpxLaunch<SpxAnalysisArgs>::go(spx_analysis_select(P.tile_frames, plan_ct_window(P)), n_tiles, spx_analysis_lds_bytes(P), st, P, streams,
-                                 n_streams, in, rec, taps, tile_order, tile_flags, nullptr, 0);
+  const int ctw = plan_ct_window(P);
+  const bool direct = mono && an_lean_layout(P.tile_frames, ctw);
+  SpxLaunch<SpxAnalysisArgs>::go(spx_analysis_select(P.tile_frames, ctw), n_tiles, analysis_lds_bytes(P, ctw, direct), st, P, streams,
+                                 n_streams, in, rec, taps, tile_order, tile_flags, nullptr, direct ? 3 : 0);
 }
 
 void spx_launch_analysis_frames(const SpxPlanDev& P, const SpxStreamDev* streams, int n_tiles, const float* frames,
@@ -1394,6 +1576,6 @@
   if (n_tiles <= 0) return;
   SpxPlanDev Q = P;
   if (Q.tile_frames != SPX_TF_SMALL && Q.tile_frames != SPX_TF_TINY) Q.tile_frames = SPX_TF;
-  SpxLaunch<SpxAnalysisArgs>::go(spx_analysis_select(Q.tile_frames, 0), n_tiles, analysis_lds_bytes(Q, false), st, Q, streams, 1, nullptr, rec,
+  SpxLaunch<SpxAnalysisArgs>::go(spx_analysis_select(Q.tile_frames, 0), n_tiles, analysis_lds_bytes(Q, 0, false), st, Q, streams, 1, nullptr, rec,
                                  taps, nullptr, nullptr, frames, preemph ? 1 : 2);
 }
diff --git a/speedy_amd/csrc/spx_diag.hip b/speedy_amd/csrc/spx_diag.hip
--- a/speedy_amd/csrc/spx_diag.hip
+++ b/speedy_amd/csrc/spx_diag.hip
@@ -59,7 +59,7 @@
   int scratch = -1;
   out[0] = spx_analysis_vgprs(*P, &scratch);
   out[1] = scratch;
-  out[2] = (int)spx_analysis_lds_bytes(*P);
+  out[2] = (int)spx_analysis_lds_bytes(*P, true);
   out[3] = P->dft_waves;
   return 0;
 }
diff --git a/speedy_amd/csrc/spx_engine.hip b/speedy_amd/csrc/spx_engine.hip
--- a/speedy_amd/csrc/spx_engine.hip
+++ b/speedy_amd/csrc/spx_engine.hip
@@ -184,7 +184,10 @@
   return 0;
 }
 
-int walk_stream_count() { return 2; }
+#ifndef SPX_WALK_STREAMS
+#define SPX_WALK_STREAMS 3
+#endif
+int walk_stream_count() { return SPX_WALK_STREAMS; }
 int dev_walk_streams(int dev, hipStream_t* w, int n) {
   static std::mutex mu;
   static hipStream_t s3[64][SPX_MAX_WALK_STREAMS];
@@ -289,9 +292,9 @@
   R.tile_small = spx_analysis_small_tile_frames();
   SpxPlanDev d8 = d;
   d8.tile_frames = R.tile_small;
-  R.an_lds_default = spx_analysis_lds_bytes(d);
+  R.an_lds_default = spx_analysis_lds_bytes(d, maxC == 1);
   R.an_vgprs_default = spx_analysis_vgprs(d);
-  R.an_lds_small = spx_analysis_lds_bytes(d8);
+  R.an_lds_small = spx_analysis_lds_bytes(d8, maxC == 1);
   R.an_vgprs_small = spx_analysis_vgprs(d8);
   if (plan->res_cache.size() > 64) plan->res_cache.clear();
   return plan->res_cache.emplace(key, R).first->second;
@@ -501,7 +504,7 @@
       hipLaunchKernelGGL(spx_gate_kernel, dim3(1), dim3(64), 0, sa, d_ready + n, n, 1200u);
     if (do_a && tiles[c] > 0) {
       SpxTimed tm(timed, 0, sa);
-      spx_launch_analysis(d, dj, n, tiles[c], in, rec, td, concurrent ? d_order : nullptr, concurrent ? d_flags : nullptr, sa);
+      spx_launch_analysis(d, dj, n, tiles[c], in, rec, td, concurrent ? d_order : nullptr, concurrent ? d_flags : nullptr, maxC == 1, sa);
     }
     if (force && force->after_analysis && c == nch - 1) HIPCHK(hipEventRecord(force->after_analysis, sa));
     if (sa != st) HIPCHK(hipEventRecord(plan->ev_chunk[c], sa));
diff --git a/speedy_amd/csrc/spx_internal.h b/speedy_amd/csrc/spx_internal.h
--- a/speedy_amd/csrc/spx_internal.h
+++ b/speedy_amd/csrc/spx_internal.h
@@ -40,7 +40,21 @@
   const int* perm;
   const int* iperm;
   const int* qlog;
-};
+  const void* lane_consts;
+};
+#ifdef SPX_PREEMPH_V1
+#define SPX_WIN_SCALE 1.0f
+#else
+#define SPX_WIN_SCALE 0x1p-15f
+#endif
+#define SPX_LC_W1 0
+#define SPX_LC_W2 3
+#define SPX_LC_W3 6
+#define SPX_LC_WU 10
+#define SPX_LC_WN 14
+#define SPX_LC_ENTRIES 15
+#define SPX_LC_BYTES (SPX_LC_ENTRIES * 64 * 16)
+void spx_lane_consts_fill(const double* tw, const double* tw2, const float* win, unsigned char* out);
 
 #define SPX_F_INIT 1
 #define SPX_F_FLUSH 2
@@ -136,7 +150,7 @@
 
 void spx_launch_analysis(const SpxPlanDev& P, const SpxStreamDev* streams, int n_streams, int n_tiles,
                          const int16_t* in, SpxFrameRec* rec, SpxTapsDev taps, const int* tile_order, int* tile_flags,
-                         hipStream_t st);
+                         bool mono, hipStream_t st);
 void spx_launch_analysis_frames(const SpxPlanDev& P, const SpxStreamDev* streams, int n_tiles, const float* frames,
                                 bool preemph, SpxFrameRec* rec, SpxTapsDev taps, hipStream_t st);
 void spx_launch_tension(const SpxPlanDev& P, const SpxStreamDev* streams, int n_streams, SpxStreamState* states,
@@ -171,7 +185,7 @@
 void spx_launch_walk(const SpxPlanDev& P, const SpxWalkAsk& ask, const SpxStreamDev* streams, const int16_t* in, int16_t* out,
                      int64_t* n_out, SpxStreamState* states, const float* scratch, const int* speed_ready, size_t lds_min,
                      hipStream_t st);
-size_t spx_analysis_lds_bytes(const SpxPlanDev& P);
+size_t spx_analysis_lds_bytes(const SpxPlanDev& P, bool mono);
 int spx_analysis_ct_window(const SpxPlanDev& P);
 void spx_host_dft(int n, const int* radix, int nstages, const double* tw, const double* in, double* out);
 size_t spx_walk_lds_bytes(const SpxPlanDev& P, int max_channels, bool speedup_only);
diff --git a/speedy_amd/csrc/spx_mixed.hip b/speedy_amd/csrc/spx_mixed.hip
--- a/speedy_amd/csrc/spx_mixed.hip
+++ b/speedy_amd/csrc/spx_mixed.hip
@@ -87,7 +87,7 @@
     mg.n = (int)gj[g].size();
     mg.walk = mode_walk(d, {.n_streams = mg.n, .max_channels = maxC, .speedup_only = SC.speedup_only, .any_speed = SC.any_speed});
     mg.any_nonlinear = any_nl;
-    mg.an_lds = spx_analysis_lds_bytes(d);
+    mg.an_lds = spx_analysis_lds_bytes(d, maxC == 1);
     mg.an_vgprs = spx_analysis_vgprs(d);
     G.push_back(mg);
   }
diff --git a/speedy_amd/csrc/spx_mode.h b/speedy_amd/csrc/spx_mode.h
--- a/speedy_amd/csrc/spx_mode.h
+++ b/speedy_amd/csrc/spx_mode.h
@@ -72,6 +72,11 @@
 static inline bool spx_mode_fits2(const SpxModeResources& R, const SpxModeWalk& w, size_t lds_usable) {
   return w.lds + R.tension_lds + 2 * R.an_lds_default <= lds_usable &&
          ((w.waves + 3) / 4) * w.vgprs + R.tension_vgprs + 2 * R.an_vgprs_default <= 512;
+}
+
+static inline int spx_mode_an_waves(const SpxModeResources& R, const SpxModeWalk& w) {
+  const int left = 512 - ((w.waves + 3) / 4) * w.vgprs - R.tension_vgprs;
+  return (left > 0 && R.an_vgprs_default > 0) ? left / R.an_vgprs_default : 0;
 }
 
 static inline SpxMode spx_mode_pass(const SpxModeShape& S, const SpxModeResources& R, const SpxModeEnv& E, const SpxModeRuntime& T,
@@ -165,7 +170,9 @@
   const bool lean_possible = S.do_a && S.do_w && S.max_channels == 1 && S.n <= R.cu_count && R.walk.fast_kernel && R.walk.nwc > 0 &&
                              !S.forced && R.lean_valid && R.walk_lean.fast_kernel && R.walk_lean.nwc == 0;
   const bool lean_fits = lean_possible && spx_mode_fits2(R, R.walk_lean, lds_usable);
-  const bool need_lean = lean_fits && !spx_mode_fits2(R, R.walk, lds_usable);
+  const bool lean_analysis_build = R.tile_default == R.tile_big && R.an_vgprs_default < R.an_vgprs_small;
+  const bool need_lean = lean_fits && (!spx_mode_fits2(R, R.walk, lds_usable) ||
+                                       (lean_analysis_build && spx_mode_an_waves(R, R.walk_lean) > spx_mode_an_waves(R, R.walk)));
   SpxMode M = spx_mode_pass(S, R, E, T, trial_in, need_lean);
   if (!need_lean && lean_fits && M.walk2 && S.overlap_req && !T.two_workspaces) {
     SpxMode L = spx_mode_pass(S, R, E, T, trial_in, true);
diff --git a/speedy_amd/csrc/spx_plan.hip b/speedy_amd/csrc/spx_plan.hip
--- a/speedy_amd/csrc/spx_plan.hip
+++ b/speedy_amd/csrc/spx_plan.hip
@@ -8,6 +8,42 @@
   double s = nonlinear ? 0.01 : (double)speed;
   if (s < 1e-4) s = 1e-4;
   return (int64_t)((double)(n_in + 2 * (int64_t)P.maxRequired) * (2.0 / s)) + slack;
+}
+
+void spx_lane_consts_fill(const double* tw, const double* tw2, const float* win, unsigned char* out) {
+  double* d = reinterpret_cast<double*>(out);
+  auto put = [&](int c, int lane, const double* src, int idx) {
+    d[2 * (64 * c + lane)] = src[2 * idx];
+    d[2 * (64 * c + lane) + 1] = src[2 * idx + 1];
+  };
+  for (int lane = 0; lane < 64; lane++) {
+    const int bb = lane < 60 ? lane : 0;
+    for (int j = 1; j < 4; j++) {
+      put(SPX_LC_W1 + j - 1, lane, tw, bb * j);
+      put(SPX_LC_W2 + j - 1, lane, tw, 4 * (bb >> 2) * j);
+    }
+    for (int u = 0; u < 2; u++) {
+      const int b3 = lane + 64 * u, p3 = (b3 < 80) ? (b3 >> 4) : 0;
+      put(SPX_LC_W3 + 2 * u, lane, tw, 16 * p3);
+      put(SPX_LC_W3 + 2 * u + 1, lane, tw, 32 * p3);
+    }
+    for (int u = 0; u < 4; u++) {
+      const int k = lane + 64 * u;
+      put(SPX_LC_WU + u, lane, tw2, k < 240 ? k : 0);
+    }
+    float* f = reinterpret_cast<float*>(out + 16 * (size_t)(64 * SPX_LC_WN + lane));
+    const int wi[4] = {2 * bb, 2 * bb + 1, 2 * bb + 120, 2 * bb + 121};
+    for (int k = 0; k < 4; k++) f[k] = win[wi[k]] * SPX_WIN_SCALE;
+  }
+}
+static void plan_host_tables(int W, double* tw, double* tw2, float* win) {
+  for (int t = 0; t < W; t++) {
+    spx_tw::entry(t, W, &tw[2 * t]);
+    spx_tw::entry(t, 2L * W, &tw2[2 * t]);
+    double c = 1.0, sn = 0.0;
+    if (W > 1) spx_tw::sincos_2pi(t, W - 1, &c, &sn);
+    win[t] = 0.54 - 0.46 * c;
+  }
 }
 
 void spx_internal_set_error(const char* msg) { g_spx_err = msg ? msg : ""; }
@@ -26,6 +62,13 @@
   return h;
 }
 int spx_abi_version(void) { return 1; }
+int spx_debug_lane_consts(int sample_rate, void* out, double* tw, double* tw2, float* win) {
+  if (!out || !tw || !tw2 || !win) return -1;
+  if ((int)(1.5 * sample_rate / (float)100.0) != 240) return 0;
+  plan_host_tables(240, tw, tw2, win);
+  spx_lane_consts_fill(tw, tw2, win, static_cast<unsigned char*>(out));
+  return SPX_LC_BYTES;
+}
 
 static int factor_radices(int n, int* radix) {
   int ns = 0;
@@ -92,7 +135,7 @@
   for (int c = 0; c < 5; c++) {
     d.tile_frames = cand[c][0];
     d.dft_waves = cand[c][1];
-    if (spx_analysis_lds_bytes(d) <= 160 * 1024) break;
+    if (spx_analysis_lds_bytes(d, false) <= 160 * 1024) break;
   }
   if (spx_analysis_prefers_small_tile(d)) {
     d.tile_frames = spx_analysis_small_tile_frames();
@@ -102,8 +145,11 @@
   const size_t n_rd = rader ? 2 * (size_t)M : 0;
   const size_t n_ri = rader ? (size_t)M : 0;
   const size_t n_ql = rader ? (size_t)W : 0;
-  const size_t bytes = sizeof(double) * (2 * n_tw + 2 * n_rd) + sizeof(float) * (n_win + n_tf + n_tp + 8) +
-                       sizeof(int) * (2 * n_ri + n_ql);
+  const size_t bytes0 = sizeof(double) * (2 * n_tw + 2 * n_rd) + sizeof(float) * (n_win + n_tf + n_tp + 8) +
+                        sizeof(int) * (2 * n_ri + n_ql);
+  const bool lane_tab = !rader && W == 240;
+  const size_t off_lc = (bytes0 + 15) & ~(size_t)15;
+  const size_t bytes = lane_tab ? off_lc + SPX_LC_BYTES : bytes0;
   std::vector<unsigned char> host(bytes, 0);
   double* tw = reinterpret_cast<double*>(host.data());
   double* tw2 = tw + n_tw;
@@ -115,13 +161,8 @@
   int* perm = reinterpret_cast<int*>(tp + n_tp + 8);
   int* iperm = perm + n_ri;
   int* qlog = iperm + n_ri;
-  for (int t = 0; t < W; t++) {
-    spx_tw::entry(t, W, &tw[2 * t]);
-    spx_tw::entry(t, 2L * W, &tw2[2 * t]);
-    double c = 1.0, sn = 0.0;
-    if (W > 1) spx_tw::sincos_2pi(t, W - 1, &c, &sn);
-    win[t] = 0.54 - 0.46 * c;
-  }
+  plan_host_tables(W, tw, tw2, win);
+  if (lane_tab) spx_lane_consts_fill(tw, tw2, win, host.data() + off_lc);
   if (rader) {
     for (int t = 0; t < M; t++) spx_tw::entry(t, M, &twM[2 * t]);
     int g = 2;
@@ -174,6 +215,7 @@
   d.perm = reinterpret_cast<const int*>(d.taperP + n_tp + 8);
   d.iperm = d.perm + n_ri;
   d.qlog = d.iperm + n_ri;
+  d.lane_consts = lane_tab ? base + off_lc : nullptr;
   return p;
 }
 
@@ -218,7 +260,7 @@
 }
 
 }
-bool spx_internal_analysis_fits(const SpxPlanDev& d) { return spx_analysis_lds_bytes(d) <= 160 * 1024; }
+bool spx_internal_analysis_fits(const SpxPlanDev& d) { return spx_analysis_lds_bytes(d, false) <= 160 * 1024; }
 
 spx_plan* shared_plan_full(int sample_rate, int match_matlab) {
   static std::mutex mu;
```

New measurement: 49750, median of 6. 9.5% higher.
